# AIBluefisher/DReg-NeRF

Measured on AMD Instinct MI355X. Metric: nerf_pairs_per_sec_regtr_fwd_bwd_128, higher is better.
Workload: dtype bf16; 1 GPU; RegTR fwd+bwd+AdamW, shell-R synthetic pairs, 128^3 grids, 4 pairs (8 grids) per GPU per step, random-init weights; global_batch_pairs=4, resolution=128, fpn_head=active-set (identical results; rows around occupied voxels), parallelism=dp1

## Files before the change

dreg_nerf_amd/csrc/conv.hip:

```cpp
#include "common.h"
#include "../../include/dreg_nerf.h"
#include <cstring>
extern "C" int dreg_fill_zero(void* p, size_t bytes, void* stream);

struct ConvGeom {
    int B, Di, Hi, Wi, Cin, log2Cin;
    int Cmask;
    int Do, Ho, Wo, Cout;
    int ksz, ntaps;
    int sn, dsign, off, sd;
    uint32_t M;
    uint32_t magW, magH, magD;
    int Kpad;
};

__device__ __forceinline__ void tap_decode(int tap, int ksz, int& dz, int& dy, int& dx) {
    if (ksz == 1) { dz = dy = dx = 0; }
    else if (ksz == 3) { dz = tap / 9; int r = tap - dz * 9; dy = r / 3; dx = r - dy * 3; }
    else { int k2 = ksz * ksz; dz = tap / k2; int r = tap - dz * k2; dy = r / ksz; dx = r - dy * ksz; }
}

__device__ __forceinline__ void vox_decode(uint32_t m, const ConvGeom& g, int& b, int& z, int& y, int& x) {
    uint32_t q1 = fdiv(m, g.magW); x = (int)(m - q1 * g.Wo);
    uint32_t q2 = fdiv(q1, g.magH); y = (int)(q1 - q2 * g.Ho);
// ... 785 lines not shown
        }
    };

    if (v_begin < v_end) {
        const int nk = (int)((v_end - v_begin + KV - 1) / KV);
        auto next = [&](int k) {
            if (rowocc)
                while (k < nk && rowocc[(v_begin + (uint32_t)k * KV) / (uint32_t)g.Wo] == 0) ++k;
            return k;
        };
        int k = next(0), buf = 0;
        if (k < nk) {
            load_g(v_begin + (uint32_t)k * KV);
            store_l(0);
        }
        __syncthreads();
        while (k < nk) {
            const int kn = next(k + 1);
            if (kn < nk) load_g(v_begin + (uint32_t)kn * KV);
            compute(buf);
            if (kn < nk) store_l(buf ^ 1);
            __syncthreads();
            k = kn; buf ^= 1;
        }
    }
    float* dst = part + (size_t)blockIdx.y * g.Cout * g.Kpad;
    const int col_l = lane & 15, rowq = (lane >> 4) * 4;
#pragma unroll
    for (int i = 0; i < TM; ++i)
#pragma unroll
        for (int r = 0; r < 4; ++r) {
            const int co = co0 + wm * WM + i * 16 + rowq + r;
#pragma unroll
            for (int j = 0; j < TN; ++j)
                dst[(size_t)co * g.Kpad + n0 + wn * WN + j * 16 + col_l] = acc[i][j][r];
        }
}

#ifdef DREG_PROBE
__device__ unsigned long long g_wgrad_dbg[8];
#endif
template <int GP> __device__ __forceinline__ int wg_swz(int row) {
    return GP >= 16 ? (((row & 3) + 4 * ((row >> 3) & 1)) << 1) : ((((row >> 1) & 1) + 2 * ((row >> 3) & 1)) << 1);
}

struct WgradGroupDesc {
    const bf16_t* gout; const bf16_t* in; float* part;
    ConvGeom g;
    int tilesCol, tiles, nsplit;
    uint32_t vps, gbytes, ibytes, nrows;
    int block0;
};
static_assert(sizeof(WgradGroupDesc) == 144, "descriptor layout is part of the ABI (dreg_wgrad_group_desc_bytes)");
template <int BM, int BNC, bool ROWS, int NW = 4, int ABL = 0, int KV_ = 64, int NS_ = 2, int PIPE = 0, int AP = 0, bool GRP = false>
__global__ __launch_bounds__(NW * 64) void conv_wgrad_glds_kernel(
    const bf16_t* __restrict__ gout, const bf16_t* __restrict__ in, float* __restrict__ part,
    ConvGeom g, int tilesCol, int tiles, int nsplit, uint32_t vox_per_split, uint32_t gout_bytes, uint32_t in_bytes,
    const int* __restrict__ rowlist, uint32_t nrows, const uint8_t* __restrict__ rowocc = nullptr, int rows_fast = 0)
{
    uint32_t bid = blockIdx.x;
    if constexpr (GRP) {
        const WgradGroupDesc* D = reinterpret_cast<const WgradGroupDesc*>(rowocc);
        int lo = 0, hi = rows_fast - 1;
        while (lo < hi) {
            const int mid = (lo + hi + 1) >> 1;
            if (D[mid].block0 <= (int)bid) lo = mid; else hi = mid - 1;
        }
        const WgradGroupDesc d = D[lo];
        gout = d.gout; in = d.in; part = d.part; g = d.g; tilesCol = d.tilesCol; tiles = d.tiles; nsplit = d.nsplit;
        vox_per_split = d.vps; gout_bytes = d.gbytes; in_bytes = d.ibytes; nrows = d.nrows;
        rowocc = nullptr; rows_fast = 0; rowlist = nullptr;
        bid -= (uint32_t)d.block0;
    }
    typedef __attribute__((address_space(3))) void* lds_ptr_t;
    typedef __attribute__((address_space(3))) bf16x4_t* lds4_t;
    constexpr int KV = KV_, NS = NS_;
    constexpr int RSA = BM * 2, RSB = BNC * 2;
    constexpr int GPA = RSA / 16, GPB = RSB / 16;
    constexpr int A_BYTES = KV * RSA, B_BYTES = KV * RSB, STAGE = A_BYTES + B_BYTES;
    constexpr int IA = A_BYTES / 1024 / NW, IB = B_BYTES / 1024 / NW;
    constexpr int LPS = IA + IB;
    static_assert(IA >= 1 && IB >= 1, "stage too small for the wave count");
    constexpr int RPA = 64 / GPA, RPB = 64 / GPB;
    constexpr int WAVES_N = NW / 2;
    constexpr int WN = BNC / WAVES_N, WM = BM / 2, TM = WM / 16, TN = WN / 16;
    constexpr uint32_t OOB = 0x7fffff00u;
    extern __shared__ __attribute__((aligned(16))) char smem[];

    const int t = threadIdx.x, lane = t & 63;
    const int wave = __builtin_amdgcn_readfirstlane(t >> 6);
    const int wm = wave / WAVES_N, wn = wave % WAVES_N;
    uint32_t split, tile;
    if ((nsplit & 7) == 0) { const uint32_t xcd = bid & 7, j = bid >> 3; split = (j / tiles) * 8 + xcd; tile = j % tiles; }
    else { split = bid / tiles; tile = bid - split * tiles; }
    const uint32_t tile_r = tile / tilesCol, tile_c = tile - tile_r * tilesCol;
    const int co0 = tile_r * BM, n0 = tile_c * BNC;
    const uint32_t v_begin = split * vox_per_split;
    const uint32_t v_end = min(v_begin + vox_per_split, nrows);
    const int* srow = reinterpret_cast<const int*>(smem + NS * STAGE);
    typedef __attribute__((ext_vector_type(2))) uint32_t u32x2_t;
    const u32x2_t* srow2 = reinterpret_cast<const u32x2_t*>(smem + NS * STAGE);
    if constexpr (ROWS && AP >= 3) {
        u32x2_t* w2_ = reinterpret_cast<u32x2_t*>(smem + NS * STAGE);
        const uint32_t nreal = v_begin < v_end ? v_end - v_begin : 0u;
        const uint32_t npad = ((nreal + KV - 1) / KV + 4) * KV;
        const uint32_t m_sent = 0x7fffff00u / (uint32_t)((g.Cout > g.Cin ? g.Cout : g.Cin) * 2) + 1u;
        for (uint32_t i = t; i < npad; i += NW * 64) {
            if (i < nreal) {
                const int m = rowlist[v_begin + i];
                int b, z, y, x;
                vox_decode((uint32_t)m, g, b, z, y, x);
                const uint32_t fl = (z == 0 ? 1u : 0u) | (z == g.Do - 1 ? 2u : 0u) | (y == 0 ? 4u : 0u) | (y == g.Ho - 1 ? 8u : 0u) |
                                    (x == 0 ? 16u : 0u) | (x == g.Wo - 1 ? 32u : 0u) | 256u;
                w2_[i] = (u32x2_t){(uint32_t)m, fl};
            } else w2_[i] = (u32x2_t){m_sent, 128u};
        }
        __syncthreads();
    } else
    if constexpr (ROWS) {
        int* w_ = reinterpret_cast<int*>(smem + NS * STAGE);
        u32x2_t* w2_ = reinterpret_cast<u32x2_t*>(smem + NS * STAGE);
        for (uint32_t i = v_begin + t; i < v_end; i += NW * 64) {
            const int m = rowlist[i];
            if (rows_fast) {
                int b, z, y, x;
                vox_decode((uint32_t)m, g, b, z, y, x);
                w2_[i - v_begin] = (u32x2_t){(uint32_t)m, ((uint32_t)z << 20) | ((uint32_t)y << 10) | (uint32_t)x};
            } else w_[i - v_begin] = m;
        }
        __syncthreads();
    }
    const __amdgpu_buffer_rsrc_t rs_g = __builtin_amdgcn_make_buffer_rsrc((void*)gout, 0, gout_bytes, 0x00020000);
    const __amdgpu_buffer_rsrc_t rs_in = __builtin_amdgcn_make_buffer_rsrc((void*)in, 0, in_bytes, 0x00020000);

    const int ra = lane / GPA, rb = lane / GPB;
    uint32_t a_col[IA];
    int b_dz[IB], b_dy[IB], b_dx[IB], b_ci[IB];
    bool b_tv[IB];
#pragma unroll
    for (int i = 0; i < IA; ++i) {
        const int row = (wave * IA + i) * RPA + ra;
        a_col[i] = (uint32_t)(co0 + (((lane % GPA) ^ wg_swz<GPA>(row)) * 8)) * 2u;
    }
#pragma unroll
    for (int i = 0; i < IB; ++i) {
        const int row = (wave * IB + i) * RPB + rb;
        const int n = n0 + (((lane % GPB) ^ wg_swz<GPB>(row)) * 8);
        const int tap = n >> g.log2Cin;
        b_ci[i] = n & g.Cmask;
        tap_decode(tap, g.ksz, b_dz[i], b_dy[i], b_dx[i]);
        b_dz[i] *= g.dsign; b_dy[i] *= g.dsign; b_dx[i] *= g.dsign;
        b_tv[i] = tap < g.ntaps && b_ci[i] < g.Cin;
    }

    f32x4_t acc[TM][TN];
#pragma unroll
    for (int i = 0; i < TM; ++i)
#pragma unroll
        for (int j = 0; j < TN; ++j) acc[i][j] = (f32x4_t){0.f, 0.f, 0.f, 0.f};

    const bool aligned = !ROWS && g.sn == 1 && g.sd == 1 && g.dsign == 1 &&
                         (((KV % g.Wo) == 0 && ((g.Ho * g.Wo) % KV) == 0) || (g.Wo % KV) == 0) &&
                         (uint64_t)g.B * g.Di * g.Hi * g.Wi * g.Cin * 2 < 0x7fffff00ull;
    int al_dz[IB], al_dy[IB], al_x[IB];
    uint32_t al_off[IB];
    uint32_t al_l[IB];
    if (ROWS && rows_fast) {
#pragma unroll
        for (int i = 0; i < IB; ++i) {
            al_dz[i] = g.off + b_dz[i]; al_dy[i] = g.off + b_dy[i]; al_x[i] = g.off + b_dx[i];
            al_off[i] = (uint32_t)((((al_dz[i] * g.Hi + al_dy[i]) * g.Wi + al_x[i]) * g.Cin + b_ci[i]) * 2);
        }
    }
    if (aligned) {
#pragma unroll
        for (int i = 0; i < IB; ++i) {
            const int l = (wave * IB + i) * RPB + rb;
            const int ly = l / g.Wo, lx = l - ly * g.Wo;
            al_l[i] = b_tv[i] ? (uint32_t)l : 0x7fffffffu;
            al_dz[i] = g.off + b_dz[i];
            al_dy[i] = ly + g.off + b_dy[i];
            al_x[i] = lx + g.off + b_dx[i];
            al_off[i] = (uint32_t)((((al_dz[i] * g.Hi + al_dy[i]) * g.Wi + al_x[i]) * g.Cin + b_ci[i]) * 2);
        }
    }

    auto issue = [&](uint32_t v0, int buf) {
        char* sA = smem + buf * STAGE;
        char* sB = sA + A_BYTES;
        if constexpr (ROWS) {
            if (rows_fast) {
                uint32_t am[IA];
                u32x2_t bm[IB];
                const uint32_t last = v_end - 1 - v_begin;
#pragma unroll
                for (int i = 0; i < IA; ++i) am[i] = srow2[min(v0 + (wave * IA + i) * RPA + ra - v_begin, last)][0];
#pragma unroll
                for (int i = 0; i < IB; ++i) bm[i] = srow2[min(v0 + ((wave * IB) + i) * RPB + rb - v_begin, last)];
#pragma unroll
                for (int i = 0; i < IA; ++i) {
                    const int j = wave * IA + i;
                    const uint32_t vi = v0 + j * RPA + ra;
                    const uint32_t voff = (vi < v_end) ? am[i] * (uint32_t)(g.Cout * 2) + a_col[i] : OOB;
                    if constexpr (ABL != 3) __builtin_amdgcn_raw_ptr_buffer_load_lds(rs_g, (lds_ptr_t)(sA + j * 1024), 16, (int)voff, 0, 0, 0);
                    else asm volatile("" :: "v"(voff));
                }
#pragma unroll
                for (int i = 0; i < IB; ++i) {
                    const int j = wave * IB + i;
                    const uint32_t vi = v0 + j * RPB + rb, p = bm[i][1];
                    const bool v = vi < v_end && b_tv[i] && (unsigned)((int)(p >> 20) + al_dz[i]) < (unsigned)g.Di &&
                                   (unsigned)((int)((p >> 10) & 1023u) + al_dy[i]) < (unsigned)g.Hi && (unsigned)((int)(p & 1023u) + al_x[i]) < (unsigned)g.Wi;
// ... 127 lines not shown
            for (int ks = 0; ks < KS; ++ks)
#pragma unroll
                for (int grp = 0; grp < NG; ++grp) {
                    const int as = (ks * NG + grp) & 1, bs = ks & 1;
                    if (grp + 1 < NG) rdA(ks, grp + 1, as ^ 1);
                    else if (ks + 1 < KS) { rdB(ks + 1, bs ^ 1); rdA(ks + 1, 0, as ^ 1); }
                    __builtin_amdgcn_sched_barrier(0);
                    bf16x8_t af[G], bf[TN];
#pragma unroll
                    for (int i = 0; i < G; ++i) { i32x4_t t4 = {alo[as][i][0], alo[as][i][1], ahi[as][i][0], ahi[as][i][1]}; af[i] = __builtin_bit_cast(bf16x8_t, t4); }
#pragma unroll
                    for (int j = 0; j < TN; ++j) { i32x4_t t4 = {blo[bs][j][0], blo[bs][j][1], bhi[bs][j][0], bhi[bs][j][1]}; bf[j] = __builtin_bit_cast(bf16x8_t, t4); }
#pragma unroll
                    for (int i = 0; i < G; ++i)
#pragma unroll
                        for (int j = 0; j < TN; ++j)
                            acc[grp * G + i][j] = __builtin_amdgcn_mfma_f32_16x16x32_bf16(af[i], bf[j], acc[grp * G + i][j], 0, 0, 0);
                    asm volatile("s_waitcnt lgkmcnt(0)" ::: "memory");
                    __builtin_amdgcn_sched_barrier(0);
                }
            return;
        }
#pragma unroll
        for (int ks = 0; ks < KV / 32; ++ks) {
            const int kb = ks * 32 + (lane >> 4) * 8;
            const int r0 = kb + (fi >> 2), r1 = r0 + 4;
            i32x2_t alo[TM], ahi[TM], blo[TN], bhi[TN];
#pragma unroll
            for (int i = 0; i < TM; ++i) {
                const int gi = (wm * WM + i * 16) / 8 + ((fi & 3) >> 1), o8 = (fi & 1) * 8;
                alo[i] = tr_read(sA + r0 * RSA + ((gi ^ wg_swz<GPA>(r0)) << 4) + o8);
                ahi[i] = tr_read(sA + r1 * RSA + ((gi ^ wg_swz<GPA>(r1)) << 4) + o8);
            }
#pragma unroll
            for (int j = 0; j < TN; ++j) {
                const int gi = (wn * WN + j * 16) / 8 + ((fi & 3) >> 1), o8 = (fi & 1) * 8;
                blo[j] = tr_read(sB + r0 * RSB + ((gi ^ wg_swz<GPB>(r0)) << 4) + o8);
                bhi[j] = tr_read(sB + r1 * RSB + ((gi ^ wg_swz<GPB>(r1)) << 4) + o8);
            }
            asm volatile("s_waitcnt lgkmcnt(0)" ::: "memory");
            __builtin_amdgcn_sched_barrier(0);
            bf16x8_t af[TM], bf[TN];
#pragma unroll
            for (int i = 0; i < TM; ++i) { typedef __attribute__((ext_vector_type(4))) int i32x4_t; i32x4_t t4 = {alo[i][0], alo[i][1], ahi[i][0], ahi[i][1]}; af[i] = __builtin_bit_cast(bf16x8_t, t4); }
#pragma unroll
            for (int j = 0; j < TN; ++j) { typedef __attribute__((ext_vector_type(4))) int i32x4_t; i32x4_t t4 = {blo[j][0], blo[j][1], bhi[j][0], bhi[j][1]}; bf[j] = __builtin_bit_cast(bf16x8_t, t4); }
#pragma unroll
            for (int i = 0; i < TM; ++i)
#pragma unroll
                for (int j = 0; j < TN; ++j) {
                    if constexpr (ABL != 1) acc[i][j] = __builtin_amdgcn_mfma_f32_16x16x32_bf16(af[i], bf[j], acc[i][j], 0, 0, 0);
                    else asm volatile("" :: "v"(af[i]), "v"(bf[j]));
                }
        }
    };

    if constexpr (AP) {
        constexpr bool FAST = AP >= 3, STAMP = (AP == 2 || AP == 4);
        static_assert(NW == 8 && KV == 32 && NS == 4 && PIPE == 0 && LPS <= 15, "anti-phase loop: 8 waves, four 32-voxel units in the ring");
        if (v_begin < v_end) {
            const int nk = (int)((v_end - v_begin + KV - 1) / KV);
            const int grp = wave >> 2;
            const int fi = lane & 15;
            i32x2_t alo[TM], ahi[TM], blo[TN], bhi[TN];
            uint32_t fa[TM + TN];
            if constexpr (FAST) {
                static_assert(RSA == RSB, "one row stride for both operands");
                const int kb = (lane >> 4) * 8;
                const int r0 = kb + (fi >> 2);
#pragma unroll
                for (int i = 0; i < TM; ++i) {
                    const int gi = (wm * WM + i * 16) / 8 + ((fi & 3) >> 1), o8 = (fi & 1) * 8;
                    fa[i] = lds_base + r0 * RSA + ((gi ^ wg_swz<GPA>(r0)) << 4) + o8;
                }
#pragma unroll
                for (int j = 0; j < TN; ++j) {
                    const int gi = (wn * WN + j * 16) / 8 + ((fi & 3) >> 1), o8 = (fi & 1) * 8;
                    fa[TM + j] = lds_base + A_BYTES + r0 * RSB + ((gi ^ wg_swz<GPB>(r0)) << 4) + o8;
                }
            }
            auto tr_read_o = [&](uint32_t addr, int which) -> i32x2_t {
                i32x2_t v;
                if constexpr (ABL != 2) {
                    if (which == 0) asm volatile("ds_read_b64_tr_b16 %0, %1" : "=v"(v) : "v"(addr));
                    else if (which == 1) asm volatile("ds_read_b64_tr_b16 %0, %1 offset:%2" : "=v"(v) : "v"(addr), "n"(4 * RSA));
                    else if (which == 2) asm volatile("ds_read_b64_tr_b16 %0, %1 offset:%2" : "=v"(v) : "v"(addr), "n"(STAGE));
                    else asm volatile("ds_read_b64_tr_b16 %0, %1 offset:%2" : "=v"(v) : "v"(addr), "n"(STAGE + 4 * RSA));
                } else { v = (i32x2_t){(int)addr, (int)addr}; asm volatile("" : "+v"(v)); }
                return v;
            };
            auto rd = [&](int buf) {
                if constexpr (FAST) {
                    const int odd = (buf & 1) * 2;
#pragma unroll
                    for (int i = 0; i < TM; ++i) { alo[i] = tr_read_o(fa[i], odd); ahi[i] = tr_read_o(fa[i], odd + 1); }
#pragma unroll
                    for (int j = 0; j < TN; ++j) { blo[j] = tr_read_o(fa[TM + j], odd); bhi[j] = tr_read_o(fa[TM + j], odd + 1); }
                    return;
                }
                const uint32_t sA = lds_base + buf * STAGE;
                const uint32_t sB = sA + A_BYTES;
                const int kb = (lane >> 4) * 8;
                const int r0 = kb + (fi >> 2), r1 = r0 + 4;
#pragma unroll
                for (int i = 0; i < TM; ++i) {
                    const int gi = (wm * WM + i * 16) / 8 + ((fi & 3) >> 1), o8 = (fi & 1) * 8;
                    alo[i] = tr_read(sA + r0 * RSA + ((gi ^ wg_swz<GPA>(r0)) << 4) + o8);
                    ahi[i] = tr_read(sA + r1 * RSA + ((gi ^ wg_swz<GPA>(r1)) << 4) + o8);
                }
#pragma unroll
                for (int j = 0; j < TN; ++j) {
                    const int gi = (wn * WN + j * 16) / 8 + ((fi & 3) >> 1), o8 = (fi & 1) * 8;
                    blo[j] = tr_read(sB + r0 * RSB + ((gi ^ wg_swz<GPB>(r0)) << 4) + o8);
                    bhi[j] = tr_read(sB + r1 * RSB + ((gi ^ wg_swz<GPB>(r1)) << 4) + o8);
                }
            };
            auto mm = [&]() {
                typedef __attribute__((ext_vector_type(4))) int i32x4_t;
                bf16x8_t af[TM], bf[TN];
#pragma unroll
                for (int i = 0; i < TM; ++i) { i32x4_t t4 = {alo[i][0], alo[i][1], ahi[i][0], ahi[i][1]}; af[i] = __builtin_bit_cast(bf16x8_t, t4); }
#pragma unroll
                for (int j = 0; j < TN; ++j) { i32x4_t t4 = {blo[j][0], blo[j][1], bhi[j][0], bhi[j][1]}; bf[j] = __builtin_bit_cast(bf16x8_t, t4); }
#pragma unroll
                for (int i = 0; i < TM; ++i)
#pragma unroll
                    for (int j = 0; j < TN; ++j) {
                        if constexpr (ABL != 1) acc[i][j] = __builtin_amdgcn_mfma_f32_16x16x32_bf16(af[i], bf[j], acc[i][j], 0, 0, 0);
                        else asm volatile("" :: "v"(af[i]), "v"(bf[j]));
                    }
            };
            uint32_t pa_off[IA], pb_off[IB], pb_m[IB];
            int cz = 0, cy = 0, cx = 0;
            uint32_t lp = 0;
            u32x2_t lm[IA];
            if constexpr (FAST && ROWS) {
                static_assert(IA == IB && RPA == RPB, "one row per lane for both operands");
                lp = lds_base + NS * STAGE + (uint32_t)(wave * IA * RPA + ra) * 8u;
#pragma unroll
                for (int i = 0; i < IA; ++i) pa_off[i] = a_col[i];
#pragma unroll
                for (int i = 0; i < IB; ++i) {
                    const int dz = g.off + b_dz[i], dy = g.off + b_dy[i], dx = g.off + b_dx[i];
                    pb_off[i] = (uint32_t)((((dz * g.Hi + dy) * g.Wi + dx) * g.Cin + b_ci[i]) * 2);
                    pb_m[i] = (dz < 0 ? 1u : 0u) | (dz > 0 ? 2u : 0u) | (dy < 0 ? 4u : 0u) | (dy > 0 ? 8u : 0u) |
                              (dx < 0 ? 16u : 0u) | (dx > 0 ? 32u : 0u) | 128u | (b_tv[i] ? 0u : 256u);
                }
            } else
            if constexpr (FAST) {
#pragma unroll
                for (int i = 0; i < IA; ++i) pa_off[i] = (uint32_t)((wave * IA + i) * RPA + ra) * (uint32_t)(g.Cout * 2) + a_col[i];
#pragma unroll
                for (int i = 0; i < IB; ++i) {
                    const int l = (wave * IB + i) * RPB + rb;
                    const int dz = g.off + b_dz[i], dy = g.off + b_dy[i], dx = g.off + b_dx[i];
                    pb_off[i] = (uint32_t)((((dz * g.Hi + dy) * g.Wi + (l + dx)) * g.Cin + b_ci[i]) * 2);
                    pb_m[i] = (dz < 0 ? 1u : 0u) | (dz > 0 ? 2u : 0u) | (dy < 0 ? 4u : 0u) | (dy > 0 ? 8u : 0u) |
                              (l + dx < 0 ? 16u : 0u) | (l + dx >= KV ? 32u : 0u) | (b_tv[i] ? 0u : 64u);
                }
                int cb;
                vox_decode(v_begin, g, cb, cz, cy, cx);
            }
            uint32_t voa[IA], vob[IB];
            uint32_t cur_a = v_begin * (uint32_t)(g.Cout * 2), cur_b = v_begin * (uint32_t)(g.Cin * 2);
            uint32_t m_zy = 0;
            auto zy_flags = [&]() { m_zy = (cz == 0 ? 1u : 0u) | (cz == g.Do - 1 ? 2u : 0u) | (cy == 0 ? 4u : 0u) | (cy == g.Ho - 1 ? 8u : 0u) | 64u; };
            if constexpr (FAST) zy_flags();
            uint32_t nx_mask = 0, nx_a = 0, nx_b = 0;
            auto prep_scalar = [&]() {
                nx_mask = m_zy | (cx == 0 ? 16u : 0u) | (cx + KV == g.Wo ? 32u : 0u);
                nx_a = cur_a; nx_b = cur_b;
                cur_a += (uint32_t)(KV * 2) * (uint32_t)g.Cout; cur_b += (uint32_t)(KV * 2) * (uint32_t)g.Cin; cx += KV;
                if (cx == g.Wo) {
                    asm volatile("" ::: "memory");
                    cx = 0; if (++cy == g.Ho) { cy = 0; if (++cz == g.Do) cz = 0; } zy_flags();
                }
            };
            auto prep_fast = [&]() {
#pragma unroll
                for (int i = 0; i < IA; ++i) voa[i] = nx_a + pa_off[i];
#pragma unroll
                for (int i = 0; i < IB; ++i) vob[i] = (pb_m[i] & nx_mask) == 0u ? nx_b + pb_off[i] : OOB;
            };
// ... 37 lines not shown
            }
            if constexpr (FAST && ROWS) {
                for (int p = nk < 3 ? nk : 3; p < 3; ++p) list_read();
                list_read(); asm volatile("s_waitcnt lgkmcnt(0)" ::: "memory"); prep_rows();
            } else if constexpr (FAST) { prep_scalar(); prep_fast(); }
            if (nk >= 3) asm volatile("s_waitcnt vmcnt(%0)" ::"n"(2 * LPS) : "memory");
            else if (nk == 2) asm volatile("s_waitcnt vmcnt(%0)" ::"n"(LPS) : "memory");
            else asm volatile("s_waitcnt vmcnt(0)" ::: "memory");
            __builtin_amdgcn_s_barrier();
            if (grp) __builtin_amdgcn_s_barrier();
            unsigned long long dsum[6] = {0, 0, 0, 0, 0, 0}, tprev = 0;
            auto stamp = [&](int q) {
                if constexpr (STAMP) {
                    unsigned long long tnow;
                    asm volatile("s_memtime %0\n\ts_waitcnt lgkmcnt(0)" : "=s"(tnow) :: "memory");
                    if (q >= 0) dsum[q] += tnow - tprev;
                    tprev = tnow;
                }
            };
            stamp(-1);
            auto unit = [&](int u, int slot) {
                rd(slot);
                if constexpr (FAST && ROWS) list_read();
                stamp(0);
                if (u + 3 < nk) {
                    request(u + 3);
                    stamp(1);
                    asm volatile("s_waitcnt vmcnt(%0)" ::"n"(2 * LPS) : "memory");
                } else {
                    stamp(1);
                    if (u + 2 < nk) asm volatile("s_waitcnt vmcnt(%0)" ::"n"(LPS) : "memory");
                    else asm volatile("s_waitcnt vmcnt(0)" ::: "memory");
                }
                asm volatile("s_waitcnt lgkmcnt(0)" ::: "memory");
                stamp(2);
                __builtin_amdgcn_sched_barrier(0);
                __builtin_amdgcn_s_barrier();
                stamp(3);
                __builtin_amdgcn_s_setprio(1);
                if constexpr (FAST && ROWS) prep_rows();
                else if constexpr (FAST) { prep_scalar(); prep_fast(); }
                mm();
                if constexpr (FAST) {
#pragma unroll
                    for (int q = 0; q < 14; ++q) {
                        __builtin_amdgcn_sched_group_barrier(0x008, 1, 0);
                        __builtin_amdgcn_sched_group_barrier(0x004, 1, 0);
                        __builtin_amdgcn_sched_group_barrier(0x008, 1, 0);
                        __builtin_amdgcn_sched_group_barrier(0x002, 1, 0);
                    }
                }
                __builtin_amdgcn_s_setprio(0);
                __builtin_amdgcn_sched_barrier(0);
                stamp(4);
                __builtin_amdgcn_s_barrier();
                stamp(5);
            };
            if constexpr (FAST) {
                for (int u = 0; u < nk; u += 4) {
                    unit(u, 0);
                    if (u + 1 < nk) unit(u + 1, 1);
#pragma unroll
                    for (int k = 0; k < TM + TN; ++k) fa[k] += 2u * STAGE;
                    if (u + 2 < nk) unit(u + 2, 2);
                    if (u + 3 < nk) unit(u + 3, 3);
#pragma unroll
                    for (int k = 0; k < TM + TN; ++k) fa[k] -= 2u * STAGE;
                }
            } else {
                for (int u = 0; u < nk; ++u) unit(u, u & 3);
            }
            if (!grp) __builtin_amdgcn_s_barrier();
            if constexpr (STAMP) {
#ifdef DREG_PROBE
                if (lane == 0) {
                    for (int q = 0; q < 6; ++q) atomicAdd(&g_wgrad_dbg[q], dsum[q]);
                    atomicAdd(&g_wgrad_dbg[6], (unsigned long long)nk);
                    atomicAdd(&g_wgrad_dbg[7], 1ull);
                }
#endif
            }
        }
    } else
    if (v_begin < v_end) {
        const int nk = (int)((v_end - v_begin + KV - 1) / KV);
        if (rowocc) {
            uint8_t* socc = reinterpret_cast<uint8_t*>(smem + NS * STAGE);
            for (int i = t; i < nk; i += NW * 64) socc[i] = rowocc[(v_begin + (uint32_t)i * KV) / (uint32_t)g.Wo];
            __syncthreads();
            auto next = [&](int k) { while (k < nk && socc[k] == 0) ++k; return k; };
            int k = next(0), buf = 0;
            if (k < nk) issue(v_begin + (uint32_t)k * KV, 0);
            while (k < nk) {
                const int kn = next(k + 1);
                asm volatile("s_waitcnt vmcnt(0)" ::: "memory");
                __builtin_amdgcn_s_barrier();
                if (kn < nk) issue(v_begin + (uint32_t)kn * KV, buf ^ 1);
                compute(buf);
                k = kn; buf ^= 1;
            }
        } else {
        static_assert(NS >= 2 && NS <= 5 && 3 * LPS <= 63, "ring depth / counted wait range");
        for (int p = 0; p < NS - 1 && p < nk; ++p) issue(v_begin + (uint32_t)p * KV, p);
        int cur = 0, nxt = NS - 1;
        for (int k = 0; k < nk; ++k) {
            const int ahead = min(nk - 1 - k, NS - 2);
            if (ahead >= 3) asm volatile("s_waitcnt vmcnt(%0)" ::"n"(3 * LPS) : "memory");
            else if (ahead == 2) asm volatile("s_waitcnt vmcnt(%0)" ::"n"(2 * LPS) : "memory");
            else if (ahead == 1) asm volatile("s_waitcnt vmcnt(%0)" ::"n"(LPS) : "memory");
            else asm volatile("s_waitcnt vmcnt(0)" ::: "memory");
            __builtin_amdgcn_s_barrier();
            if (k + NS - 1 < nk) issue(v_begin + (uint32_t)(k + NS - 1) * KV, nxt);
            compute(cur);
            cur = cur + 1 == NS ? 0 : cur + 1;
            nxt = nxt + 1 == NS ? 0 : nxt + 1;
        }
        }
    }
    float* dst = part + (size_t)split * g.Cout * g.Kpad;
    const int col_l = lane & 15, rowq = (lane >> 4) * 4;
#pragma unroll
    for (int i = 0; i < TM; ++i)
#pragma unroll
        for (int r = 0; r < 4; ++r) {
            const int co = co0 + wm * WM + i * 16 + rowq + r;
#pragma unroll
            for (int j = 0; j < TN; ++j) {
                const int n = n0 + wn * WN + j * 16 + col_l;
                if (n < g.Kpad) dst[(size_t)co * g.Kpad + n] = acc[i][j][r];
            }
        }
}

struct WgradReduceDesc {
    const float* part; float* dw;
    int nsplit, Cout, Kpad, ntaps, Cin, Cin_real, accumulate, block0;
};
static_assert(sizeof(WgradReduceDesc) == 48, "descriptor layout is part of the ABI");
constexpr int WR_STAGE = 8192;
__host__ __device__ static inline int wr_epb(int nsplit) { return nsplit < 8 ? 2048 : (nsplit < 64 ? 512 : 128); }
__host__ __device__ static inline int wr_chunk(int nsplit) { return nsplit < 32 ? 64 : 16; }
static inline int wgrad_reduce_blocks(int Cout, int Cin_real, int ntaps, int nsplit)
{
    if (ntaps == 1) return (int)(((size_t)Cout * Cin_real + wr_epb(nsplit) - 1) / wr_epb(nsplit));
    return Cout * ((Cin_real + wr_chunk(nsplit) - 1) / wr_chunk(nsplit));
}
__device__ __forceinline__ float wr_sum(const float* p, size_t slab, int k0, int kstep, int nsplit)
{
    float a = 0.f;
#pragma unroll 4
    for (int k = k0; k < nsplit; k += kstep) a += p[(size_t)k * slab];
    return a;
}
__device__ __forceinline__ void wgrad_reduce_block(const WgradReduceDesc& d, int r, float* stage)
{
    const int t = threadIdx.x;
    const size_t slab = (size_t)d.Cout * d.Kpad;
    int nwritten = d.nsplit;
    if (d.accumulate & 2) {
        const int e = *reinterpret_cast<const int*>(d.part + (size_t)d.nsplit * slab);
        nwritten = e < 1 ? 1 : (e < d.nsplit ? e : d.nsplit);
    }
    const bool accum = (d.accumulate & 1) != 0;
    if (d.ntaps == 1) {
        const int epb = wr_epb(d.nsplit), KG = 2048 / epb, EL = 256 / KG, g = t / EL, l = t - g * EL;
        const size_t total = (size_t)d.Cout * d.Cin_real;
        const bool vec = (d.Cin_real & 3) == 0;
        const int per = vec ? 4 : 1, passes = epb / (EL * per);
        for (int ps = 0; ps < passes; ++ps) {
            const size_t i = (size_t)r * epb + (size_t)(ps * EL + l) * per;
            float4 a = make_float4(0.f, 0.f, 0.f, 0.f);
            if (i < total) {
                const int co = (int)(i / d.Cin_real), ci = (int)(i - (size_t)co * d.Cin_real);
                const float* src = d.part + (size_t)co * d.Kpad + ci;
                if (vec) {
#pragma unroll 4
                    for (int k = g; k < nwritten; k += KG) {
                        const float4 v = *reinterpret_cast<const float4*>(src + (size_t)k * slab);
                        a.x += v.x; a.y += v.y; a.z += v.z; a.w += v.w;
                    }
                } else a.x = wr_sum(src, slab, g, KG, nwritten);
            }
            if (KG > 1) {
                __syncthreads();
                reinterpret_cast<float4*>(stage)[g * EL + l] = a;
                __syncthreads();
                if (g == 0) {
                    a = reinterpret_cast<float4*>(stage)[l];
                    for (int q = 1; q < KG; ++q) { const float4 v = reinterpret_cast<float4*>(stage)[q * EL + l]; a.x += v.x; a.y += v.y; a.z += v.z; a.w += v.w; }
                }
            }
            if (g == 0 && i < total) {
                if (vec) {
                    float4* o = reinterpret_cast<float4*>(d.dw + i);
                    if (accum) { const float4 q = *o; a.x += q.x; a.y += q.y; a.z += q.z; a.w += q.w; }
                    *o = a;
                } else d.dw[i] = accum ? d.dw[i] + a.x : a.x;
            }
        }
        return;
    }
    const int cc = wr_chunk(d.nsplit);
    const int nchunk = (d.Cin_real + cc - 1) / cc;
    const int co = r / nchunk, ci0 = (r - co * nchunk) * cc;
    const int nci = min(cc, d.Cin_real - ci0);
    const int chp = d.Cin < cc ? d.Cin : cc;
    const int sh = 31 - __builtin_clz(chp);
    const int ne = d.ntaps << sh;
    const int no = nci * d.ntaps;
    const int KG = (d.nsplit >= 8 && 4 * no <= WR_STAGE) ? 4 : 1, EL = 256 / KG, g = t / EL, l = t - g * EL;
    const float* src = d.part + (size_t)co * d.Kpad + ci0;
    if ((chp & 3) == 0 && (d.Cin & 3) == 0 && (d.Kpad & 3) == 0) {
        for (int e = l; e < (ne >> 2); e += EL) {
            const int tap = (e << 2) >> sh, cl = (e << 2) & (chp - 1);
            if (cl >= nci) continue;
            const float* p = src + (size_t)tap * d.Cin + cl;
// ... 611 lines not shown
    static_assert(sizeof(PackDesc) == 48, "descriptor layout is part of the ABI");
    if (n <= 0 || total_rows <= 0) return DREG_OK;
    if (stage_floats < 0 || (size_t)stage_floats * 4 > 48 * 1024) return DREG_EINVAL;
    hipLaunchKernelGGL(pack_weights_batched_kernel, dim3(total_rows), dim3(256), (size_t)(stage_floats > 0 ? 64 * 125 : 1) * 4, (hipStream_t)stream,
                       (const PackDesc*)descs, n, row_desc);
    DREG_LAUNCH_CHECK();
    return DREG_OK;
}

DREG_KNOB(int, g_force_wgrad_splits, 0);
DREG_KNOB(int, g_wgrad_target_blocks, 384);
#ifdef DREG_PROBE
void dreg_conv_set_narrow_small(int on) { if (on >= 10) { g_narrow_small = 2; g_narrow_thr = on; } else { g_narrow_small = on; g_narrow_thr = 224; } }
void dreg_conv_set_glds_stages(int stages) { g_glds_stages = (stages >= 2 && stages <= 4) ? stages : 0; }
void dreg_conv_set_wgrad_target_blocks(int blocks) { g_wgrad_target_blocks = blocks > 0 ? blocks : 384; }
void dreg_conv_set_wgrad_splits(int splits) { g_force_wgrad_splits = splits; }
#endif
int dreg_conv3d_wgrad_splits(int B, int Do, int Ho, int Wo, int Cin, int Cout, int ksz, int dtype) {
    if (g_force_wgrad_splits > 0) {
        const long Mf = (long)B * Do * Ho * Wo;
        long f = g_force_wgrad_splits;
        if (f > (Mf + 63) / 64) f = (Mf + 63) / 64;
        return (int)(f > 64 ? 64 : (f < 1 ? 1 : f));
    }
    const int Kpad = dreg_conv3d_kpad(ksz, Cin, dtype);
    const int bnc = (Kpad % 128 == 0 || (dtype == 0 && Kpad > 128)) ? 128 : 64;
    const long tiles = (long)((Cout % 128 == 0) ? Cout / 128 : Cout / 64) * ((Kpad + bnc - 1) / bnc);
    const long M = (long)B * Do * Ho * Wo;
    long s = (g_wgrad_target_blocks + tiles - 1) / tiles;
    const long vmin = ksz == 1 ? 512 : 1024;
    const long maxs = (M + vmin - 1) / vmin;
    if (s > maxs) s = maxs;
    if (s < 1) s = 1;
    const long cap = (tiles * 64 >= 1024 || dtype != 0) ? 64 : ((1024 + tiles - 1) / tiles > 512 ? 512 : (1024 + tiles - 1) / tiles);
    if (s > cap) s = cap;
    if (s > 8) s = (s + 7) / 8 * 8;
    if (dtype == 0 && Cout % 256 == 0 && (Kpad % 256 == 0 || Kpad >= 1024) && M >= 65536) {
        const long t256 = (long)(Cout / 256) * ((Kpad + 255) / 256);
        long best = s;
        double best_eff = 0.0;
        for (long c = 24; c <= 64; c += 8) {
            if (M / c < 2048) break;
            const double rounds = (double)(t256 * c) / 256.0;
            const double eff = rounds / (double)((t256 * c + 255) / 256);
            if (eff >= best_eff - 1e-9) { best_eff = eff; best = c; }
        }
        if (best_eff > 0.0) s = best;
    }
    return (int)s;
}
size_t dreg_conv3d_wgrad_workspace_bytes(int B, int Do, int Ho, int Wo, int Cin, int Cout, int ksz, int dtype) {
    const int Kpad = dreg_conv3d_kpad(ksz, Cin, dtype);
    return (size_t)dreg_conv3d_wgrad_splits(B, Do, Ho, Wo, Cin, Cout, ksz, dtype) * Cout * Kpad * sizeof(float) + 256;
}
DREG_KNOB(bool, g_row_splits, true);
#ifdef DREG_PROBE
extern "C" void dreg_conv_set_row_splits(int on) { g_row_splits = on != 0; }
#endif
static int wgrad_row_splits(int Cout, int Kpad, int ksz, uint32_t nrows, int smax, bool tile256)
{
    if (smax <= 1 || !g_row_splits) return smax;
    if (tile256) {
        const long t256 = (long)(Cout / 256) * ((Kpad + 255) / 256);
        const long vmax = (((long)160 * 1024 - (long)4 * 32 * 512 * 2 - 5 * 32 * 8) / 8) / 64 * 64;
        long cmin = ((long)nrows + vmax - 1) / vmax;
        if (cmin < 1) cmin = 1;
        if (cmin >= smax) return smax;
        long cmax = (long)nrows / 2048;
        if (cmax > smax) cmax = smax;
        if (cmax < cmin) cmax = cmin;
        long best = cmin;
        double best_eff = -1.0;
        for (long c = cmin; c <= cmax; ++c) {
            const double eff = (double)(t256 * c) / 256.0 / (double)((t256 * c + 255) / 256);
            if (eff > best_eff + 1e-9) { best_eff = eff; best = c; }
        }
        return (int)best;
    }
    const long vmin = ksz == 1 ? 512 : 1024;
    long s = ((long)nrows + vmin - 1) / vmin;
    if (s < 1) s = 1;
    return (int)(s < smax ? s : smax);
}

}

enum WgradFamily {
    WG_UNSUPPORTED = -1,
    WG_REG,
    WG_GLDS4,
    WG_256x128,
    WG_DENSE8,
    WG_ROWS8,
    WG_ROWS8_AP
};
struct WgradChoice {
    WgradFamily family;
    int bm, bnc, tilesRow, tilesCol;
    int smax, nsplit;
    uint32_t vps;
    int rows_fast;
    bool occ;
    int abl, kv, ns, pipe, ap;
    uint64_t gbytes, ibytes;
    dim3 grid; int block; size_t lds;
};
// ... 7 lines not shown
    const bool k256 = Cout % 256 == 0 && (Kpad % 256 == 0 || Kpad >= 1024);
    const bool rows_ap = rowlist && same_vol && g_rows_fast && g_wgrad_big == 3 && g_wgrad_ring == 3 && g.ksz <= 3 && k256 && nrows >= 16384;
    c.nsplit = rowlist ? wgrad_row_splits(Cout, Kpad, g.ksz, nrows, c.smax, rows_ap) : c.smax;
    c.vps = (uint32_t)((nrows + c.nsplit - 1) / c.nsplit);
    c.vps = ((c.vps + 63) / 64) * 64;
    if (c.vps == 0) c.vps = 64;
    c.gbytes = (uint64_t)g.M * Cout * 2; c.ibytes = (uint64_t)g.B * g.Di * g.Hi * g.Wi * g.Cin * 2;
    const bool glds = dtype == 0 && use_tr && g_use_glds && c.gbytes < 0x7fffff00ull && c.ibytes < 0x7fffff00ull;
    c.bm = (Cout % 128 == 0) ? 128 : 64;
    c.bnc = (Kpad % 128 == 0 || (glds && Kpad > 128)) ? 128 : 64;
    if (g_narrow_small >= 2 && dtype == 0 && (Cout / c.bm) * ((Kpad + c.bnc - 1) / c.bnc) * c.nsplit < g_narrow_thr) {
        if (c.bnc == 128) c.bnc = 64;
        if (c.bm == 128 && (Cout / c.bm) * (Kpad / c.bnc) * c.nsplit < g_narrow_thr) c.bm = 64;
    }
    c.occ = occ && !rowlist && g.Wo % 64 == 0;
    c.kv = 64; c.ns = 2; c.block = 256;
    size_t lds_rows = 0;
    if (!glds) c.family = WG_REG;
    else if (rowlist && c.vps > 20480) { c.family = WG_UNSUPPORTED; return c; }
    else if (rows_ap && (size_t)4 * 32 * 512 * 2 + ((size_t)c.vps + 5 * 32) * 8 <= (size_t)160 * 1024) {
        c.family = WG_ROWS8_AP; c.kv = 32; c.ns = 4; c.ap = 3; c.rows_fast = 1; lds_rows = ((size_t)c.vps + 5 * 32) * 8;
    } else if (rowlist && same_vol && g_rows_fast && g_wgrad_big == 3 && Cout % 256 == 0 && Kpad % 256 == 0 && nrows >= 65536 &&
               (size_t)2 * 64 * 512 * 2 + (size_t)c.vps * 8 <= (size_t)160 * 1024) {
        c.family = WG_ROWS8; c.rows_fast = 1; lds_rows = (size_t)c.vps * 8;
    } else if (!rowlist && !c.occ && g_wgrad_big && Cout % 256 == 0 && (Kpad % 256 == 0 || (Kpad >= 1024 && g_wgrad_big == 3 && g_wgrad_ring >= 3 && !g_wgrad_pipe)) && nrows >= 65536) {
        c.family = WG_DENSE8;
        if (g_wgrad_big == 1) { c.family = WG_256x128; c.kv = 32; }
        else if (g_wgrad_big >= 11 && g_wgrad_big <= 13) c.abl = g_wgrad_big - 10;
        else if (g_wgrad_pipe && !g_wgrad_ring) c.pipe = 1;
        else if (g_wgrad_ring == 2) { c.kv = 32; c.ns = 5; }
        else if (g_wgrad_ring >= 3 && g_wgrad_ring <= 8) {
            const bool fast_ok = g.ksz <= 3 && g.sn == 1 && g.sd == 1 && g.dsign == 1 && g.Di == g.Do && g.Hi == g.Ho && g.Wi == g.Wo && (g.Wo % 32) == 0 &&
                                 (g.M % 32u) == 0 && (c.vps % 32u) == 0;
            c.kv = 32; c.ns = 4;
            if (g_wgrad_ring == 8 || !fast_ok) c.ap = 1;
            else if (g_wgrad_ring == 3) c.ap = 3;
            else { c.ap = 4; c.abl = g_wgrad_ring == 5 ? 2 : (g_wgrad_ring == 6 ? 3 : (g_wgrad_ring == 7 ? 1 : 0)); }
        } else if (g_wgrad_ring == 1) { c.kv = 32; c.ns = 4; }
    } else {
        c.family = WG_GLDS4;
        if (rowlist) {
            c.rows_fast = (same_vol && g_rows_fast && (size_t)2 * 64 * (c.bm + c.bnc) * 2 + (size_t)c.vps * 8 <= (size_t)160 * 1024) ? 1 : 0;
            lds_rows = (size_t)c.vps * (c.rows_fast ? 8 : 4);
        } else if (c.occ) lds_rows = (size_t)(c.vps / 64 + 16);
    }
    if (c.family == WG_256x128) { c.bm = 256; c.bnc = 128; }
    else if (c.family >= WG_DENSE8) { c.bm = 256; c.bnc = 256; c.block = 512; }
    c.tilesRow = Cout / c.bm; c.tilesCol = (Kpad + c.bnc - 1) / c.bnc;
    if (c.family == WG_REG) { c.grid = dim3(c.tilesRow * c.tilesCol, c.nsplit); c.lds = (size_t)2 * 32 * (c.bm + c.bnc) * es; }
    else { c.grid = dim3(c.tilesRow * c.tilesCol * c.nsplit); c.lds = (size_t)c.ns * c.kv * (c.bm + c.bnc) * 2 + lds_rows; }
    return c;
}

struct WgradArgs { const void *gout, *in; float* part; const int* rowlist; uint32_t nrows; const uint8_t* rowocc; };
template <typename T, bool TR>
static void wgrad_reg_launch(const WgradChoice& c, const ConvGeom& g, const WgradArgs& a, hipStream_t st)
{
#define WG_LAUNCH(BMv, BNv) hipLaunchKernelGGL((conv_wgrad_kernel<T, BMv, BNv, TR>), c.grid, dim3(c.block), c.lds, st, (const T*)a.gout, (const T*)a.in, a.part, g, c.tilesCol, c.vps, a.rowocc)
    if (c.bm == 128 && c.bnc == 128) WG_LAUNCH(128, 128); else if (c.bm == 128) WG_LAUNCH(128, 64);
    else if (c.bnc == 128) WG_LAUNCH(64, 128); else WG_LAUNCH(64, 64);
#undef WG_LAUNCH
}
template <int BM, int BNC, bool ROWS, int NW = 4, int ABL = 0, int KV = 64, int NS = 2, int PIPE = 0, int AP = 0>
static void wgrad_glds_launch(const WgradChoice& c, const ConvGeom& g, const WgradArgs& a, hipStream_t st)
{
    if (c.lds > 65536) (void)hipFuncSetAttribute((const void*)conv_wgrad_glds_kernel<BM, BNC, ROWS, NW, ABL, KV, NS, PIPE, AP>, hipFuncAttributeMaxDynamicSharedMemorySize, (int)c.lds);
    hipLaunchKernelGGL((conv_wgrad_glds_kernel<BM, BNC, ROWS, NW, ABL, KV, NS, PIPE, AP>), c.grid, dim3(c.block), c.lds, st, (const bf16_t*)a.gout, (const bf16_t*)a.in, a.part, g,
                       c.tilesCol, c.tilesRow * c.tilesCol, c.nsplit, c.vps, (uint32_t)c.gbytes, (uint32_t)c.ibytes, a.rowlist, a.nrows, a.rowocc, c.rows_fast);
}
template <bool ROWS>
static void wgrad_glds4_launch(const WgradChoice& c, const ConvGeom& g, const WgradArgs& a, hipStream_t st)
{
    if (c.bm == 128 && c.bnc == 128) wgrad_glds_launch<128, 128, ROWS>(c, g, a, st); else if (c.bm == 128) wgrad_glds_launch<128, 64, ROWS>(c, g, a, st);
    else if (c.bnc == 128) wgrad_glds_launch<64, 128, ROWS>(c, g, a, st); else wgrad_glds_launch<64, 64, ROWS>(c, g, a, st);
}
static void wgrad_dense8_launch(const WgradChoice& c, const ConvGeom& g, const WgradArgs& a, hipStream_t st)
{
#define D8(A, KVv, NSv, PPv, APv) if (c.abl == A && c.kv == KVv && c.ns == NSv && c.pipe == PPv && c.ap == APv) return wgrad_glds_launch<256, 256, false, 8, A, KVv, NSv, PPv, APv>(c, g, a, st)
    D8(0, 32, 4, 0, 3); D8(0, 32, 4, 0, 1);
    D8(0, 64, 2, 0, 0); D8(0, 32, 4, 0, 0); D8(0, 32, 5, 0, 0); D8(0, 64, 2, 1, 0);
    D8(1, 64, 2, 0, 0); D8(2, 64, 2, 0, 0); D8(3, 64, 2, 0, 0);
    D8(0, 32, 4, 0, 4); D8(1, 32, 4, 0, 4); D8(2, 32, 4, 0, 4); D8(3, 32, 4, 0, 4);
#undef D8
}

static int wgrad_impl(const void* gout, const void* in, float* dw, void* workspace, size_t workspace_bytes,
                      int B, int Di, int Hi, int Wi, int Cin, int Cin_real, int Do, int Ho, int Wo, int Cout,
                      int ksz, int stride, int pad, int accumulate, int dtype, int use_tr, void* stream,
                      const int* rowlist, uint32_t nrows_list, const uint8_t* rowocc = nullptr, bool defer_reduce = false)
{
    ConvGeom g;
    int rc = fill_geom(g, B, Di, Hi, Wi, Cin, Do, Ho, Wo, Cout, ksz, stride, pad, 0, dtype == 0 ? 2 : 4);
    if (rc) return rc;
    if (Cout % 128 != 0 && Cout != 64) return DREG_EINVAL;
    if (workspace_bytes < dreg_conv3d_wgrad_workspace_bytes(B, Do, Ho, Wo, Cin, Cout, ksz, dtype)) return DREG_EINVAL;
    if (rowlist && !(dtype == 0 && use_tr && g_use_glds)) return DREG_EINVAL;
    hipStream_t st = (hipStream_t)stream;
    const WgradChoice c = wgrad_choose(g, dtype, use_tr != 0, rowlist != nullptr, nrows_list, rowocc != nullptr);
    float* part = (float*)workspace;
    const WgradArgs a{gout, in, part, rowlist, rowlist ? nrows_list : g.M, c.occ ? rowocc : nullptr};
    switch (c.family) {
    case WG_UNSUPPORTED: return DREG_EINVAL;
    case WG_REG:
        if (dtype != 0) wgrad_reg_launch<float, false>(c, g, a, st);
        else if (use_tr) wgrad_reg_launch<bf16_t, true>(c, g, a, st);
        else wgrad_reg_launch<bf16_t, false>(c, g, a, st);
        break;
    case WG_GLDS4: if (rowlist) wgrad_glds4_launch<true>(c, g, a, st); else wgrad_glds4_launch<false>(c, g, a, st); break;
    case WG_256x128: wgrad_glds_launch<256, 128, false, 4, 0, 32>(c, g, a, st); break;
    case WG_DENSE8: wgrad_dense8_launch(c, g, a, st); break;
    case WG_ROWS8: wgrad_glds_launch<256, 256, true, 8>(c, g, a, st); break;
    case WG_ROWS8_AP: wgrad_glds_launch<256, 256, true, 8, 0, 32, 4, 0, 3>(c, g, a, st); break;
    }
    DREG_LAUNCH_CHECK();
    if (defer_reduce) {
        if (rowlist && hipMemsetD32Async((hipDeviceptr_t)(part + (size_t)c.smax * Cout * g.Kpad), c.nsplit, 1, st) != hipSuccess) return DREG_ELAUNCH;
        return DREG_OK;
    }
    if (g.ntaps > 1 && (size_t)g.ntaps * (Cin < 64 ? Cin : 64) > (size_t)WR_STAGE) return DREG_EINVAL;
    WgradReduceDesc rd{part, dw, c.nsplit, Cout, g.Kpad, g.ntaps, Cin, Cin_real, accumulate, 0};
    hipLaunchKernelGGL(wgrad_reduce_kernel, dim3(wgrad_reduce_blocks(Cout, Cin_real, g.ntaps, c.nsplit)), dim3(256), 0, st, rd);
    DREG_LAUNCH_CHECK();
    return DREG_OK;
}

extern "C" {

int dreg_wgrad_group_desc_bytes() { return (int)sizeof(WgradGroupDesc); }
int dreg_linear_wgrad_group_fill(void* desc_host, const void* gout, const void* in, void* workspace, size_t workspace_bytes,
                                 int rows, int Cin, int Cout, int* variant, int* nblocks)
{
    return dreg_conv3d_wgrad_group_fill(desc_host, gout, in, workspace, workspace_bytes, rows, 1, 1, 1, Cin, 1, 1, 1, Cout, 1, 1, 0, variant, nblocks);
}
int dreg_conv3d_wgrad_group_fill(void* desc_host, const void* gout, const void* in, void* workspace, size_t workspace_bytes,
                                 int B, int Di, int Hi, int Wi, int Cin, int Do, int Ho, int Wo, int Cout, int ksz, int stride, int pad,
                                 int* variant, int* nblocks)
{
    ConvGeom g;
    int rc = fill_geom(g, B, Di, Hi, Wi, Cin, Do, Ho, Wo, Cout, ksz, stride, pad, 0, 2);
    if (rc) return rc;
    if (Cout % 128 != 0 && Cout != 64) return DREG_EINVAL;
    if (workspace_bytes < dreg_conv3d_wgrad_workspace_bytes(B, Do, Ho, Wo, Cin, Cout, ksz, 0)) return DREG_EINVAL;
    const WgradChoice c = wgrad_choose(g, 0, true, false, 0, false);
    if (c.family != WG_GLDS4) return DREG_EINVAL;
    WgradGroupDesc d{};
    d.gout = (const bf16_t*)gout; d.in = (const bf16_t*)in; d.part = (float*)workspace; d.g = g;
    d.tilesCol = c.tilesCol; d.tiles = c.tilesRow * c.tilesCol; d.nsplit = c.nsplit; d.vps = c.vps; d.gbytes = (uint32_t)c.gbytes; d.ibytes = (uint32_t)c.ibytes;
    d.nrows = g.M; d.block0 = 0;
    std::memcpy(desc_host, &d, sizeof(d));
    *variant = c.bm * 1000 + c.bnc;
    *nblocks = (int)c.grid.x;
    return DREG_OK;
}
int dreg_wgrad_group_launch(const void* descs_dev, int n, int variant, int total_blocks, void* stream)
{
    if (n <= 0 || total_blocks <= 0) return DREG_OK;
    if (!descs_dev) return DREG_EINVAL;
    hipStream_t st = (hipStream_t)stream;
    const int bm = variant / 1000, bnc = variant % 1000;
    const ConvGeom g0{};
#define WGRP(BMv, BNv) hipLaunchKernelGGL((conv_wgrad_glds_kernel<BMv, BNv, false, 4, 0, 64, 2, 0, 0, true>), dim3(total_blocks), dim3(256), (size_t)2 * 64 * (BMv + BNv) * 2, st, \
        (const bf16_t*)nullptr, (const bf16_t*)nullptr, (float*)nullptr, g0, 0, 0, 0, 0u, 0u, 0u, (const int*)nullptr, 0u, (const uint8_t*)descs_dev, n)
    if (bm == 128 && bnc == 128) WGRP(128, 128); else if (bm == 128 && bnc == 64) WGRP(128, 64);
    else if (bm == 64 && bnc == 128) WGRP(64, 128); else if (bm == 64 && bnc == 64) WGRP(64, 64);
    else return DREG_EINVAL;
#undef WGRP
    DREG_LAUNCH_CHECK();
    return DREG_OK;
}

int dreg_conv3d_wgrad(const void* gout, const void* in, float* dw, void* workspace, size_t workspace_bytes,
                      int B, int Di, int Hi, int Wi, int Cin, int Cin_real, int Do, int Ho, int Wo, int Cout,
                      int ksz, int stride, int pad, int accumulate, int dtype, int use_tr, void* stream)
{
    return wgrad_impl(gout, in, dw, workspace, workspace_bytes, B, Di, Hi, Wi, Cin, Cin_real, Do, Ho, Wo, Cout, ksz, stride, pad,
                      accumulate, dtype, use_tr, stream, nullptr, 0);
}
int dreg_conv3d_wgrad_occ(const void* gout, const void* in, float* dw, void* workspace, size_t workspace_bytes,
                          int B, int Di, int Hi, int Wi, int Cin, int Cin_real, int Do, int Ho, int Wo, int Cout,
                          int ksz, int stride, int pad, int accumulate, int dtype, int use_tr, const uint8_t* rowocc, void* stream)
{
    return wgrad_impl(gout, in, dw, workspace, workspace_bytes, B, Di, Hi, Wi, Cin, Cin_real, Do, Ho, Wo, Cout, ksz, stride, pad,
                      accumulate, dtype, use_tr, stream, nullptr, 0, rowocc);
}

int dreg_conv3d_igemm_rows(const void* in, const void* wt_packed, void* out, const float* bias, const void* addend,
                           const int* rows, int nrows,
                           int B, int Di, int Hi, int Wi, int Cin, int Do, int Ho, int Wo, int Cout,
                           int ksz, int stride, int pad, int transposed, int relu, int Da, int Ha, int Wa, int add_same,
                           int out_f32, void* stream)
{
    ConvGeom g;
    int rc = fill_geom(g, B, Di, Hi, Wi, Cin, Do, Ho, Wo, Cout, ksz, stride, pad, transposed, 2);
    if (rc) return rc;
    if (!rows || nrows < 0) return DREG_EINVAL;
    const int add_shift = add_same ? 0 : 1;
    hipStream_t st = (hipStream_t)stream;
    if (out_f32) return launch_conv<bf16_t, float>(in, wt_packed, out, bias, addend, g, relu, Da, Ha, Wa, add_shift, st, rows, (uint32_t)nrows);
    return launch_conv<bf16_t, bf16_t>(in, wt_packed, out, bias, addend, g, relu, Da, Ha, Wa, add_shift, st, rows, (uint32_t)nrows);
}
int dreg_conv3d_wgrad_partials(const void* gout, const void* in, void* workspace, size_t workspace_bytes, const int* rows, int nrows,
                               int B, int Di, int Hi, int Wi, int Cin, int Cin_real, int Do, int Ho, int Wo, int Cout,
                               int ksz, int stride, int pad, const uint8_t* rowocc, void* stream)
{
    if (rows && nrows < 0) return DREG_EINVAL;
    return wgrad_impl(gout, in, nullptr, workspace, workspace_bytes, B, Di, Hi, Wi, Cin, Cin_real, Do, Ho, Wo, Cout, ksz, stride, pad,
                      0, 0, 1, stream, rows, rows ? (uint32_t)nrows : 0, rows ? nullptr : rowocc, true);
}
int dreg_wgrad_reduce_blocks(int Cout, int Cin_real, int ksz, int nsplit) { return wgrad_reduce_blocks(Cout, Cin_real, ksz * ksz * ksz, nsplit); }
int dreg_wgrad_reduce_batched(const void* descs_dev, int n, int block_base, int nblocks, void* stream)
{
    if (n <= 0 || nblocks <= 0) return DREG_OK;
    if (!descs_dev || block_base < 0) return DREG_EINVAL;
    hipLaunchKernelGGL(wgrad_reduce_batched_kernel, dim3(nblocks), dim3(256), 0, (hipStream_t)stream, (const WgradReduceDesc*)descs_dev, n, block_base);
    DREG_LAUNCH_CHECK();
    return DREG_OK;
}
int dreg_conv3d_wgrad_variant(int B, int Do, int Ho, int Wo, int Cin, int Cout, int ksz, int rows, int nrows, int occ)
{
    ConvGeom g;
    if (fill_geom(g, B, Do, Ho, Wo, Cin, Do, Ho, Wo, Cout, ksz, 1, ksz / 2, 0, 2) || (Cout % 128 != 0 && Cout != 64) || (rows && nrows < 0)) return -1;
    const WgradChoice c = wgrad_choose(g, 0, true, rows != 0, (uint32_t)nrows, occ != 0);
    if (c.family == WG_UNSUPPORTED) return -1;
    return (c.family == WG_REG ? 1000000 : 0) + c.bm * 1000 + c.bnc;
}
int dreg_conv3d_wgrad_rows(const void* gout, const void* in, float* dw, void* workspace, size_t workspace_bytes,
                           const int* rows, int nrows,
                           int B, int Di, int Hi, int Wi, int Cin, int Cin_real, int Do, int Ho, int Wo, int Cout,
                           int ksz, int stride, int pad, int accumulate, void* stream)
{
    if (!rows || nrows < 0) return DREG_EINVAL;
    return wgrad_impl(gout, in, dw, workspace, workspace_bytes, B, Di, Hi, Wi, Cin, Cin_real, Do, Ho, Wo, Cout, ksz, stride, pad,
                      accumulate, 0, 1, stream, rows, (uint32_t)nrows);
}

}
```

dreg_nerf_amd/csrc/executor.hip:

```cpp
#include <hip/hip_runtime.h>
#include <cstdint>
#include <cstring>
#include <algorithm>
#include <vector>
#include <string>
#include <cstdio>
#include "../../include/dreg_nerf.h"
#ifndef DREG_ELAUNCH
#define DREG_ELAUNCH (-2)
#endif

namespace {

enum { OP_CONV = 0, OP_BN = 1, OP_MAXPOOL = 2, OP_CONV_ROWS = 3 };
constexpr int OP_INTS = 16;
constexpr int TENSOR_INTS = 5;
constexpr int RL = 8;
constexpr int PARAM_I64 = 5;

struct Tensor { int B, D, H, W, C; size_t bytes, off, goff; };
struct Param {
    float* val; float* grad; int d0, d1, ksz;
    size_t pk_fwd = SIZE_MAX, pk_dgrad = SIZE_MAX, pk_cls = SIZE_MAX;
    size_t pk_halo_fwd = SIZE_MAX, pk_halo_dgrad = SIZE_MAX;
    size_t pk_brick_fwd = SIZE_MAX, pk_brick_dgrad = SIZE_MAX;
    int cin_pad = 0;
};
struct Op {
    int kind, in, out, in2, w, b, p2, p3, p4, ksz, stride, pad, relu, add_same, rows_out, rows_in;
    size_t aux0 = 0, aux1 = 0;
    size_t wg_off = 0, wg_bytes = 0;
    int rd = -1;
    int ds_rows = -1;
    int sparse_gx = 0;
    size_t cl_off = 0;
    int cl_count = 0;
    int ds_sparse = 0;
    size_t cl2_off = 0;
    int cl2_count = 0;
    int pool = -1;
    int sstem = 0;
    int sstem_conv = -1, sstem_lat = -1;
    size_t xam_off = 0, pmask_off = 0;
    int halo = 0;
    int pointwise = 0;
    int stats_bn = -1;
    size_t stats_off = 0;
    int stats_conv = -1;
    int grp = 0;
    int fold_sk_fwd = 0, fold_sk_bwd = 0;
    int fold_into = -1, res_from = -1;
    int bt = -1;
    size_t keep_var = 0, keep_sums = 0;
    int self_coef = 0;
};
struct HaloPack { const float* w; size_t off; int Cout, Cin, transposed, brick; };
struct PackRec { const float* w; void* out; int Cout, Cin_real, inner, ntaps, for_dgrad, Kpad, dtype, row0; };
static_assert(sizeof(PackRec) == 48, "matches PackDesc of conv.hip");

struct ReduceRec { const float* part; float* dw; int nsplit, Cout, Kpad, ntaps, Cin, Cin_real, accumulate, block0; };
static_assert(sizeof(ReduceRec) == 48, "matches WgradReduceDesc of conv.hip");

struct BnTailRec { const float* a; const float* b; float* o0; float* o1; int B, V, C, block0; };
static_assert(sizeof(BnTailRec) == 48, "matches BnTailDesc of fpn_ops.hip");

struct TimedLaunch { hipEvent_t e0, e1; int op, kind, variant; };

struct Exec {
    std::vector<Tensor> t;
    std::vector<Op> ops;
    std::vector<Param> prm;
    std::vector<char> needs_grad;
    size_t act_bytes = 0, arena_bytes = 0, pack_bytes = 0;
    size_t off_bn_ws = 0, off_coef = 0, off_ks = 0, off_rd = 0, off_cs = 0, off_tmp = 0;
    size_t sz_ks = 0;
    std::vector<ReduceRec> reduce;
    const void* sparse_arena = nullptr;
    std::vector<ReduceRec> reduce_abs;
    int reduce_blocks = 0;
    const void* reduce_arena = nullptr;
    std::vector<BnTailRec> bn_fwd, bn_bwd;
    size_t off_bnf = 0, off_bnb = 0;
    int bn_blocks = 0;
    std::vector<PackRec> packs;
    std::vector<HaloPack> halo_packs;
    int pack_rows = 0, pack_max_floats = 0;
    int out_slot = -1;
    bool timing = false;
    std::vector<TimedLaunch> timed;
    size_t timed_used = 0;
    hipStream_t aux = nullptr;
    std::vector<hipEvent_t> ev;
    hipEvent_t ev_done = nullptr;
    bool use_aux = true;
    const uint8_t* in_rowocc = nullptr;
    char* pack_base = nullptr;
    std::vector<char> written;
    bool aux_used = false;
    struct GrpLaunch { size_t off; int n, variant, blocks; };
    std::vector<int> grp_ops;
    std::vector<GrpLaunch> grp_launch;
    size_t off_grp = 0;
    bool grp_ready = false;
    int pend_sk_bn = -1, pend_sk_n = 0;
    size_t pend_sk_slice = 0;
    const void* fwd_rows_arena = nullptr;
    struct Band { size_t off; const char* tag; int idx; };
    std::vector<Band> bands;
    size_t off_guard_tab = 0, off_guard_res = 0;
    const void* guard_arena = nullptr;
    int guard_op = -1, guard_pass = 0; long long guard_band = -1;
    dreg_exec_opts opt;
};

inline size_t align256(size_t v) { return (v + 255) / 256 * 256; }
constexpr size_t GUARD_BYTES = 64 * 1024;
struct Bump {
    size_t v = 0;
    std::vector<Exec::Band>* bands = nullptr;
    const char* tag = "?"; int idx = -1;
    operator size_t() const { return v; }
    Bump& operator+=(size_t n) { v += n; if (bands && n) { bands->push_back(Exec::Band{v, tag, idx}); v += GUARD_BYTES; } return *this; }
    void name(const char* t, int i) { tag = t; idx = i; }
};
inline int out_dim(int i, int k, int s, int p) { return (i + 2 * p - k) / s + 1; }

struct Scope {
    Exec* e; hipStream_t st; TimedLaunch* tl = nullptr;
    Scope(Exec* ex, hipStream_t s, int op, int kind) : e(ex), st(s) {
        if (!e->timing) return;
        if (e->timed_used == e->timed.size()) {
            TimedLaunch n{}; n.op = op; n.kind = kind;
            if (hipEventCreate(&n.e0) != hipSuccess || hipEventCreate(&n.e1) != hipSuccess) return;
            e->timed.push_back(n);
        }
        tl = &e->timed[e->timed_used++];
        tl->op = op; tl->kind = kind; tl->variant = 0;
        (void)hipEventRecord(tl->e0, st);
    }
    ~Scope() { if (tl) (void)hipEventRecord(tl->e1, st); }
    void variant(int v) { if (tl) tl->variant = v; }
};

#define CK(expr) do { int rc_ = (expr); if (rc_) return rc_; } while (0)

bool s2_class_ok(const Param& p, int ksz, int stride, int pad)
{
    return stride == 2 && ((ksz == 3 && pad == 1) || (ksz == 1 && pad == 0)) && p.d0 % 64 == 0 && p.d1 % 64 == 0 && dreg_conv_get_glds();
}

}

extern "C" {

void dreg_exec_default_opts(dreg_exec_opts* o)
{
    std::memset(o, 0, sizeof(*o));
    o->sparse_grads = 1; o->bn_batch_tails = 1; o->fuse_stem = 1; o->sparse_stem = 1; o->fold_res_bn = 1; o->fold_splitk = 1;
    o->group_wgrad = 1; o->s2_accumulate = 1; o->fuse_bn_stats = 1; o->brick = 1; o->defer_head_pg = 0; o->pointwise_stream = 1;
    o->bn_self_coef = 1;
}
void* dreg_exec_create(const int* tensors, int nt, const int* ops, int nops, const int64_t* params, int np)
{
    return dreg_exec_create_opts(tensors, nt, ops, nops, params, np, nullptr);
}
void* dreg_exec_create_opts(const int* tensors, int nt, const int* ops, int nops, const int64_t* params, int np, const dreg_exec_opts* opts)
{
    Exec* e = new Exec();
    if (opts) e->opt = *opts; else dreg_exec_default_opts(&e->opt);
    e->opt.brick &= 3;
    const int g_sparse_grads = e->opt.sparse_grads, g_bn_batch_tails = e->opt.bn_batch_tails, g_fuse_stem = e->opt.fuse_stem, g_sparse_stem = e->opt.sparse_stem,
              g_fold_res_bn = e->opt.fold_res_bn, g_fold_splitk = e->opt.fold_splitk, g_group_wgrad = e->opt.group_wgrad, g_fuse_bn_stats = e->opt.fuse_bn_stats,
              g_brick = e->opt.brick, g_bn_self_coef = e->opt.bn_self_coef;
    e->t.resize(nt);
    for (int i = 0; i < nt; ++i) {
        Tensor& t = e->t[i];
        t.B = tensors[i * TENSOR_INTS]; t.D = tensors[i * TENSOR_INTS + 1]; t.H = tensors[i * TENSOR_INTS + 2];
        t.W = tensors[i * TENSOR_INTS + 3]; t.C = tensors[i * TENSOR_INTS + 4];
        t.bytes = align256((size_t)t.B * t.D * t.H * t.W * t.C * 2);
    }
    e->prm.resize(np);
    for (int i = 0; i < np; ++i) {
        Param& p = e->prm[i];
        p.val = (float*)params[i * PARAM_I64]; p.grad = (float*)params[i * PARAM_I64 + 1];
        p.d0 = (int)params[i * PARAM_I64 + 2]; p.d1 = (int)params[i * PARAM_I64 + 3]; p.ksz = (int)params[i * PARAM_I64 + 4];
    }
    e->ops.resize(nops);
    for (int i = 0; i < nops; ++i) {
        const int* r = ops + i * OP_INTS;
        Op& o = e->ops[i];
        o.kind = r[0]; o.in = r[1]; o.out = r[2]; o.in2 = r[3]; o.w = r[4]; o.b = r[5]; o.p2 = r[6]; o.p3 = r[7]; o.p4 = r[8];
        o.ksz = r[9]; o.stride = r[10]; o.pad = r[11]; o.relu = r[12]; o.add_same = r[13]; o.rows_out = r[14]; o.rows_in = r[15];
        if (o.in < 0 || o.in >= nt || o.out <= 0 || o.out >= nt || o.in2 >= nt) { delete e; return nullptr; }
    }
    e->out_slot = nops ? e->ops.back().out : -1;

    e->needs_grad.assign(nt, 0);
    for (const Op& o : e->ops) {
        bool g = e->needs_grad[o.in] || (o.in2 >= 0 && e->needs_grad[o.in2]);
        if (o.kind == OP_CONV || o.kind == OP_CONV_ROWS) g = g || e->prm[o.w].grad || (o.b >= 0 && e->prm[o.b].grad);
        if (o.kind == OP_BN) g = g || e->prm[o.w].grad || e->prm[o.b].grad;
        e->needs_grad[o.out] = g;
    }

    for (size_t i = 0; i + 1 < e->ops.size(); ++i) {
        Op& o = e->ops[i];
        if (o.kind != OP_BN || o.in2 >= 0 || o.out == e->out_slot) continue;
        int users = 0, pool = -1;
        for (size_t j = 0; j < e->ops.size(); ++j) {
            const Op& q = e->ops[j];
            if (q.in == o.out || q.in2 == o.out) { ++users; if (q.kind == OP_MAXPOOL && q.in == o.out && j > i) pool = (int)j; }
        }
        if (users == 1 && pool >= 0 && e->t[o.out].C % 8 == 0 && g_fuse_stem) { o.pool = pool; e->ops[pool].pool = (int)i; }
// ... 63 lines not shown
                o.xam_off = off; off += align256((size_t)p.B * p.D * p.H * p.W * p.C * 2);
                o.pmask_off = off; off += align256((size_t)p.B * p.D * p.H * p.W);
            }
            if (w > bn_ws) bn_ws = w;
            if (sb > coef) coef = sb;
            bool shared = false;
            for (const Op& q : e->ops) shared = shared || (&q != &o && q.kind == OP_BN && (q.w == o.w || q.b == o.b || q.p2 == o.p2 || q.p3 == o.p3));
            if (g_bn_batch_tails && o.pool < 0 && !shared && dreg_bn_small(x.B, (int)V, x.C, 0)) {
                o.keep_var = off; off += align256((size_t)x.B * x.C * sizeof(float));
                o.keep_sums = off; off += sb;
                BnTailRec f{}, b{};
                f.a = (const float*)o.aux1; f.b = (const float*)o.keep_var; f.o0 = e->prm[o.p2].val; f.o1 = e->prm[o.p3].val;
                b.a = (const float*)o.keep_sums; b.b = nullptr; b.o0 = e->prm[o.w].grad; b.o1 = e->prm[o.b].grad;
                f.B = b.B = x.B; f.V = b.V = (int)V; f.C = b.C = x.C; f.block0 = b.block0 = e->bn_blocks;
                e->bn_blocks += (x.C + 255) / 256;
                o.bt = (int)e->bn_fwd.size();
                e->bn_fwd.push_back(f); e->bn_bwd.push_back(b);
            } else if (g_bn_self_coef && g_bn_batch_tails && o.pool < 0 && !shared && o.fold_into < 0 &&
                       (dreg_bn_self_coef_use(x.B, (int)V, x.C, 0, 0) || dreg_bn_self_coef_use(x.B, (int)V, x.C, 0, 1))) {
                o.self_coef = (dreg_bn_self_coef_use(x.B, (int)V, x.C, 0, 0) ? 1 : 0) | (dreg_bn_self_coef_use(x.B, (int)V, x.C, 0, 1) ? 2 : 0);
                const size_t kb = align256((size_t)x.B * x.C * 2 * sizeof(double));
                o.keep_var = off; off += kb;
                o.keep_sums = off; off += kb;
                BnTailRec f{}, b{};
                f.b = (const float*)o.keep_var; f.o0 = e->prm[o.p2].val; f.o1 = e->prm[o.p3].val;
                b.b = (const float*)o.keep_sums; b.o0 = e->prm[o.w].grad; b.o1 = e->prm[o.b].grad;
                f.B = b.B = x.B; f.V = b.V = (int)V; f.C = b.C = x.C; f.block0 = b.block0 = e->bn_blocks;
                e->bn_blocks += (x.C + 255) / 256;
                o.bt = (int)e->bn_fwd.size();
                e->bn_fwd.push_back(f); e->bn_bwd.push_back(b);
            }
        } else if (o.kind == OP_MAXPOOL) {
            const Tensor& y = e->t[o.out];
            o.aux0 = off; off += align256((size_t)y.B * y.D * y.H * y.W * y.C);
        } else {
            const Param& w = e->prm[o.w];
            const Tensor& y = e->t[o.out];
            const size_t k1 = dreg_conv3d_igemm_workspace_bytes(x.B, x.D, x.H, x.W, x.C, y.D, y.H, y.W, w.d0, o.ksz, o.stride, o.pad, 0, o.in2 >= 0, 0);
            const size_t k2 = dreg_conv3d_igemm_workspace_bytes(x.B, y.D, y.H, y.W, w.d0, x.D, x.H, x.W, w.d1, o.ksz, o.stride, o.pad, 1, 0, 0);
            if (k1 > e->sz_ks) e->sz_ks = k1;
            if (k2 > e->sz_ks) e->sz_ks = k2;
            if (w.grad) {
                o.wg_bytes = dreg_conv3d_wgrad_workspace_bytes(x.B, y.D, y.H, y.W, x.C, w.d0, o.ksz, 0);
                bool shared = false;
                for (const ReduceRec& q : e->reduce) shared = shared || q.dw == w.grad;
                if (shared) o.rd = -2;
                else {
                    ReduceRec r{};
                    r.dw = w.grad; r.nsplit = dreg_conv3d_wgrad_splits(x.B, y.D, y.H, y.W, x.C, w.d0, o.ksz, 0);
                    r.Cout = w.d0; r.Kpad = dreg_conv3d_kpad(o.ksz, x.C, 0); r.ntaps = o.ksz * o.ksz * o.ksz; r.Cin = x.C; r.Cin_real = w.d1;
                    r.accumulate = (o.kind == OP_CONV_ROWS || o.rows_out >= 0) ? 3 : 1;
                    r.block0 = e->reduce_blocks;
                    e->reduce_blocks += dreg_wgrad_reduce_blocks(w.d0, w.d1, o.ksz, r.nsplit);
                    o.rd = (int)e->reduce.size();
                    e->reduce.push_back(r);
                }
            }
            const size_t c = dreg_colsum_workspace_bytes((size_t)y.B * y.D * y.H * y.W, w.d0);
            if (c > cs) cs = c;
        }
    }
    if (g_fuse_bn_stats) {
        for (size_t j = 0; j < e->ops.size(); ++j) {
            Op& bn = e->ops[j];
            if (bn.kind != OP_BN || bn.pool >= 0) continue;
            const Tensor& x = e->t[bn.in];
            const int V = x.D * x.H * x.W;
            if (V % 128 != 0 || dreg_bn_small(x.B, V, x.C, 0)) continue;
            int prod = -1, writers = 0;
            for (size_t i = 0; i < j; ++i) if (e->ops[i].out == bn.in) { prod = (int)i; ++writers; }
            if (writers != 1 || e->ops[prod].kind != OP_CONV || e->ops[prod].stats_bn >= 0) continue;
            {
                const Op& pc = e->ops[prod];
                const Tensor& px = e->t[pc.in];
                const Param& pp = e->prm[pc.w];
                if (!pc.relu && pp.d1 == px.C && pp.d0 != 64 && dreg_conv3_halo_use(px.B, px.D, px.H, px.W, px.C, pp.d0, pc.ksz, pc.stride, pc.pad)) continue;
            }
            e->ops[prod].stats_bn = (int)j;
            bn.stats_conv = prod;
            off.name("epilogue chunk sums of BatchNorm op", (int)j);
            bn.stats_off = off; off += align256((size_t)x.B * (V / 128) * x.C * 2 * sizeof(float));
        }
    }
    e->act_bytes = off;
    for (int i = 1; i < nt; ++i) {
        if (e->t[i].bytes > max_tensor) max_tensor = e->t[i].bytes;
        off.name("gradient of activation", i);
        if (e->needs_grad[i] && i != e->out_slot) { e->t[i].goff = off; off += e->t[i].bytes; } else e->t[i].goff = SIZE_MAX;
    }
    for (Op& o : e->ops) {
        if (o.kind != OP_CONV_ROWS || o.in2 < 0 || o.add_same || !e->needs_grad[o.in2] || !g_sparse_grads) continue;
        for (const Op& q : e->ops) if (q.out == o.in2 && q.kind == OP_CONV_ROWS) o.ds_rows = q.rows_out;
    }
    for (Op& o : e->ops) {
        if (o.kind != OP_CONV_ROWS || !e->needs_grad[o.in] || o.in == 0 || e->t[o.in].goff == SIZE_MAX) continue;
        int writers = 0;
        for (const Op& q : e->ops) {
            if (q.kind == OP_MAXPOOL && q.pool >= 0 && e->ops[q.pool].sstem) continue;
            if ((q.in == o.in || q.in2 == o.in) && e->needs_grad[q.out]) ++writers;
        }
        if (writers != 1 || !g_sparse_grads) continue;
        const Tensor& x = e->t[o.in];
        off.name("row-list copy (sparse_gx) of op", (int)(&o - e->ops.data()));
        o.sparse_gx = 1; o.cl_off = off; off += align256((size_t)x.B * x.D * x.H * x.W * sizeof(int));
    }
    for (Op& o : e->ops) {
// ... 500 lines not shown
            const Tensor& ta = e->t[o.in2];
            if (fresh) { if (hipMemsetAsync(A + ta.goff, 0, (size_t)ta.B * ta.D * ta.H * ta.W * ta.C * 2, st) != hipSuccess) return DREG_ELAUNCH; }
            else if (o.cl2_count > 0) CK(dreg_zero_rows(A + ta.goff, (const int*)(A + o.cl2_off), o.cl2_count, ta.C, 0, stream));
            o.cl2_count = 0;
        }
        e->sparse_arena = arena;
    }
    const int g_s2_accumulate = e->opt.s2_accumulate, g_group_wgrad = e->opt.group_wgrad, g_brick = e->opt.brick, g_defer_head_pg = e->opt.defer_head_pg;
    std::vector<char> rd_done(e->reduce.size(), 0);
    hipStream_t rd_stream = st;
    size_t rd_pending = 0;
    auto flush_reduce = [&]() -> int {
        for (int lo = 0, nrec = (int)rd_done.size(); lo < nrec;) {
            if (!rd_done[lo]) { ++lo; continue; }
            int hi = lo;
            while (hi + 1 < nrec && rd_done[hi + 1]) ++hi;
            Scope sc(e, rd_stream, -1, 3);
            const int b0 = e->reduce[lo].block0;
            const int b1 = hi + 1 < nrec ? e->reduce[hi + 1].block0 : e->reduce_blocks;
            CK(dreg_wgrad_reduce_batched((const ReduceRec*)(A + e->off_rd) + lo, hi - lo + 1, b0, b1 - b0, (void*)rd_stream));
            for (int q = lo; q <= hi; ++q) rd_done[q] = 0;
            lo = hi + 1;
        }
        return DREG_OK;
    };
    const bool grp_active = g_group_wgrad && e->grp_ready && aux_on && !e->timing && op_begin == 0 && op_end == (int)e->ops.size() && (flags & 3) == 3;
    std::vector<int> grp_seen;
    auto param_grads = [&](int i, bool event_recorded) -> int {
        const Op& o = e->ops[i];
        const Tensor& x = e->t[o.in];
        const Tensor& y = e->t[o.out];
        const Param& w = e->prm[o.w];
        const void* gy = grad(o.out);
        const bool rows = o.kind == OP_CONV_ROWS;
        const bool lrows = rows || (o.kind == OP_CONV && o.rows_out >= 0 && o.rows_out < nlists);
        const int* r_out = lrows ? (const int*)rowlists[RL * o.rows_out] : nullptr;
        const int n_out = lrows ? (int)rowlists[RL * o.rows_out + 1] : 0;
        hipStream_t ws = st;
        if (aux_on && !(grp_active && o.grp && !(o.b >= 0 && e->prm[o.b].grad))) {
            if (!e->ev[i] && hipEventCreateWithFlags(&e->ev[i], hipEventDisableTiming) != hipSuccess) return DREG_ELAUNCH;
            if (!event_recorded && hipEventRecord(e->ev[i], st) != hipSuccess) return DREG_ELAUNCH;
            if (hipStreamWaitEvent(e->aux, e->ev[i], 0) != hipSuccess) return DREG_ELAUNCH;
            ws = e->aux;
            aux_used = true;
        }
        hipStream_t bs = ws;
        bool flush_now = false;
        if (w.grad && grp_active && o.grp) {
            grp_seen.push_back(i);
        } else
        if (w.grad) {
            Scope sc(e, ws, i, 2);
            if (o.rd >= 0) {
                CK(dreg_conv3d_wgrad_partials(gy, act(o.in), A + o.wg_off, o.wg_bytes, lrows ? r_out : nullptr, n_out, x.B, x.D, x.H, x.W, x.C, w.d1,
                                              y.D, y.H, y.W, w.d0, o.ksz, rows ? 1 : o.stride, o.pad, (!lrows && o.in == 0) ? e->in_rowocc : nullptr, (void*)ws));
                rd_done[o.rd] = 1;
                rd_stream = ws;
                rd_pending += o.wg_bytes;
                flush_now = rd_pending >= ((size_t)192 << 20);
            } else if (lrows) {
                CK(dreg_conv3d_wgrad_rows(gy, act(o.in), w.grad, A + o.wg_off, o.wg_bytes, r_out, n_out, x.B, x.D, x.H, x.W, x.C, w.d1,
                                          y.D, y.H, y.W, w.d0, o.ksz, rows ? 1 : o.stride, o.pad, 1, (void*)ws));
            } else {
                CK(dreg_conv3d_wgrad_occ(gy, act(o.in), w.grad, A + o.wg_off, o.wg_bytes, x.B, x.D, x.H, x.W, x.C, w.d1, y.D, y.H, y.W, w.d0,
                                         o.ksz, o.stride, o.pad, 1, 0, 1, o.in == 0 ? e->in_rowocc : nullptr, (void*)ws));
            }
        }
        if (flush_now) { CK(flush_reduce()); rd_pending = 0; }
        if (o.b >= 0 && e->prm[o.b].grad) {
            if (rows) CK(dreg_colsum_rows(gy, r_out, n_out, e->prm[o.b].grad, (float*)(A + e->off_cs), w.d0, 1, 0, (void*)bs));
            else CK(dreg_colsum(gy, e->prm[o.b].grad, (float*)(A + e->off_cs), (size_t)y.B * y.D * y.H * y.W, w.d0, 1, 0, (void*)bs));
        }
        return DREG_OK;
    };
    auto flush_group = [&](int ev_op) -> int {
        if (grp_seen.empty()) return DREG_OK;
        if (!e->ev[ev_op] && hipEventCreateWithFlags(&e->ev[ev_op], hipEventDisableTiming) != hipSuccess) return DREG_ELAUNCH;
        if (hipEventRecord(e->ev[ev_op], st) != hipSuccess || hipStreamWaitEvent(e->aux, e->ev[ev_op], 0) != hipSuccess) return DREG_ELAUNCH;
        aux_used = true;
        if (grp_seen.size() == e->grp_ops.size()) {
            for (const Exec::GrpLaunch& q : e->grp_launch) CK(dreg_wgrad_group_launch(A + q.off, q.n, q.variant, q.blocks, (void*)e->aux));
        } else {
            for (int j : grp_seen) {
                const Op& oj = e->ops[j]; const Tensor& xj = e->t[oj.in]; const Tensor& yj = e->t[oj.out]; const Param& wj = e->prm[oj.w];
                CK(dreg_conv3d_wgrad_partials(grad(oj.out), act(oj.in), A + oj.wg_off, oj.wg_bytes, nullptr, 0, xj.B, xj.D, xj.H, xj.W, xj.C, wj.d1,
                                              yj.D, yj.H, yj.W, wj.d0, oj.ksz, oj.stride, oj.pad, nullptr, (void*)e->aux));
            }
        }
        for (int j : grp_seen) { rd_done[e->ops[j].rd] = 1; rd_pending += e->ops[j].wg_bytes; }
        rd_stream = e->aux;
        grp_seen.clear();
        return DREG_OK;
    };
    std::vector<int> deferred_pg;
    bool deep_reached = false;
    auto run_deferred = [&]() -> int {
        for (int j : deferred_pg) CK(param_grads(j, true));
        deferred_pg.clear();
        return DREG_OK;
    };
    for (int i = op_end - 1; i >= op_begin; --i) {
        if (i < op_end - 1) CK(guard_after_op(e, A, i + 1, 1, st, aux_on ? e->aux : nullptr));
        const Op& o = e->ops[i];
        const Tensor& x = e->t[o.in];
        const Tensor& y = e->t[o.out];
        if (o.kind == OP_MAXPOOL && o.pool >= 0) continue;
        if (o.kind == OP_BN && o.pool >= 0) {
            const Op& q = e->ops[o.pool];
            const Tensor& p = e->t[q.out];
            if (!e->needs_grad[q.out] || !written[q.out]) continue;
            if (!e->prm[o.w].grad || !e->prm[o.b].grad) return DREG_EINVAL;
            if (o.sstem) {
                const Op& cv = e->ops[o.sstem_conv];
                if (cv.rows_out >= nlists) return DREG_EINVAL;
                const int64_t* rl = rowlists + RL * cv.rows_out;
                const int* ra = nullptr; int na = 0;
                const bool lat = o.sstem_lat >= 0 && written[o.out];
                if (lat) { const int li = e->ops[o.sstem_lat].rows_in; ra = (const int*)rowlists[RL * li]; na = (int)rowlists[RL * li + 1]; }
                CK(dreg_sparse_stem_bwd(act(o.in), grad(q.out), (const uint8_t*)(A + q.aux0), A + o.xam_off, lat ? grad(o.out) : nullptr, ra, na,
                                        (const int*)rl[0], (int)rl[1], (float*)(A + o.aux0), (float*)(A + o.aux1), dst_for(o.in), e->prm[o.w].grad, e->prm[o.b].grad,
                                        (float*)(A + e->off_coef), (float*)(A + e->off_bn_ws), x.B, x.D, x.H, x.W, p.D, p.H, p.W, x.C, o.relu, 1, stream));
                CK(commit(o.in));
// ... 157 lines not shown
```

dreg_nerf_amd/csrc/pointset_exec.hip:

```cpp
#include <hip/hip_runtime.h>
#include <cstdint>
#include <cstring>
#include <algorithm>
#include <vector>
#include "../../include/dreg_nerf.h"
#ifndef DREG_ELAUNCH
#define DREG_ELAUNCH (-2)
#endif

namespace {

constexpr int E = 256, E3 = 768, FF = 1024, NL = 6, NH = 8;
enum { N1W, N1B, SIW, SIB, SOW, SOB, N2W, N2B, CIW, CIB, COW, COB, N3W, N3B, L1W, L1B, L2W, L2B, PL_COUNT };
enum { FNW = NL * PL_COUNT, FNB, QW, QB, KW, KB, CW, CB, PS_NPARAM };
enum { LIN_SI, LIN_SO, LIN_CI, LIN_CO, LIN_1, LIN_2, LIN_PER_LAYER };
constexpr int NLIN = NL * LIN_PER_LAYER + 2;

struct Lin { int cout, cin, w, b; };
struct ReduceRec { const float* part; float* dw; int nsplit, Cout, Kpad, ntaps, Cin, Cin_real, accumulate, block0; };
static_assert(sizeof(ReduceRec) == 48, "matches WgradReduceDesc of conv.hip");
struct ColsumRec { const void* g; float* out; float* partial; int M, C, rpc, nch, pblock0, fblock0, accumulate, pad; };
static_assert(sizeof(ColsumRec) == 56, "matches ColsumDesc of fpn_ops.hip");
struct LnRec { const float* part; float* dg; float* db; int nblk, accumulate; };
static_assert(sizeof(LnRec) == 32, "matches LnFinalDesc of pointset.hip");

inline size_t al(size_t v) { return (v + 255) / 256 * 256; }

struct LayerBuf {
    size_t xa, xb, st1, st2, st3, h1, h2, h3, qkv1, qkv2, o1, o2, lse1, lse2, f;
    size_t gF, gB, gQ2, gC, gQ1;
    size_t wg[LIN_PER_LAYER], cs[LIN_PER_LAYER], lnp[3];
};
struct Layout {
    int R = -1;
    size_t allx, stf, dec_in, q, k, corr_lse;
    LayerBuf L[NL];
    size_t dallx, dallx_bf, dq, dk, ddec, ddec2, dH, dO, dvec, gx[2], lnpf[2], wgq, wgk, csq, csk, ov_ws, ks_ws, cs_ws, tables;
    size_t ks_bytes = 0, total = 0;
    size_t wg_bytes[NLIN];
};

struct Ps {
    float* val[PS_NPARAM];
    float* grad[PS_NPARAM];
    Lin lin[NLIN];
    Layout lay;
    int fuse = 1;
    int panel = 2;
    int group_wgrad = 1;
    std::vector<hipEvent_t> ev;
    hipEvent_t ev_done = nullptr;
    static constexpr int RING = 8;
    static constexpr size_t TABLE_BYTES = 16384;
    char* pinned = nullptr;
    hipEvent_t ring_ev[RING] = {};
    unsigned ring_next = 0;
    struct Timed { hipEvent_t e0, e1; int kind, rows, cin, cout, flags; };
    bool timing = false;
    std::vector<Timed> timed;
    size_t timed_used = 0;
};

struct PsScope {
    Ps::Timed* t = nullptr; hipStream_t st;
    PsScope(Ps* p, void* stream, int kind, int rows, int cin, int cout, int flags) : st((hipStream_t)stream) {
        if (!p->timing) return;
        if (p->timed_used == p->timed.size()) {
            Ps::Timed n{};
            if (hipEventCreate(&n.e0) != hipSuccess || hipEventCreate(&n.e1) != hipSuccess) return;
            p->timed.push_back(n);
        }
        t = &p->timed[p->timed_used++];
        t->kind = kind; t->rows = rows; t->cin = cin; t->cout = cout; t->flags = flags;
        (void)hipEventRecord(t->e0, st);
    }
    ~PsScope() { if (t) (void)hipEventRecord(t->e1, st); }
};

inline int lin_index(int layer, int which) { return layer * LIN_PER_LAYER + which; }

void build_layout(Ps* p, int R)
{
    Layout& y = p->lay;
    if (y.R == R) return;
    y = Layout();
    y.R = R;
    size_t off = 0;
    auto take = [&](size_t bytes) { const size_t o = off; off += al(bytes); return o; };
    const size_t r = (size_t)R;
    y.allx = take(NL * r * E * 4);
    y.stf = take(NL * r * 2 * 4);
    y.dec_in = take(NL * r * E * 2);
    y.q = take(NL * r * E * 2);
    y.k = take(NL * r * E * 2);
    y.corr_lse = take(NL * r * 4);
    for (int i = 0; i < NLIN; ++i) {
        const Lin& l = p->lin[i];
        const int rows = i < NL * LIN_PER_LAYER ? R : NL * R;
        y.wg_bytes[i] = dreg_conv3d_wgrad_workspace_bytes(rows, 1, 1, 1, l.cin, l.cout, 1, 0);
        const size_t k1 = dreg_conv3d_igemm_workspace_bytes(rows, 1, 1, 1, l.cin, 1, 1, 1, l.cout, 1, 1, 0, 0, 0, 0);
        const size_t k2 = dreg_conv3d_igemm_workspace_bytes(rows, 1, 1, 1, l.cout, 1, 1, 1, l.cin, 1, 1, 0, 1, 0, 0);
        if (k1 > y.ks_bytes) y.ks_bytes = k1;
        if (k2 > y.ks_bytes) y.ks_bytes = k2;
    }
    const size_t lnp = dreg_layernorm_bwd_workspace_bytes(R), lnpf = dreg_layernorm_bwd_workspace_bytes(NL * R);
    for (int l = 0; l < NL; ++l) {
        LayerBuf& b = y.L[l];
        b.xa = take(r * E * 4); b.xb = take(r * E * 4);
        b.st1 = take(r * 8); b.st2 = take(r * 8); b.st3 = take(r * 8);
        b.h1 = take(r * E * 2); b.h2 = take(r * E * 2); b.h3 = take(r * E * 2);
        b.qkv1 = take(r * E3 * 2); b.qkv2 = take(r * E3 * 2);
        b.o1 = take(r * E * 2); b.o2 = take(r * E * 2);
        b.lse1 = take(NH * r * 4); b.lse2 = take(NH * r * 4);
        b.f = take(r * FF * 2);
        b.gF = take(r * FF * 2); b.gB = take(r * E * 2); b.gQ2 = take(r * E3 * 2); b.gC = take(r * E * 2); b.gQ1 = take(r * E3 * 2);
        for (int w = 0; w < LIN_PER_LAYER; ++w) {
            b.wg[w] = take(y.wg_bytes[lin_index(l, w)]);
            b.cs[w] = take(dreg_colsum_workspace_bytes(r, p->lin[lin_index(l, w)].cout));
        }
        for (int k = 0; k < 3; ++k) b.lnp[k] = take(lnp);
    }
    y.dallx = take(NL * r * E * 4);
    y.dallx_bf = take(NL * r * E * 2);
    y.dq = take(NL * r * E * 2); y.dk = take(NL * r * E * 2);
    y.ddec = take(NL * r * E * 2); y.ddec2 = take(NL * r * E * 2);
    y.dH = take(r * E * 2); y.dO = take(r * FF * 2);
    y.dvec = take((size_t)NL * r * 4 > NH * r * 4 ? NL * r * 4 : NH * r * 4);
    y.gx[0] = take(r * E * 4); y.gx[1] = take(r * E * 4);
    y.lnpf[0] = take(lnpf); y.lnpf[1] = take(lnpf);
    y.wgq = take(y.wg_bytes[NLIN - 2]); y.wgk = take(y.wg_bytes[NLIN - 1]);
    y.csq = take(dreg_colsum_workspace_bytes(NL * r, E)); y.csk = take(dreg_colsum_workspace_bytes(NL * r, E));
    y.ov_ws = take(dreg_overlap_bwd_workspace_bytes(NL * R));
    y.ks_ws = take(y.ks_bytes);
    y.cs_ws = take(dreg_colsum_workspace_bytes(NL * r, FF));
    y.tables = take(Ps::TABLE_BYTES);
    y.total = off + 256;
}

#define CK(expr) do { int rc_ = (expr); if (rc_) return rc_; } while (0)

int linear_fwd(Ps* p, const Layout& y, char* A, const void* x, const void* wpk, const float* bias, const void* residual, void* out,
               int rows, int cin, int cout, int relu, int out_f32, void* st)
{
    PsScope sc(p, st, 0, rows, cin, cout, (residual ? 1 : 0) | (out_f32 ? 2 : 0) | (y.ks_bytes ? 4 : 0));
    return dreg_conv3d_igemm_ws(x, wpk, out, bias, residual, rows, 1, 1, 1, cin, 1, 1, 1, cout, 1, 1, 0, 0, relu, residual ? 1 : 0, residual ? 1 : 0,
                                residual ? 1 : 0, residual ? 1 : 0, 0, out_f32, y.ks_bytes ? A + y.ks_ws : nullptr, y.ks_bytes, st);
}
int linear_dgrad(Ps* p, const Layout& y, char* A, const void* g, const void* wpk_t, void* gx, const void* mask, const void* add,
                 int rows, int cin, int cout, void* st)
{
    const void* addend = mask ? mask : add;
    PsScope sc(p, st, 1, rows, cin, cout, (addend ? 1 : 0) | (y.ks_bytes ? 4 : 0));
    return dreg_conv3d_igemm_ws(g, wpk_t, gx, nullptr, addend, rows, 1, 1, 1, cout, 1, 1, 1, cin, 1, 1, 0, 1, mask ? 2 : 0, addend ? 1 : 0, addend ? 1 : 0,
                                addend ? 1 : 0, addend ? 1 : 0, 0, 0, y.ks_bytes ? A + y.ks_ws : nullptr, y.ks_bytes, st);
}

}

extern "C" {

int dreg_ps_num_params(void) { return PS_NPARAM; }
int dreg_ps_num_linears(void) { return NLIN; }

void* dreg_ps_create(const int64_t* params)
{
    Ps* p = new Ps();
    for (int i = 0; i < PS_NPARAM; ++i) { p->val[i] = (float*)params[2 * i]; p->grad[i] = (float*)params[2 * i + 1]; }
    for (int l = 0; l < NL; ++l) {
        const int o = l * PL_COUNT;
        p->lin[lin_index(l, LIN_SI)] = {E3, E, o + SIW, o + SIB};
        p->lin[lin_index(l, LIN_SO)] = {E, E, o + SOW, o + SOB};
        p->lin[lin_index(l, LIN_CI)] = {E3, E, o + CIW, o + CIB};
        p->lin[lin_index(l, LIN_CO)] = {E, E, o + COW, o + COB};
        p->lin[lin_index(l, LIN_1)] = {FF, E, o + L1W, o + L1B};
        p->lin[lin_index(l, LIN_2)] = {E, FF, o + L2W, o + L2B};
    }
    p->lin[NLIN - 2] = {E, E, QW, QB};
    p->lin[NLIN - 1] = {E, E, KW, KB};
    if (hipHostMalloc((void**)&p->pinned, Ps::RING * Ps::TABLE_BYTES, hipHostMallocDefault) != hipSuccess) { delete p; return nullptr; }
    return p;
}
void dreg_ps_destroy(void* h)
{
    Ps* p = (Ps*)h;
    if (!p) return;
    for (auto& e : p->ev) if (e) (void)hipEventDestroy(e);
    if (p->ev_done) (void)hipEventDestroy(p->ev_done);
    for (auto& e : p->ring_ev) if (e) (void)hipEventDestroy(e);
    for (auto& t : p->timed) { (void)hipEventDestroy(t.e0); (void)hipEventDestroy(t.e1); }
    if (p->pinned) (void)hipHostFree(p->pinned);
    delete p;
}
void dreg_ps_set_fuse(void* h, int fuse) { ((Ps*)h)->fuse = fuse ? 1 : 0; ((Ps*)h)->panel = fuse >= 3 ? 2 : fuse >= 2 ? 1 : 0; }
void dreg_ps_set_group_wgrad(void* h, int on) { ((Ps*)h)->group_wgrad = on ? 1 : 0; }
void dreg_ps_set_timing(void* h, int enable) { ((Ps*)h)->timing = enable != 0; }
int dreg_ps_read_timings(void* h, int* info, float* ms, int cap)
{
    Ps* p = (Ps*)h;
    int n = 0;
    for (size_t i = 0; i < p->timed_used && n < cap; ++i) {
        const Ps::Timed& t = p->timed[i];
        float v = 0.f;
        if (hipEventElapsedTime(&v, t.e0, t.e1) != hipSuccess) continue;
        info[5 * n] = t.kind; info[5 * n + 1] = t.rows; info[5 * n + 2] = t.cin; info[5 * n + 3] = t.cout; info[5 * n + 4] = t.flags;
        ms[n++] = v;
    }
    p->timed_used = 0;
    return n;
}
size_t dreg_ps_arena_bytes(void* h, int R) { Ps* p = (Ps*)h; build_layout(p, R); return p->lay.total; }

int dreg_ps_forward(void* h, void* arena, size_t arena_bytes, const int64_t* packs, const float* feats, const float* xyz, const float* pe,
                    const int* probs_self, const int* probs_cross, int nprob, int max_len, int R,
                    float* cond, float* corr, float* ov, void* stream)
{
    Ps* p = (Ps*)h;
    if (R <= 0) return DREG_EINVAL;
    build_layout(p, R);
    const Layout& y = p->lay;
    if (arena_bytes < y.total) return DREG_EINVAL;
    char* A = (char*)arena;
    const float sc = 0.17677669529663687f;
    auto pk = [&](int li, int t) { return (const void*)packs[2 * li + t]; };
    const float* xin = feats;
    const bool panel = p->fuse && p->panel;
    auto chain = [&](const void* a1, int li1, int b1, const float* res, float* x, int nw, int nb, const float* pe_, void* hh, float* stt, int li2, int b2,
                     void* out2, int k1, int n2, int relu) {
        PsScope sc(p, stream, 3, R, k1, n2, 0);
        return dreg_ps_panel_fwd(a1, pk(li1, 0), p->val[b1], res, x, p->val[nw], p->val[nb], pe_, hh, stt, pk(li2, 0), p->val[b2], out2, R, k1, n2, relu, 1e-5f, stream);
    };
    for (int l = 0; l < NL; ++l) {
        const LayerBuf& b = y.L[l];
        const int o = l * PL_COUNT;
        float* xout = (float*)(A + y.allx) + (size_t)l * R * E;
        if (l == 0 || !panel) {
            CK(dreg_layernorm_fwd(xin, p->val[o + N1W], p->val[o + N1B], pe, A + b.h1, (float*)(A + b.st1), R, E, 1e-5f, 0, stream));
            CK(linear_fwd(p, y, A, A + b.h1, pk(lin_index(l, LIN_SI), 0), p->val[o + SIB], nullptr, A + b.qkv1, R, E, E3, 0, 0, stream));
        }
        CK(dreg_mha_varlen_fwd(A + b.qkv1, A + b.qkv1 + E * 2, A + b.qkv1 + 2 * E * 2, A + b.o1, (float*)(A + b.lse1), probs_self, nprob, max_len, max_len,
                               R, NH, E3, E3, E3, E, sc, 0, stream));
        if (panel) {
            CK(chain(A + b.o1, lin_index(l, LIN_SO), o + SOB, xin, (float*)(A + b.xa), o + N2W, o + N2B, pe, A + b.h2, (float*)(A + b.st2),
                     lin_index(l, LIN_CI), o + CIB, A + b.qkv2, E, E3, 0));
        } else {
            CK(linear_fwd(p, y, A, A + b.o1, pk(lin_index(l, LIN_SO), 0), p->val[o + SOB], xin, A + b.xa, R, E, E, 0, 1, stream));
            CK(dreg_layernorm_fwd((const float*)(A + b.xa), p->val[o + N2W], p->val[o + N2B], pe, A + b.h2, (float*)(A + b.st2), R, E, 1e-5f, 0, stream));
            CK(linear_fwd(p, y, A, A + b.h2, pk(lin_index(l, LIN_CI), 0), p->val[o + CIB], nullptr, A + b.qkv2, R, E, E3, 0, 0, stream));
// ... 7 lines not shown
            CK(linear_fwd(p, y, A, A + b.o2, pk(lin_index(l, LIN_CO), 0), p->val[o + COB], A + b.xa, A + b.xb, R, E, E, 0, 1, stream));
            CK(dreg_layernorm_fwd((const float*)(A + b.xb), p->val[o + N3W], p->val[o + N3B], nullptr, A + b.h3, (float*)(A + b.st3), R, E, 1e-5f, 0, stream));
            CK(linear_fwd(p, y, A, A + b.h3, pk(lin_index(l, LIN_1), 0), p->val[o + L1B], nullptr, A + b.f, R, E, FF, 1, 0, stream));
        }
        if (panel && l + 1 < NL) {
            const LayerBuf& nb = y.L[l + 1];
            const int no = o + PL_COUNT;
            CK(chain(A + b.f, lin_index(l, LIN_2), o + L2B, (const float*)(A + b.xb), xout, no + N1W, no + N1B, pe, A + nb.h1, (float*)(A + nb.st1),
                     lin_index(l + 1, LIN_SI), no + SIB, A + nb.qkv1, FF, E3, 0));
        } else {
            CK(linear_fwd(p, y, A, A + b.f, pk(lin_index(l, LIN_2), 0), p->val[o + L2B], A + b.xb, xout, R, FF, E, 0, 1, stream));
        }
        xin = xout;
    }
    const int R6 = NL * R;
    CK(dreg_layernorm_fwd2((const float*)(A + y.allx), p->val[FNW], p->val[FNB], pe, R, cond, A + y.dec_in, (float*)(A + y.stf), R6, E, 1e-5f, stream));
    CK(linear_fwd(p, y, A, A + y.dec_in, pk(NLIN - 2, 0), p->val[QB], nullptr, A + y.q, R6, E, E, 0, 0, stream));
    CK(linear_fwd(p, y, A, A + y.dec_in, pk(NLIN - 1, 0), p->val[KB], nullptr, A + y.k, R6, E, E, 0, 0, stream));
    CK(dreg_corr_attention_varlen_fwd(A + y.q, A + y.k, xyz, corr, (float*)(A + y.corr_lse), probs_cross, nprob, max_len, max_len, NL, R, 0.0625f, 0, stream));
    CK(dreg_overlap_fwd(cond, p->val[CW], p->val[CB], ov, R6, stream));
    return DREG_OK;
}

int dreg_ps_backward(void* h, void* arena, size_t arena_bytes, const int64_t* packs, const float* feats, const float* xyz, const float* pe,
                     const int* probs_self, const int* probs_cross, int nprob, int max_len, int R,
                     const float* cond, const float* corr, const float* ov, const float* g_cond, const float* g_corr, const float* g_ov,
                     float* d_feats, void* stream, void* aux_stream, int last_only)
{
    Ps* p = (Ps*)h;
    if (R <= 0 || R != p->lay.R) return DREG_EINVAL;
    const Layout& y = p->lay;
    if (arena_bytes < y.total) return DREG_EINVAL;
    for (int i = 0; i < PS_NPARAM; ++i) if (!p->grad[i]) return DREG_EINVAL;
    char* A = (char*)arena;
    hipStream_t st = (hipStream_t)stream;
    hipStream_t ax = aux_stream && aux_stream != stream ? (hipStream_t)aux_stream : st;
    const bool two = ax != st;
    const float sc = 0.17677669529663687f;
    const int LB = last_only ? NL - 1 : 0, nlb = last_only ? 1 : NL;
    const int R6 = nlb * R;
    const size_t rb = (size_t)LB * R;
    const int fuse = p->fuse;
    auto pk = [&](int li, int t) { return (const void*)packs[2 * li + t]; };
    cond += rb * E; corr += rb * 3; ov += rb;
    if (p->ev.size() < (size_t)NLIN + 2) {
        p->ev.resize(NLIN + 2, nullptr);
        for (auto& e : p->ev) if (!e && hipEventCreateWithFlags(&e, hipEventDisableTiming) != hipSuccess) return DREG_ELAUNCH;
        if (hipEventCreateWithFlags(&p->ev_done, hipEventDisableTiming) != hipSuccess) return DREG_ELAUNCH;
    }
    std::vector<ReduceRec> rd;
    std::vector<ColsumRec> cs;
    std::vector<LnRec> ln;
    int rd_blocks = 0, cs_p = 0, cs_f = 0;
    struct GroupRec { char d[160]; int variant, nblocks; };
    std::vector<GroupRec> grp;
    const bool group = fuse && p->group_wgrad && !p->timing;
    const bool panel = fuse && p->panel >= 2;
    auto panel_bwd = [&](const void* g1, const void* w1t, const float* x, const float* stt, const float* gamma, const float* add, const float* add2, float* dx, void* dx_bf,
                         float* part, const void* w2t, void* out2, int k1, int n2) {
        PsScope sc(p, stream, 4, R, k1, n2, 0);
        return dreg_ps_panel_bwd(g1, w1t, x, stt, gamma, add, add2, dx, dx_bf, part, w2t, out2, R, k1, n2, stream);
    };
    auto param_grads = [&](int li, const void* g, const void* x, int rows, size_t wg_off, size_t cs_off) -> int {
        const Lin& l = p->lin[li];
        bool grouped = false;
        if (group) {
            GroupRec gr{};
            if (dreg_linear_wgrad_group_fill(gr.d, g, x, A + wg_off, y.wg_bytes[li], rows, l.cin, l.cout, &gr.variant, &gr.nblocks) == DREG_OK) { grp.push_back(gr); grouped = true; }
        }
        if (!grouped) {
            if (two) { if (hipEventRecord(p->ev[li], st) != hipSuccess || hipStreamWaitEvent(ax, p->ev[li], 0) != hipSuccess) return DREG_ELAUNCH; }
            PsScope sc(p, ax, 2, rows, l.cin, l.cout, 0);
            CK(dreg_conv3d_wgrad_partials(g, x, A + wg_off, y.wg_bytes[li], nullptr, 0, rows, 1, 1, 1, l.cin, l.cin, 1, 1, 1, l.cout, 1, 1, 0, nullptr, ax));
        }
        ReduceRec r{};
        r.part = (const float*)(A + wg_off); r.dw = p->grad[l.w];
        r.nsplit = dreg_conv3d_wgrad_splits(rows, 1, 1, 1, l.cin, l.cout, 1, 0);
        r.Cout = l.cout; r.Kpad = dreg_conv3d_kpad(1, l.cin, 0); r.ntaps = 1; r.Cin = l.cin; r.Cin_real = l.cin; r.accumulate = 1; r.block0 = rd_blocks;
        rd_blocks += dreg_wgrad_reduce_blocks(l.cout, l.cin, 1, r.nsplit);
        rd.push_back(r);
        if (!fuse) return dreg_colsum(g, p->grad[l.b], (float*)(A + y.cs_ws), (size_t)rows, l.cout, 1, 0, ax);
        ColsumRec c{};
        c.g = g; c.out = p->grad[l.b]; c.partial = (float*)(A + cs_off); c.M = rows; c.C = l.cout;
        c.rpc = dreg_colsum_rows_per_chunk((size_t)rows); c.nch = (rows + c.rpc - 1) / c.rpc; c.pblock0 = cs_p; c.fblock0 = cs_f; c.accumulate = 1;
        cs_p += c.nch; cs_f += (l.cout + 3) / 4;
        cs.push_back(c);
        return DREG_OK;
    };
    auto ln_rec = [&](size_t part_off, int wi, int bi, int rows) {
        LnRec r{(const float*)(A + part_off), p->grad[wi], p->grad[bi], dreg_layernorm_bwd_blocks(rows), 1};
        ln.push_back(r);
    };

    const float* Gcond = g_cond;
    if (g_ov) {
        CK(dreg_overlap_bwd_acc(cond, p->val[CW], ov, g_ov, (float*)(A + y.dallx) + rb * E, g_cond, p->grad[CW], p->grad[CB], 1, (float*)(A + y.ov_ws), R6, stream));
        Gcond = (const float*)(A + y.dallx) + rb * E;
    }
    bool have_dec = false;
    if (g_corr) {
        const size_t ob = rb * E * 2;
        CK(dreg_corr_attention_varlen_bwd(A + y.q + ob, A + y.k + ob, xyz, corr, g_corr, (const float*)(A + y.corr_lse) + rb, (float*)(A + y.dvec), A + y.dq + ob, A + y.dk + ob,
                                          probs_cross, nprob, max_len, max_len, nlb, R, 0.0625f, 0, stream));
        CK(param_grads(NLIN - 1, A + y.dk + ob, A + y.dec_in + ob, R6, y.wgk, y.csk));
        CK(param_grads(NLIN - 2, A + y.dq + ob, A + y.dec_in + ob, R6, y.wgq, y.csq));
        CK(linear_dgrad(p, y, A, A + y.dk + ob, pk(NLIN - 1, 1), A + y.ddec + ob, nullptr, nullptr, R6, E, E, stream));
        if (fuse) CK(linear_dgrad(p, y, A, A + y.dq + ob, pk(NLIN - 2, 1), A + y.ddec + ob, nullptr, A + y.ddec + ob, R6, E, E, stream));
        else {
            CK(linear_dgrad(p, y, A, A + y.dq + ob, pk(NLIN - 2, 1), A + y.ddec2 + ob, nullptr, nullptr, R6, E, E, stream));
            CK(dreg_add_inplace(A + y.ddec + ob, A + y.ddec2 + ob, (size_t)R6 * E, 0, stream));
        }
        have_dec = true;
    }
    float* dallx = (float*)(A + y.dallx);
    const float* allx = (const float*)(A + y.allx);
    {
        const float* ax = allx + rb * E;
        const float* stf = (const float*)(A + y.stf) + rb * 2;
        float* dg = dallx + rb * E;
        char* dgb = A + y.dallx_bf + rb * E * 2;
        const char* dd = A + y.ddec + rb * E * 2;
    if (Gcond && have_dec && fuse) {
        CK(dreg_layernorm_bwd_parts(ax, Gcond, dd, p->val[FNW], stf, dg, nullptr, nullptr, dgb, (float*)(A + y.lnpf[0]), R6, E, 1, stream));
        ln_rec(y.lnpf[0], FNW, FNB, R6);
    } else if (Gcond || have_dec) {
        bool first = true;
        if (Gcond) {
            CK(dreg_layernorm_bwd_parts(ax, Gcond, nullptr, p->val[FNW], stf, dg, nullptr, nullptr, have_dec ? nullptr : dgb, (float*)(A + y.lnpf[0]), R6, E, 1, stream));
            ln_rec(y.lnpf[0], FNW, FNB, R6);
            first = false;
        }
        if (have_dec) {
            CK(dreg_layernorm_bwd_parts(ax, dd, nullptr, p->val[FNW], stf, dg, first ? nullptr : dg, nullptr, dgb, (float*)(A + y.lnpf[1]), R6, E, 0, stream));
// ... 26 lines not shown
        CK(linear_dgrad(p, y, A, A + b.gF, pk(lin_index(l, LIN_1), 1), A + y.dH, nullptr, nullptr, R, E, FF, stream));
        CK(param_grads(lin_index(l, LIN_1), A + b.gF, A + b.h3, R, b.wg[LIN_1], b.cs[LIN_1]));
        CK(dreg_layernorm_bwd_parts((const float*)(A + b.xb), A + y.dH, nullptr, p->val[o + N3W], (const float*)(A + b.st3), Gb, G, nullptr, A + b.gB,
                                    (float*)(A + b.lnp[2]), R, E, 0, stream));
        ln_rec(b.lnp[2], o + N3W, o + N3B, R);
        CK(linear_dgrad(p, y, A, A + b.gB, pk(lin_index(l, LIN_CO), 1), A + y.dO, nullptr, nullptr, R, E, E, stream));
        }
        CK(param_grads(lin_index(l, LIN_CO), A + b.gB, A + b.o2, R, b.wg[LIN_CO], b.cs[LIN_CO]));
        CK(dreg_mha_varlen_bwd(A + b.qkv2, A + b.qkv2 + E * 2, A + b.qkv2 + 2 * E * 2, A + b.o2, A + y.dO, (const float*)(A + b.lse2), (float*)(A + y.dvec),
                               A + b.gQ2, A + b.gQ2 + E * 2, A + b.gQ2 + 2 * E * 2, probs_cross, nprob, max_len, max_len, R, NH, E3, E3, E3, E, sc, 0, stream));
        float* Ga = (float*)(A + y.gx[1]);
        if (panel) {
            CK(panel_bwd(A + b.gQ2, pk(lin_index(l, LIN_CI), 1), (const float*)(A + b.xa), (const float*)(A + b.st2), p->val[o + N2W], Gb, nullptr, Ga, A + b.gC,
                                 (float*)(A + b.lnp[1]), pk(lin_index(l, LIN_SO), 1), A + y.dO, E3, E));
            CK(param_grads(lin_index(l, LIN_CI), A + b.gQ2, A + b.h2, R, b.wg[LIN_CI], b.cs[LIN_CI]));
            ln_rec(b.lnp[1], o + N2W, o + N2B, R);
        } else {
        CK(linear_dgrad(p, y, A, A + b.gQ2, pk(lin_index(l, LIN_CI), 1), A + y.dH, nullptr, nullptr, R, E, E3, stream));
        CK(param_grads(lin_index(l, LIN_CI), A + b.gQ2, A + b.h2, R, b.wg[LIN_CI], b.cs[LIN_CI]));
        CK(dreg_layernorm_bwd_parts((const float*)(A + b.xa), A + y.dH, nullptr, p->val[o + N2W], (const float*)(A + b.st2), Ga, Gb, nullptr, A + b.gC,
                                    (float*)(A + b.lnp[1]), R, E, 0, stream));
        ln_rec(b.lnp[1], o + N2W, o + N2B, R);
        CK(linear_dgrad(p, y, A, A + b.gC, pk(lin_index(l, LIN_SO), 1), A + y.dO, nullptr, nullptr, R, E, E, stream));
        }
        CK(param_grads(lin_index(l, LIN_SO), A + b.gC, A + b.o1, R, b.wg[LIN_SO], b.cs[LIN_SO]));
        CK(dreg_mha_varlen_bwd(A + b.qkv1, A + b.qkv1 + E * 2, A + b.qkv1 + 2 * E * 2, A + b.o1, A + y.dO, (const float*)(A + b.lse1), (float*)(A + y.dvec),
                               A + b.gQ1, A + b.gQ1 + E * 2, A + b.gQ1 + 2 * E * 2, probs_self, nprob, max_len, max_len, R, NH, E3, E3, E3, E, sc, 0, stream));
        if (!panel) CK(linear_dgrad(p, y, A, A + b.gQ1, pk(lin_index(l, LIN_SI), 1), A + y.dH, nullptr, nullptr, R, E, E3, stream));
        CK(param_grads(lin_index(l, LIN_SI), A + b.gQ1, A + b.h1, R, b.wg[LIN_SI], b.cs[LIN_SI]));
        if (panel) {
            float* Gprev = l == 0 ? d_feats : dallx + (size_t)(l - 1) * R * E;
            void* Gprev_bf = l == 0 ? nullptr : A + y.dallx_bf + (size_t)(l - 1) * R * E * 2;
            CK(panel_bwd(A + b.gQ1, pk(lin_index(l, LIN_SI), 1), xin, (const float*)(A + b.st1), p->val[o + N1W], Ga, (l == 0 || last_only) ? nullptr : Gprev, Gprev,
                                 Gprev_bf, (float*)(A + b.lnp[0]), nullptr, nullptr, E3, 0));
            if (l > 0) { G = Gprev; Gbf = Gprev_bf; }
        } else if (l == 0) {
            CK(dreg_layernorm_bwd_parts(xin, A + y.dH, nullptr, p->val[o + N1W], (const float*)(A + b.st1), d_feats, Ga, nullptr, nullptr,
                                        (float*)(A + b.lnp[0]), R, E, 0, stream));
        } else {
            float* Gprev = dallx + (size_t)(l - 1) * R * E;
            void* Gprev_bf = A + y.dallx_bf + (size_t)(l - 1) * R * E * 2;
            CK(dreg_layernorm_bwd_parts(xin, A + y.dH, nullptr, p->val[o + N1W], (const float*)(A + b.st1), Gprev, Ga, last_only ? nullptr : Gprev, Gprev_bf,
                                        (float*)(A + b.lnp[0]), R, E, 0, stream));
            G = Gprev; Gbf = Gprev_bf;
        }
        ln_rec(b.lnp[0], o + N1W, o + N1B, R);
    }

    const size_t nb_rd = rd.size() * sizeof(ReduceRec), nb_cs = cs.size() * sizeof(ColsumRec), nb_ln = ln.size() * sizeof(LnRec);
    const size_t o_cs = al(nb_rd), o_ln = o_cs + al(nb_cs);
    const int gd = dreg_wgrad_group_desc_bytes();
    std::stable_sort(grp.begin(), grp.end(), [](const GroupRec& a, const GroupRec& b) { return a.variant < b.variant; });
    const size_t o_grp = al(o_ln + nb_ln), nb_grp = grp.size() * (size_t)gd;
    if (gd > 160 || o_grp + nb_grp > Ps::TABLE_BYTES) return DREG_EINVAL;
    if (o_ln + nb_ln > Ps::TABLE_BYTES) return DREG_EINVAL;
    const unsigned slot = p->ring_next++ % Ps::RING;
    if (!p->ring_ev[slot]) { if (hipEventCreateWithFlags(&p->ring_ev[slot], hipEventDisableTiming) != hipSuccess) return DREG_ELAUNCH; }
    else if (hipEventSynchronize(p->ring_ev[slot]) != hipSuccess) return DREG_ELAUNCH;
    char* host = p->pinned + (size_t)slot * Ps::TABLE_BYTES;
    std::memcpy(host, rd.data(), nb_rd);
    std::memcpy(host + o_cs, cs.data(), nb_cs);
    std::memcpy(host + o_ln, ln.data(), nb_ln);
    struct GroupLaunch { size_t off; int n, variant, blocks; };
    std::vector<GroupLaunch> gl;
    for (size_t i = 0; i < grp.size(); ++i) {
        if (gl.empty() || gl.back().variant != grp[i].variant) gl.push_back(GroupLaunch{o_grp + i * (size_t)gd, 0, grp[i].variant, 0});
        const int b0 = gl.back().blocks;
        std::memcpy(grp[i].d + gd - (int)sizeof(int), &b0, sizeof(int));
        std::memcpy(host + o_grp + i * (size_t)gd, grp[i].d, (size_t)gd);
        gl.back().n += 1; gl.back().blocks += grp[i].nblocks;
    }
    if (hipMemcpyAsync(A + y.tables, host, grp.empty() ? o_ln + nb_ln : o_grp + nb_grp, hipMemcpyHostToDevice, st) != hipSuccess) return DREG_ELAUNCH;
    if (hipEventRecord(p->ring_ev[slot], st) != hipSuccess) return DREG_ELAUNCH;
    if (two && hipStreamWaitEvent(ax, p->ring_ev[slot], 0) != hipSuccess) return DREG_ELAUNCH;
    const int ln_dup = (ln.size() >= 2 && ln[0].dg == ln[1].dg) ? 1 : 0;
    if (ln_dup) CK(dreg_layernorm_bwd_final_batched(A + y.tables + o_ln, 1, stream));
    CK(dreg_layernorm_bwd_final_batched(A + y.tables + o_ln + ln_dup * sizeof(LnRec), (int)ln.size() - ln_dup, stream));
    for (const GroupLaunch& q : gl) CK(dreg_wgrad_group_launch(A + y.tables + q.off, q.n, q.variant, q.blocks, ax));
    CK(dreg_wgrad_reduce_batched(A + y.tables, (int)rd.size(), 0, rd_blocks, ax));
    if (fuse) CK(dreg_colsum_batched(A + y.tables + o_cs, (int)cs.size(), cs_p, cs_f, ax));
    return DREG_OK;
}

}
```

dreg_nerf_amd/lib.py:

```python
import ctypes
import os
from ctypes import c_float, c_int, c_size_t, c_void_p

import torch

_HERE = os.path.dirname(os.path.abspath(__file__))
LIB_PATH = os.path.join(_HERE, "libdreg_nerf_hip.so")

DT_BF16 = 0
DT_F32 = 1

_lib = None


class DregError(RuntimeError):
    pass


def _sig(lib, name, restype, argtypes):
    fn = getattr(lib, name)
    fn.restype = restype
    fn.argtypes = argtypes
    return fn

# ... 6 lines not shown
    "dreg_conv3d_igemm_ws": (I, [P, P, P, P, P] + [I] * 18 + [I, I, P, Z, P]),
    "dreg_conv3d_igemm_occ": (I, [P, P, P, P, P] + [I] * 18 + [I, I, P, Z, P, P]),
    "dreg_conv3d_igemm_bnstats": (I, [P, P, P, P, P] + [I] * 17 + [P, Z, P, P, P]),
    "dreg_conv3d_kpad": (I, [I, I, I]),
    "dreg_gemm_f32_desc_bytes": (I, []),
    "dreg_gemm_f32_batched": (I, [P, I, I, P, P]),
    "dreg_infonce_wsym": (I, [P, P, I, P]),
    "dreg_conv3d_igemm_defer": (I, [P, P, P, P, P] + [I] * 18 + [P, Z, P, P, P, P]),
    "dreg_bn3d_fwd_ex": (I, [P] * 10 + [I, I, I, F, F, I, I, I, P, P, I, P, P]),
    "dreg_bn3d_bwd_ex": (I, [P] * 11 + [I] * 6 + [P, P, P, P]),
    "dreg_exec_default_opts": (None, [P]),
    "dreg_exec_guard_bands": (I, [P]),
    "dreg_exec_guard_check": (I, [P, P, P, P]),
    "dreg_exec_guard_describe": (I, [P, I, P, I]),
    "dreg_exec_guard_last": (I, [P, P, P, P]),
    "dreg_guard_fill": (I, [P, P, I, I, P]),
    "dreg_guard_scan": (I, [P, P, I, I, P, P]),
    "dreg_exec_create_opts": (P, [P, I, P, I, P, I, P]),
    "dreg_ps_set_group_wgrad": (None, [P, I]),
    "dreg_conv_get_glds": (I, []),
    "dreg_conv3d_dgrad_s2": (I, [P, P, P] + [I] * 11 + [P]),
    "dreg_conv3d_dgrad_s2_acc": (I, [P, P, P] + [I] * 11 + [P]),
    "dreg_pack_conv_weight": (I, [P, P, I, I, I, I, I, I, P]),
    "dreg_pack_conv_weights_batched": (I, [P, I, I, I, P, P]),
    "dreg_conv3d_wgrad_splits": (I, [I] * 8),
    "dreg_conv3d_wgrad_workspace_bytes": (Z, [I] * 8),
    "dreg_conv3d_wgrad": (I, [P, P, P, P, Z] + [I] * 16 + [P]),
    "dreg_conv3d_wgrad_occ": (I, [P, P, P, P, Z] + [I] * 16 + [P, P]),
    "dreg_conv3d_igemm_rows": (I, [P] * 5 + [P, I] + [I] * 18 + [I, P]),
    "dreg_conv3d_wgrad_rows": (I, [P, P, P, P, Z] + [P, I] + [I] * 14 + [P]),
    "dreg_conv3d_wgrad_partials": (I, [P, P, P, Z, P, I] + [I] * 13 + [P, P]),
    "dreg_wgrad_reduce_blocks": (I, [I, I, I, I]),
    "dreg_wgrad_reduce_batched": (I, [P, I, I, I, P]),
    "dreg_conv3_halo_supported": (I, [I] * 6),
    "dreg_conv3_halo_use": (I, [I] * 9),
    "dreg_conv3_halo_pack_bytes": (Z, [I]),
    "dreg_pack_conv_weight_halo": (I, [P, P, I, I, I, P]),
    "dreg_conv3_halo": (I, [P, P, P, P, P] + [I] * 10 + [P]),
    "dreg_conv3_halo_pack_bytes_n": (Z, [I, I]),
    "dreg_conv3_halo_n": (I, [P, P, P, P, P] + [I] * 11 + [P]),
    "dreg_conv3_halo_n_bnstats": (I, [P, P, P, P, P] + [I] * 10 + [P, P, P]),
    "dreg_conv1_stream_variant": (I, [I, I]),
    "dreg_conv1_stream_supported": (I, [I] * 14),
    "dreg_conv1_stream_use": (I, [I] * 14),
    "dreg_conv1_stream": (I, [P, P, P, P, P] + [I] * 20 + [P, Z, P, I]),
    "dreg_conv1_stream_bnstats": (I, [P, P, P, P, P] + [I] * 17 + [P, Z, P, P, P, I]),
    "dreg_conv3d_wgrad_variant": (I, [I] * 10),
    "dreg_conv3d_igemm_variant": (I, [I] * 17),
    "dreg_conv3d_wgrad_group_fill": (I, [P, P, P, P, Z] + [I] * 12 + [P, P]),
    "dreg_bn_small_in_regs": (I, [I, I, I, I]),
    "dreg_wgrad_group_desc_bytes": (I, []),
    "dreg_linear_wgrad_group_fill": (I, [P, P, P, P, Z, I, I, I, P, P]),
    "dreg_wgrad_group_launch": (I, [P, I, I, I, P]),
    "dreg_bn_num_chunks": (I, [I]),
    "dreg_bn_relu_maxpool_fwd": (I, [P] * 10 + [I] * 8 + [F, F, I, I, P]),
    "dreg_bn_relu_maxpool_bwd": (I, [P] * 10 + [I] * 10 + [P]),
    "dreg_sparse_stem_workspace_floats": (Z, [I] * 5),
    "dreg_sparse_stem_fwd": (I, [P, P, I, P, I] + [P] * 12 + [I] * 8 + [F, F, I, I, P]),
    "dreg_sparse_stem_bwd": (I, [P] * 6 + [I, P, I] + [P] * 7 + [I] * 10 + [P]),
    "dreg_bn3d_fwd": (I, [P] * 10 + [I, I, I, F, F, I, I, I, P]),
    "dreg_bn3d_bwd": (I, [P] * 11 + [I, I, I, I, I, I, P]),
    "dreg_bn_small": (I, [I, I, I, I]),
    "dreg_bn3d_fwd_defer_update": (I, [P] * 10 + [I, I, I, F, F, I, I, I, P, P, P]),
    "dreg_bn3d_fwd_from_sums": (I, [P] * 10 + [I, I, I, I, F, F, I, I, P]),
    "dreg_bn3d_bwd_defer_params": (I, [P] * 11 + [I, I, I, I, I, I, P, P, P]),
    "dreg_bn_running_update_batched": (I, [P, I, I, I, F, P]),
    "dreg_bn_param_grad_batched": (I, [P, I, I, I, I, P]),
    "dreg_bn_self_coef_supported": (I, [I, I, I, I]),
    "dreg_bn_self_coef_use": (I, [I, I, I, I, I]),
    "dreg_bn_self_coef_rows": (I, [I, I, I, I]),
    "dreg_bn3d_fwd_self_coef": (I, [P, P, P, P, P, P, P, P, I, I, I, I, F, I, I, P, P, P]),
    "dreg_bn3d_bwd_self_coef": (I, [P, P, P, P, P, P, P, P, I, I, I, I, I, P, P]),
    "dreg_maxpool3d_fwd": (I, [P, P, P] + [I] * 9 + [P]),
    "dreg_maxpool3d_bwd": (I, [P, P, P] + [I] * 9 + [P]),
    "dreg_maxpool3d_bwd_acc": (I, [P, P, P] + [I] * 10 + [P]),
    "dreg_downsample_sum": (I, [P, P] + [I] * 9 + [P]),
    "dreg_downsample_sum_rows": (I, [P, P, P] + [I] * 9 + [P]),
    "dreg_colsum_workspace_bytes": (Z, [Z, I]),
    "dreg_colsum": (I, [P, P, P, Z, I, I, I, P]),
    "dreg_trilinear_gather_fwd": (I, [P, P, P, P] + [I] * 10 + [P]),
    "dreg_trilinear_gather_bwd": (I, [P, P, P, P] + [I] * 8 + [P]),
    "dreg_cast_from_f32": (I, [P, P, Z, I, P]),
    "dreg_fill_zero": (I, [P, Z, P]),
    "dreg_active_sets_workspace_bytes": (Z, [I] * 4),
    "dreg_active_sets": (I, [P, P] + [I] * 8 + [P, P, P, P, Z, P]),
    "dreg_active_sets_level2_workspace_bytes": (Z, [I] * 4),
    "dreg_active_sets_level2": (I, [P] + [I] * 7 + [P, P, P, Z, P]),
    "dreg_conv_rows_workspace_bytes": (Z, [I, I, I, I]),
    "dreg_conv_rows": (I, [P, P, I, I, I, I, I, I, I, I, I, I, I, P, P, P, Z, P]),
    "dreg_trilinear_gather_bwd_rows": (I, [P, P, P, P, I, P, P, P] + [I] * 10 + [P]),
    "dreg_colsum_rows": (I, [P, P, I, P, P, I, I, I, P]),
    "dreg_trilinear_gather_bwd_gather": (I, [P, P, P, P, I, P, P] + [I] * 10 + [P]),
    "dreg_trilinear_gather_bwd_gather_rows_only": (I, [P, P, P, P, I, P, P] + [I] * 10 + [P]),
    "dreg_trilinear_gather_bwd_gather_seg": (I, [P, P, P, P, P, I, P, P] + [I] * 11 + [P]),
    "dreg_gather_segment_mean": (I, [P, P, P, I, P, P, P, P] + [I] * 9 + [P]),
    "dreg_zero_rows": (I, [P, P, I, I, I, P]),
    "dreg_add_inplace": (I, [P, P, Z, I, P]),
    "dreg_pack_rgba_grids": (I, [P, P, I, I, I, I, I, P]),
    "dreg_pack_rgba_grids_occ": (I, [P, P, P, I, I, I, I, I, P]),
    "dreg_pack_rgba_sparse": (I, [P, P, P, P, I, I, I, I, I, I, P]),
    "dreg_pack_rgba_sparse_occ": (I, [P, P, P, P, P, I, I, I, I, I, I, P]),
    "dreg_conv_row_occupancy": (I, [P, P, I, I, I, I, I, I, I, I, P]),
    "dreg_gather_grid_xyz": (I, [P, P, P, P, I, I, I, I, P]),
    "dreg_exec_create": (P, [P, I, P, I, P, I]),
    "dreg_exec_destroy": (None, [P]),
    "dreg_exec_op_halo": (I, [P, I]),
# ... 136 lines not shown
    "dreg_scene_voxel_grid": (I, [I, I, I, P, P, I, P, F, F, F, P, P, P, P]),
}


PROBE_SIGNATURES = {
    "dreg_conv1_bnrelu_a_probe": (I, [P, P, P, P, I, I, I, I, I, I, P]),
    "dreg_conv_set_glds": (None, [I]),
    "dreg_conv_set_wgrad_splits": (None, [I]),
    "dreg_conv_set_wgrad_big": (None, [I]),
    "dreg_conv_igemm_probe": (None, [I]),
    "dreg_conv_set_igemm_ap": (None, [I]),
    "dreg_conv_set_igemm_ap256": (None, [I]),
    "dreg_conv_set_pointwise_rmw_cin": (None, [I]),
    "dreg_conv_igemm_probe_read": (I, [P]),
    "dreg_conv_set_wgrad_pipe": (None, [I]),
    "dreg_conv_wgrad_probe_read": (I, [P]),
    "dreg_conv_set_wgrad_ring": (None, [I]),
    "dreg_conv_set_wgrad_rows_fast": (None, [I]),
    "dreg_conv_set_row_splits": (None, [I]),
    "dreg_conv_set_glds_stages": (None, [I]),
    "dreg_conv_set_wgrad_target_blocks": (None, [I]),
    "dreg_conv_set_narrow_small": (None, [I]),
    "dreg_bn_set_debug_skip": (None, [I]),
    "dreg_bn_set_store_g": (None, [I]),
    "dreg_bn_set_small_regs": (None, [I]),
    "dreg_sstem_set_pool_blocks": (None, [I]),
    "dreg_voxel_set_own_sort": (None, [I]),
    "dreg_conv_set_bn_stats_epilogue": (None, [I]),
    "dreg_conv3_halo_set_variant": (None, [I]),
    "dreg_conv3_halo64_set": (None, [I]),
    "dreg_conv3_halo_set_prof": (None, [P]),
    "dreg_bn_set_small_max_voxels": (None, [I]),
    "dreg_bn_set_self_wgs": (None, [I]),
    "dreg_ngp_set_rgb_chunks": (None, [I]),
    "dreg_ngp_set_density_unroll": (None, [I]),
    "dreg_ngp_set_xcd_levels": (None, [I]),
    "dreg_visibility_set_waves": (None, [I]),
    "dreg_visibility_set_pass_bound": (I, [ctypes.c_long]),
    "dreg_render_set_waves": (None, [I]),
    "dreg_render_pair_set_waves": (None, [I]),
    "dreg_render_bwd_set_waves": (None, [I]),
    "dreg_render_scene_set_waves": (None, [I]),
    "dreg_points_bwd_set_waves": (None, [I]),
    "dreg_render_samples_set_waves": (None, [I]),
    "dreg_scene_grid_set_waves": (None, [I]),
    "dreg_scene_grid_set_lanes_z": (None, [I]),
}
PROBE_LIB_PATH = os.path.join(_HERE, "libdreg_nerf_hip_probe.so")
_probe_lib = None


class ExecOpts(ctypes.Structure):
    _fields_ = [(n, c_int) for n in ("sparse_grads", "bn_batch_tails", "fuse_stem", "sparse_stem", "fold_res_bn", "fold_splitk", "group_wgrad",
                                     "s2_accumulate", "fuse_bn_stats", "brick", "defer_head_pg", "persistent_deep", "guard", "pointwise_stream", "bn_self_coef")] + [("reserved", c_int * 1)]


SCENE_MAX_BLOCKS = 4


class SceneBlock(ctypes.Structure):
    _fields_ = ([("origins", P), ("viewdirs", P), ("binary", P), ("rx", c_int), ("ry", c_int), ("rz", c_int), ("coarse_bits", P)] +
                [(n, P) for n in ("table", "w1", "w2", "cw1", "cw2", "cw3", "offset", "size", "res", "scale", "hashed", "roi_aabb", "scene_aabb", "model_aabb")] +
                [(n, c_float) for n in ("near_plane", "far_plane", "render_step_size", "alpha_thre")] + [("center", P)])


class FieldBlock(ctypes.Structure):
    _fields_ = ([("binary", P), ("rx", c_int), ("ry", c_int), ("rz", c_int)] +
                [(n, P) for n in ("table", "w1", "w2", "offset", "size", "res", "scale", "hashed", "roi_aabb", "model_aabb", "center", "pose")])


class RadianceBlock(ctypes.Structure):
    _fields_ = [("field", FieldBlock)] + [(n, P) for n in ("cw1", "cw2", "cw3", "dirbias")]


class IcpBlock(ctypes.Structure):
    _fields_ = [("src", P), ("n", c_int), ("tgt_points", P), ("tgt_normals", P), ("cell_start", P), ("grid_lo", c_float * 3), ("cell", c_float),
                ("nx", c_int), ("ny", c_int), ("nz", c_int)]


def load_probe():
    global _probe_lib
    if _probe_lib is None:
        if not os.path.exists(PROBE_LIB_PATH):
            raise DregError(f"{PROBE_LIB_PATH} not found: build it with `python -m dreg_nerf_amd.build`")
        lib = ctypes.CDLL(PROBE_LIB_PATH)
        for name, (rt, at) in list(SIGNATURES.items()) + list(PROBE_SIGNATURES.items()):
            _sig(lib, name, rt, at)
        _probe_lib = lib
    return _probe_lib


def use_probe():
    global _lib
    _lib = load_probe()
    return _lib


class probe:

    def __init__(self):
        self._restore = []

    def __enter__(self):
        global _lib
        self._saved = _lib
        _lib = load_probe()
        self.lib = _lib
# ... 97 lines not shown
```

dreg_nerf_amd/ops.py:

```python
import os
from typing import Optional

import numpy as np
import torch

from . import lib as L


def _ws(nbytes: int, device) -> torch.Tensor:
    return torch.empty(max(int(nbytes), 16), dtype=torch.uint8, device=device)


class KernelTimer:

    def __init__(self):
        self.entries = []
        self.measured = []
        self._overhead = None
        self.enabled = True

    def record(self, name, label, flops):
        if not self.enabled:
            return None
        start = torch.cuda.Event(enable_timing=True)
# ... 236 lines not shown
    L.check(lib.dreg_pack_conv_weight_halo(L.ptr(w.detach().contiguous()), L.ptr(out), cout, cin, int(transposed), L.stream()), "dreg_pack_conv_weight_halo")
    if len(_halo_cache) > 64:
        for k in [k for k, v in _halo_cache.items() if v[0]() is None]:
            del _halo_cache[k]
    _halo_cache[key] = (weakref.ref(base), stamp, out)
    return out


def halo_applies(x_shape, cin, cout, ksz, stride, pad, dt) -> bool:
    return dt == L.DT_BF16 and bool(L.load().dreg_conv3_halo_use(x_shape[0], x_shape[1], x_shape[2], x_shape[3], cin, cout, ksz, stride, pad))


def conv_halo(x, w, bias, addend, transposed: bool, add_same: bool = False, out_f32: bool = False):
    lib = L.load()
    B, D, H, W, C = x.shape
    n = w.shape[1] if transposed else w.shape[0]
    out = torch.empty(B, D, H, W, n, dtype=torch.float32 if out_f32 else torch.bfloat16, device=x.device)
    Da = Ha = Wa = 0
    if addend is not None:
        assert addend.dtype == out.dtype and addend.shape[0] == B and addend.shape[4] == n
        Da, Ha, Wa = addend.shape[1:4]
    ev = None
    if PROFILER is not None:
        label = f"{'dgrad' if transposed else 'fwd'} B{B} {D}x{H}x{W}x{C}->{D}x{H}x{W}x{n} k3s1"
        ev = PROFILER.record("conv3_halo64_kernel<bf16>" if n == 64 else "conv3_halo_kernel<bf16>", label, 2.0 * B * D * H * W * n * 27 * C)
        if ev is not None:
            ev[0].record()
    L.check(lib.dreg_conv3_halo_n(L.ptr(x), L.ptr(halo_packed_weight(w, transposed)), L.ptr(out), L.ptr(bias), L.ptr(addend), B, D, H, W, C, n,
                                  Da, Ha, Wa, int(add_same), int(out_f32), L.stream()), "dreg_conv3_halo_n")
    if ev is not None:
        ev[1].record()
    return out


def conv_dgrad_s2(g, wpk_class, x_shape, cout, ksz, pad):
    lib = L.load()
    B, Di, Hi, Wi, cin = x_shape
    Do, Ho, Wo = g.shape[1:4]
    gx = torch.empty(x_shape, dtype=g.dtype, device=g.device)
    ev = None
    if PROFILER is not None:
        ev = PROFILER.record("conv_igemm_glds_kernel<bf16,s2-dgrad>", f"dgrad-s2 B{B} {Do}x{Ho}x{Wo}x{cout}->{Di}x{Hi}x{Wi}x{cin} k{ksz}s2",
                             2.0 * B * Do * Ho * Wo * cout * (ksz ** 3) * cin)
        if ev is not None:
            ev[0].record()
    L.check(lib.dreg_conv3d_dgrad_s2(L.ptr(g), L.ptr(wpk_class), L.ptr(gx), B, Di, Hi, Wi, cin, Do, Ho, Wo, cout, ksz, pad, L.stream()),
            "dreg_conv3d_dgrad_s2")
    if ev is not None:
        ev[1].record()
    return gx


_PENDING_REDUCE = []
_REDUCE_DT = np.dtype([("part", "<u8"), ("dw", "<u8"), ("nsplit", "<i4"), ("Cout", "<i4"), ("Kpad", "<i4"), ("ntaps", "<i4"),
                       ("Cin", "<i4"), ("Cin_real", "<i4"), ("accumulate", "<i4"), ("block0", "<i4")])


def flush_wgrad_reduce():
    if not _PENDING_REDUCE:
        return
    lib = L.load()
    rounds = []
    for rec in _PENDING_REDUCE:
        key = rec[1].data_ptr()
        for seen, lst in rounds:
            if key not in seen:
                seen.add(key); lst.append(rec)
                break
        else:
            rounds.append(({key}, [rec]))
    dev = _PENDING_REDUCE[0][0].device
    st = torch.cuda.current_stream(dev)
    for _, lst in rounds:
        recs = np.zeros(len(lst), dtype=_REDUCE_DT)
        blocks = 0
        for i, (ws, dw, nsplit, cout, kpad, ntaps, cin, cin_real, ksz) in enumerate(lst):
            recs[i] = (ws.data_ptr(), dw.data_ptr(), nsplit, cout, kpad, ntaps, cin, cin_real, 1, blocks)
            blocks += lib.dreg_wgrad_reduce_blocks(cout, cin_real, ksz, nsplit)
        table = torch.from_numpy(recs.view(np.uint8)).pin_memory().to(dev, non_blocking=True)
        L.check(lib.dreg_wgrad_reduce_batched(L.ptr(table), len(lst), 0, blocks, L.stream()), "dreg_wgrad_reduce_batched")
        table.record_stream(st)
    for ws, *_ in _PENDING_REDUCE:
        ws.record_stream(st)
    _PENDING_REDUCE.clear()


def conv_wgrad(gout, x, w_shape, cin_pad, ksz, stride, pad, use_tr=True, accumulate_into=None, defer=False):
    lib = L.load()
    dt = L.dt_of(x)
    B, Di, Hi, Wi = x.shape[:4]
    Do, Ho, Wo, cout = gout.shape[1:]
    cin_real = w_shape[1]
    nbytes = lib.dreg_conv3d_wgrad_workspace_bytes(B, Do, Ho, Wo, cin_pad, cout, ksz, dt)
    ws = _ws(nbytes, x.device)
    if defer and accumulate_into is not None and dt == L.DT_BF16 and use_tr and accumulate_into.is_contiguous():
        L.check(lib.dreg_conv3d_wgrad_partials(L.ptr(gout), L.ptr(x), L.ptr(ws), nbytes, None, 0, B, Di, Hi, Wi, cin_pad, cin_real,
                                               Do, Ho, Wo, cout, ksz, stride, pad, None, L.stream()), "dreg_conv3d_wgrad_partials")
        _PENDING_REDUCE.append((ws, accumulate_into, lib.dreg_conv3d_wgrad_splits(B, Do, Ho, Wo, cin_pad, cout, ksz, dt), cout,
                                lib.dreg_conv3d_kpad(ksz, cin_pad, dt), ksz ** 3, cin_pad, cin_real, ksz))
        return None
    dw = accumulate_into if accumulate_into is not None else torch.empty(w_shape, dtype=torch.float32, device=x.device)
    ev = None
    if PROFILER is not None:
        tn = "bf16" if dt == L.DT_BF16 else "f32"
        label = f"wgrad B{B} {Di}x{Hi}x{Wi}x{cin_pad} g{Do}x{Ho}x{Wo}x{cout} k{ksz}s{stride}"
        if dt == L.DT_BF16 and use_tr:
            wname = wgrad_kernel_name(lib, B, Do, Ho, Wo, cin_pad, cout, ksz) + "+reduce"
        else:
# ... 514 lines not shown
```

dreg_nerf_amd/pointset_exec.py:

```python
import ctypes
from typing import Dict, Optional

import numpy as np
import torch

from . import lib as L
from . import ops

N_LAYERS = 6
_PER_LAYER = ("norm1.weight", "norm1.bias", "self_attn.in_proj_weight", "self_attn.in_proj_bias", "self_attn.out_proj.weight",
              "self_attn.out_proj.bias", "norm2.weight", "norm2.bias", "cross_attn.in_proj_weight", "cross_attn.in_proj_bias",
              "cross_attn.out_proj.weight", "cross_attn.out_proj.bias", "norm3.weight", "norm3.bias", "linear1.weight", "linear1.bias",
              "linear2.weight", "linear2.bias")
_TAIL = ("transformer_encoder.norm.weight", "transformer_encoder.norm.bias", "correspondence_decoder.q_proj.weight",
         "correspondence_decoder.q_proj.bias", "correspondence_decoder.k_proj.weight", "correspondence_decoder.k_proj.bias",
         "correspondence_decoder.conf_logits_decoder.weight", "correspondence_decoder.conf_logits_decoder.bias")
_LINEARS = ("self_attn.in_proj_weight", "self_attn.out_proj.weight", "cross_attn.in_proj_weight", "cross_attn.out_proj.weight",
            "linear1.weight", "linear2.weight")

FUSE = True
PANEL = 3
GROUP_WGRAD = True


def _fuse_level() -> int:
    return 0 if not FUSE else int(PANEL)


def param_names():
    names = [f"transformer_encoder.layers.{l}.{n}" for l in range(N_LAYERS) for n in _PER_LAYER]
    return names + list(_TAIL)


def linear_names():
    names = [f"transformer_encoder.layers.{l}.{n}" for l in range(N_LAYERS) for n in _LINEARS]
    return names + ["correspondence_decoder.q_proj.weight", "correspondence_decoder.k_proj.weight"]


class PointSetExecutor:

    def __init__(self, P: Dict[str, torch.Tensor], with_grad: bool):
        self.lib = L.load()
        names = param_names()
        assert len(names) == self.lib.dreg_ps_num_params()
        self.params = [P[n] for n in names]
        self.linears = [P[n] for n in linear_names()]
        assert len(self.linears) == self.lib.dreg_ps_num_linears()
        self.with_grad = with_grad
        tab = np.zeros((len(names), 2), dtype=np.int64)
        self._sig = []
        for i, t in enumerate(self.params):
            assert t.is_contiguous() and t.dtype == torch.float32, "the executor reads fp32 master parameters in place"
            g = t.grad if with_grad else None
            if with_grad and (g is None or not g.is_contiguous() or g.dtype != torch.float32):
                raise L.DregError("PointSetExecutor needs preallocated contiguous fp32 .grad buffers (FlatAdamW) on every parameter")
            tab[i, 0] = t.data_ptr()
            tab[i, 1] = g.data_ptr() if g is not None else 0
            self._sig.append((t.data_ptr(), int(tab[i, 1])))
        self.h = self.lib.dreg_ps_create(tab.ctypes.data)
        if not self.h:
            raise L.DregError("dreg_ps_create failed")
        self.lib.dreg_ps_set_fuse(self.h, _fuse_level())
        self.lib.dreg_ps_set_group_wgrad(self.h, int(GROUP_WGRAD))
        self._fuse = _fuse_level()
        self._group = GROUP_WGRAD
        self.device = self.params[0].device
        self.arena = None
        self.arena_bytes = 0
        self._timing = False
        self._packs = (ctypes.c_int64 * (2 * len(self.linears)))()
        self._pack_stamp = None
        self._pack_keep = None

    def __del__(self):
        try:
            if getattr(self, "h", None):
                self.lib.dreg_ps_destroy(self.h)
                self.h = None
        except Exception:
            pass

    def still_valid(self) -> bool:
        for t, (vp, gp) in zip(self.params, self._sig):
            g = t.grad if self.with_grad else None
            if t.data_ptr() != vp or (g.data_ptr() if g is not None else 0) != gp:
                return False
        return True

    def _pack_table(self):
        stamp = (ops._weight_generation, sum(t._version for t in self.linears))
        if stamp != self._pack_stamp:
            keep = []
            for i, w in enumerate(self.linears):
                f = ops.packed_weight(w, w.shape[1], False, L.DT_BF16)
                d = ops.packed_weight(w, w.shape[1], True, L.DT_BF16)
                self._packs[2 * i], self._packs[2 * i + 1] = f.data_ptr(), d.data_ptr()
                keep += [f, d]
            self._pack_keep, self._pack_stamp = keep, stamp
        return ctypes.addressof(self._packs)

    def _arena_for(self, R: int):
        need = self.lib.dreg_ps_arena_bytes(self.h, R)
        if need > self.arena_bytes:
            self.arena = None
            self.arena_bytes = int(need * 1.25)
            self.arena = torch.empty(self.arena_bytes, dtype=torch.uint8, device=self.device)
        return self.arena

    def set_timing(self, on: bool):
        self._timing = bool(on)
        self.lib.dreg_ps_set_timing(self.h, int(on))

    def drain_timings(self, profiler: "ops.KernelTimer"):
        cap = 4096
        info = (ctypes.c_int * (5 * cap))()
        ms = (ctypes.c_float * cap)()
        n = self.lib.dreg_ps_read_timings(self.h, info, ms, cap)
        for i in range(n):
            kind, rows, cin, cout, flags = (info[5 * i + k] for k in range(5))
            fl = 2.0 * rows * cin * cout
            if kind in (3, 4):
                fl = 2.0 * rows * 256 * (cin + cout)
                name = f"ps_panel_kernel<{'true' if kind == 4 else 'false'}>"
                label = f"panel {'bwd' if kind == 4 else 'fwd'} B{rows} {cin}->256->{cout}"
            elif kind == 2:
                name = ops.wgrad_kernel_name(self.lib, rows, 1, 1, 1, cin, cout, 1)
                label = f"wgrad B{rows} 1x1x1x{cin} g1x1x1x{cout} k1s1"
            elif kind == 1:
                name = ops.igemm_kernel_name(self.lib, rows, 1, 1, 1, cout, 1, 1, 1, cin, 1, 1, 0, 1, 0, bool(flags & 4), bool(flags & 1), L.DT_BF16, False)
                label = f"dgrad B{rows} 1x1x1x{cout}->1x1x1x{cin} k1s1"
            else:
                name = ops.igemm_kernel_name(self.lib, rows, 1, 1, 1, cin, 1, 1, 1, cout, 1, 1, 0, 0, 0, bool(flags & 4), bool(flags & 1), L.DT_BF16, bool(flags & 2))
                label = f"fwd B{rows} 1x1x1x{cin}->1x1x1x{cout} k1s1"
            profiler.add_measured(name, label, fl, ms[i])

    def forward(self, feats, xyz, pe, tab):
        if self._fuse != _fuse_level():
            self._fuse = _fuse_level()
            self.lib.dreg_ps_set_fuse(self.h, self._fuse)
        if self._group != GROUP_WGRAD:
            self.lib.dreg_ps_set_group_wgrad(self.h, int(GROUP_WGRAD))
            self._group = GROUP_WGRAD
        want = ops.PROFILER is not None and ops.PROFILER.enabled
        if want != self._timing:
            self.set_timing(want)
        ops.wait_packs()
        R = feats.shape[0]
        arena = self._arena_for(R)
        dev = feats.device
        cond = torch.empty(N_LAYERS, R, 256, dtype=torch.float32, device=dev)
        corr = torch.empty(N_LAYERS, R, 3, dtype=torch.float32, device=dev)
        ov = torch.empty(N_LAYERS, R, 1, dtype=torch.float32, device=dev)
        L.check(self.lib.dreg_ps_forward(self.h, L.ptr(arena), self.arena_bytes, self._pack_table(), L.ptr(feats), L.ptr(xyz), L.ptr(pe),
                                         L.ptr(tab.self_probs), L.ptr(tab.cross_probs), tab.nprob, tab.max_len, R,
                                         L.ptr(cond), L.ptr(corr), L.ptr(ov), L.stream()), "dreg_ps_forward")
        self.generation = getattr(self, "generation", 0) + 1
        return cond, corr, ov

    def backward(self, feats, xyz, pe, tab, cond, corr, ov, g_cond, g_corr, g_ov, last_only=False, generation=None):
        if generation is not None and generation != getattr(self, "generation", 0):
            raise L.DregError("PointSetExecutor.backward: the shared arena was overwritten by a later forward pass (two grad-mode forwards before a "
                              "backward: gradient accumulation over several forwards / retain_graph need one executor per live graph)")
        R = feats.shape[0]
        d_feats = torch.empty_like(feats)
        aux = None if self._timing else ops.PARAM_GRAD_STREAM
        if aux is not None:
            self.arena.record_stream(aux)
        L.check(self.lib.dreg_ps_backward(self.h, L.ptr(self.arena), self.arena_bytes, self._pack_table(), L.ptr(feats), L.ptr(xyz), L.ptr(pe),
                                          L.ptr(tab.self_probs), L.ptr(tab.cross_probs), tab.nprob, tab.max_len, R,
                                          L.ptr(cond), L.ptr(corr), L.ptr(ov), L.ptr(g_cond), L.ptr(g_corr), L.ptr(g_ov), L.ptr(d_feats),
                                          L.stream(), aux.cuda_stream if aux is not None else None, int(last_only)), "dreg_ps_backward")
        return d_feats


class _PointSetFn(torch.autograd.Function):

    @staticmethod
    def forward(ctx, feats, anchor, ex: PointSetExecutor, xyz, pe, tab):
        cond, corr, ov = ex.forward(feats, xyz, pe, tab)
        ctx.ex, ctx.tab, ctx.generation = ex, tab, ex.generation
        ctx.save_for_backward(feats, xyz, pe, cond, corr, ov)
        ctx.set_materialize_grads(False)
        return cond, corr, ov, cond[-1].clone(), corr[-1].clone(), ov[-1].clone()

    @staticmethod
    def backward(ctx, g_cond, g_corr, g_ov, g_cl, g_rl, g_ol):
        feats, xyz, pe, cond, corr, ov = ctx.saved_tensors
        f32 = lambda g: g.contiguous().float() if g is not None else None
        if FUSE and g_cond is None and g_corr is None and g_ov is None:
            d_feats = ctx.ex.backward(feats, xyz, pe, ctx.tab, cond, corr, ov, f32(g_cl), f32(g_rl), f32(g_ol), last_only=True, generation=ctx.generation)
            return d_feats, None, None, None, None, None
        full = []
        for g, gl, ref in ((g_cond, g_cl, cond), (g_corr, g_rl, corr), (g_ov, g_ol, ov)):
            if gl is not None:
                g = torch.zeros_like(ref) if g is None else g.contiguous().float().clone()
# ... 30 lines not shown
```

include/dreg_nerf.h:

```cpp
#ifndef DREG_NERF_H
#define DREG_NERF_H
#include <stddef.h>
#include <stdint.h>

#ifdef __cplusplus
extern "C" {
#endif

#define DREG_OK 0
#define DREG_EINVAL (-1)

int dreg_conv_get_glds(void);


int dreg_conv3d_kpad(int ksz, int Cin, int dtype);

int dreg_pack_conv_weight(const float* w, void* out, int Cout, int Cin_real, int Cin, int ksz, int for_dgrad,
                          int dtype, void* stream);
int dreg_pack_conv_weights_batched(const void* descs, int n, int total_rows, int stage_floats, const int* row_desc,
                                   void* stream);

int dreg_conv3d_igemm(const void* in, const void* wt_packed, void* out, const float* bias, const void* addend,
                      int B, int Di, int Hi, int Wi, int Cin, int Do, int Ho, int Wo, int Cout,
                      int ksz, int stride, int pad, int transposed, int relu, int Da, int Ha, int Wa, int add_same,
// ... 22 lines not shown
size_t dreg_conv3_halo_pack_bytes(int Cin_reduced);
int dreg_pack_conv_weight_halo(const float* w, void* out, int Cout, int Cin, int transposed, void* stream);
int dreg_conv3_halo(const void* in, const void* wpk, void* out, const float* bias, const void* addend,
                    int B, int D, int H, int W, int Cin, int Da, int Ha, int Wa, int add_same, int out_f32, void* stream);
size_t dreg_conv3_halo_pack_bytes_n(int Cin_reduced, int rows);
int dreg_conv3_halo_n(const void* in, const void* wpk, void* out, const float* bias, const void* addend,
                      int B, int D, int H, int W, int Cin, int Cout, int Da, int Ha, int Wa, int add_same, int out_f32, void* stream);
int dreg_conv3_halo_n_bnstats(const void* in, const void* wpk, void* out, const float* bias, const void* addend,
                              int B, int D, int H, int W, int Cin, int Cout, int Da, int Ha, int Wa, int add_same, float* bn_partial, int* rows_per_chunk, void* stream);

int dreg_conv1_stream_variant(int Cin, int Cout);
int dreg_conv1_stream_supported(int B, int D, int H, int W, int Cin, int Cout, int ksz, int stride, int pad, int relu,
                                int has_addend, int add_same, int dtype, int nrows);
int dreg_conv1_stream_use(int B, int D, int H, int W, int Cin, int Cout, int ksz, int stride, int pad, int relu,
                          int has_addend, int add_same, int dtype, int nrows);
int dreg_conv1_stream(const void* in, const void* wt_packed, void* out, const float* bias, const void* addend,
                      int B, int Di, int Hi, int Wi, int Cin, int Do, int Ho, int Wo, int Cout,
                      int ksz, int stride, int pad, int transposed, int relu, int Da, int Ha, int Wa, int add_same,
                      int dtype, int out_f32, void* workspace, size_t workspace_bytes, void* stream, int max_blocks);
int dreg_conv1_stream_bnstats(const void* in, const void* wt_packed, void* out, const float* bias, const void* addend,
                              int B, int Di, int Hi, int Wi, int Cin, int Do, int Ho, int Wo, int Cout,
                              int ksz, int stride, int pad, int relu, int Da, int Ha, int Wa, int add_same,
                              void* workspace, size_t workspace_bytes, float* bn_partial, int* rows_per_chunk, void* stream, int max_blocks);

int dreg_conv3d_dgrad_s2(const void* gout, const void* wt_class_packed, void* din, int B, int Di, int Hi, int Wi, int Cin,
                         int Do, int Ho, int Wo, int Cout, int ksz, int pad, void* stream);
int dreg_conv3d_dgrad_s2_acc(const void* gout, const void* wt_class_packed, void* din, int B, int Di, int Hi, int Wi, int Cin,
                             int Do, int Ho, int Wo, int Cout, int ksz, int pad, void* stream);

int dreg_conv3d_igemm_variant(int B, int Di, int Hi, int Wi, int Cin, int Do, int Ho, int Wo, int Cout, int ksz, int stride, int pad,
                              int transposed, int nrows, int has_ws, int has_addend, int dtype);
int dreg_conv3d_wgrad_variant(int B, int Do, int Ho, int Wo, int Cin, int Cout, int ksz, int rows, int nrows, int occ);
int dreg_conv3d_wgrad_splits(int B, int Do, int Ho, int Wo, int Cin, int Cout, int ksz, int dtype);
size_t dreg_conv3d_wgrad_workspace_bytes(int B, int Do, int Ho, int Wo, int Cin, int Cout, int ksz, int dtype);
int dreg_conv3d_wgrad(const void* gout, const void* in, float* dw, void* workspace, size_t workspace_bytes,
                      int B, int Di, int Hi, int Wi, int Cin, int Cin_real, int Do, int Ho, int Wo, int Cout,
                      int ksz, int stride, int pad, int accumulate, int dtype, int use_tr, void* stream);
int dreg_conv3d_wgrad_occ(const void* gout, const void* in, float* dw, void* workspace, size_t workspace_bytes,
                          int B, int Di, int Hi, int Wi, int Cin, int Cin_real, int Do, int Ho, int Wo, int Cout,
                          int ksz, int stride, int pad, int accumulate, int dtype, int use_tr, const uint8_t* rowocc, void* stream);

int dreg_conv3d_igemm_rows(const void* in, const void* wt_packed, void* out, const float* bias, const void* addend,
                           const int* rows, int nrows,
                           int B, int Di, int Hi, int Wi, int Cin, int Do, int Ho, int Wo, int Cout,
                           int ksz, int stride, int pad, int transposed, int relu, int Da, int Ha, int Wa, int add_same,
                           int out_f32, void* stream);
int dreg_conv3d_wgrad_rows(const void* gout, const void* in, float* dw, void* workspace, size_t workspace_bytes,
                           const int* rows, int nrows,
                           int B, int Di, int Hi, int Wi, int Cin, int Cin_real, int Do, int Ho, int Wo, int Cout,
                           int ksz, int stride, int pad, int accumulate, void* stream);
int dreg_conv3d_wgrad_partials(const void* gout, const void* in, void* workspace, size_t workspace_bytes, const int* rows, int nrows,
                               int B, int Di, int Hi, int Wi, int Cin, int Cin_real, int Do, int Ho, int Wo, int Cout,
                               int ksz, int stride, int pad, const uint8_t* rowocc, void* stream);
int dreg_wgrad_reduce_blocks(int Cout, int Cin_real, int ksz, int nsplit);
int dreg_wgrad_reduce_batched(const void* descs_dev, int n, int block_base, int nblocks, void* stream);
int dreg_wgrad_group_desc_bytes(void);
int dreg_linear_wgrad_group_fill(void* desc_host, const void* gout, const void* in, void* workspace, size_t workspace_bytes,
                                 int rows, int Cin, int Cout, int* variant, int* nblocks);
int dreg_conv3d_wgrad_group_fill(void* desc_host, const void* gout, const void* in, void* workspace, size_t workspace_bytes,
                                 int B, int Di, int Hi, int Wi, int Cin, int Do, int Ho, int Wo, int Cout, int ksz, int stride, int pad,
                                 int* variant, int* nblocks);
int dreg_wgrad_group_launch(const void* descs_dev, int n, int variant, int total_blocks, void* stream);

int dreg_bn_num_chunks(int V);
int dreg_bn3d_fwd(const void* x, const void* res, void* y, const float* gamma, const float* beta,
                  float* running_mean, float* running_var, float* scale_shift, float* mean_rstd, float* workspace,
                  int B, int V, int C, float eps, float momentum, int train, int relu, int dtype, void* stream);
int dreg_bn3d_bwd(const void* x, const void* dy, const void* y, const float* scale_shift, const float* mean_rstd,
                  void* dx, void* dres, float* dgamma, float* dbeta, float* coef, float* workspace,
                  int B, int V, int C, int relu, int accumulate, int dtype, void* stream);
int dreg_bn_small(int B, int V, int C, int dtype);
int dreg_bn3d_fwd_defer_update(const void* x, const void* res, void* y, const float* gamma, const float* beta,
                               float* running_mean, float* running_var, float* scale_shift, float* mean_rstd, float* workspace,
                               int B, int V, int C, float eps, float momentum, int train, int relu, int dtype, float* var_keep, int* deferred, void* stream);
int dreg_bn3d_bwd_defer_params(const void* x, const void* dy, const void* y, const float* scale_shift, const float* mean_rstd,
                               void* dx, void* dres, float* dgamma, float* dbeta, float* coef, float* workspace,
                               int B, int V, int C, int relu, int accumulate, int dtype, float* sums_keep, int* deferred, void* stream);
typedef struct dreg_bn_extra {
    const float* res_scale_shift;
    const float* splitk_part;
    int splitk_nsplit;
    size_t splitk_slice;
} dreg_bn_extra;
int dreg_bn3d_fwd_ex(const void* x, const void* res, void* y, const float* gamma, const float* beta,
                     float* running_mean, float* running_var, float* scale_shift, float* mean_rstd, float* workspace,
                     int B, int V, int C, float eps, float momentum, int train, int relu, int dtype, float* var_keep, int* deferred,
                     int sums_rows_per_chunk, const dreg_bn_extra* ex, void* stream);
int dreg_bn3d_bwd_ex(const void* x, const void* dy, const void* y, const float* scale_shift, const float* mean_rstd,
                     void* dx, void* dres, float* dgamma, float* dbeta, float* coef, float* workspace,
                     int B, int V, int C, int relu, int accumulate, int dtype, float* sums_keep, int* deferred, const dreg_bn_extra* ex, void* stream);
int dreg_conv3d_igemm_defer(const void* in, const void* wt_packed, void* out, const float* bias, const void* addend,
                            int B, int Di, int Hi, int Wi, int Cin, int Do, int Ho, int Wo, int Cout,
                            int ksz, int stride, int pad, int transposed, int relu, int Da, int Ha, int Wa, int add_same,
                            void* workspace, size_t workspace_bytes, const uint8_t* rowocc, int* sk_nsplit, size_t* sk_slice, void* stream);
int dreg_bn_small_in_regs(int B, int V, int C, int dtype);
int dreg_bn_running_update_batched(const void* descs_dev, int n, int block_base, int nblocks, float momentum, void* stream);
int dreg_bn_param_grad_batched(const void* descs_dev, int n, int block_base, int nblocks, int accumulate, void* stream);
int dreg_bn_self_coef_supported(int B, int V, int C, int dtype);
int dreg_bn_self_coef_use(int B, int V, int C, int dtype, int backward);
int dreg_bn_self_coef_rows(int B, int V, int C, int dtype);
int dreg_bn3d_fwd_self_coef(const void* x, const void* res, void* y, const float* gamma, const float* beta, float* scale_shift, float* mean_rstd,
                            float* sums, int rows_per_chunk, int B, int V, int C, float eps, int relu, int dtype, double* keep,
                            const float* res_scale_shift, void* stream);
int dreg_bn3d_bwd_self_coef(const void* x, const void* dy, const void* y, const float* scale_shift, const float* mean_rstd,
                            void* dx, void* dres, float* workspace, int B, int V, int C, int relu, int dtype, double* keep, void* stream);

// ... 40 lines not shown
int dreg_pack_rgba_grids_occ(const void* grids, void* out, uint8_t* inocc, int B, int Z, int X, int Y, int dtype, void* stream);
int dreg_pack_rgba_sparse(const float* vals, const int64_t* idx, const int* pt_batch, void* out, int N, int B, int Z, int X,
                          int Y, int dtype, void* stream);
int dreg_pack_rgba_sparse_occ(const float* vals, const int64_t* idx, const int* pt_batch, void* out, uint8_t* inocc, int N, int B, int Z, int X,
                              int Y, int dtype, void* stream);
int dreg_conv_row_occupancy(const uint8_t* inocc, uint8_t* rowocc, int B, int Di, int Hi, int Do, int Ho, int ksz, int stride, int pad, void* stream);
int dreg_gather_grid_xyz(const void* grids, const int64_t* idx, const int* pt_batch, float* xyz, int N, int Zr, int Xr, int Yr,
                         void* stream);

size_t dreg_active_sets_workspace_bytes(int B, int d, int h, int w);
int dreg_active_sets(const int64_t* idx, const int* pt_batch, int N, int B, int Zr, int Xr, int Yr, int d, int h, int w,
                     int* rows, int* counts, int* map1, void* workspace, size_t workspace_bytes, void* stream);
size_t dreg_active_sets_level2_workspace_bytes(int B, int d2, int h2, int w2);
int dreg_active_sets_level2(const uint8_t* child_flags, int B, int d, int h, int w, int d2, int h2, int w2, int* rows2,
                            int* counts2, void* workspace, size_t workspace_bytes, void* stream);
size_t dreg_conv_rows_workspace_bytes(int B, int d, int h, int w);
int dreg_conv_rows(const int64_t* idx, const int* pt_batch, int N, int B, int Zr, int Xr, int Yr, int d, int h, int w, int ksz, int stride, int pad,
                   int* rows, int* count, void* workspace, size_t workspace_bytes, void* stream);
int dreg_trilinear_gather_bwd_rows(const float* dfeat, const int64_t* idx, const int* pt_batch, const int* rows1, int n1,
                                   const int* map1, float* comp, void* dp1, int N, int B, int d, int h, int w, int C,
                                   int Zr, int Xr, int Yr, int dtype, void* stream);
int dreg_trilinear_gather_bwd_gather(const float* dfeat, const int64_t* idx, const int* pt_batch, const int* rows1, int n1,
                                     int* fine_map, void* dp1, int N, int B, int d, int h, int w, int C, int Zr, int Xr,
                                     int Yr, int dtype, void* stream);
int dreg_trilinear_gather_bwd_gather_rows_only(const float* dfeat, const int64_t* idx, const int* pt_batch, const int* rows1, int n1,
                                               int* fine_map, void* dp1, int N, int B, int d, int h, int w, int C, int Zr, int Xr, int Yr,
                                               int dtype, void* stream);
int dreg_trilinear_gather_bwd_gather_seg(const float* g1, const void* seg_descs, const int64_t* idx, const int* pt_batch, const int* rows1, int n1,
                                         int* fine_map, void* dp1, int N, int B, int d, int h, int w, int C, int Zr, int Xr, int Yr,
                                         int dtype, int zero_dense, void* stream);
int dreg_gather_segment_mean(const void* p1, const int64_t* idx, const int* pt_batch, int point_start, const uint32_t* order, const uint32_t* starts,
                             const int* n_out, float* out, int M, int d, int h, int w, int C, int Zr, int Xr, int Yr, int dtype, void* stream);
int dreg_zero_rows(void* buf, const int* rows, int nrows, int C, int dtype, void* stream);
int dreg_colsum_rows(const void* g, const int* rows, int nrows, float* out, float* workspace, int C, int accumulate,
                     int dtype, void* stream);

void* dreg_exec_create(const int* tensors, int nt, const int* ops, int nops, const int64_t* params, int np);
typedef struct dreg_exec_opts {
    int sparse_grads;
    int bn_batch_tails;
    int fuse_stem;
    int sparse_stem;
    int fold_res_bn;
    int fold_splitk;
    int group_wgrad;
    int s2_accumulate;
    int fuse_bn_stats;
    int brick;
    int defer_head_pg;
    int persistent_deep;
    int guard;
    int pointwise_stream;
    int bn_self_coef;
    int reserved[1];
} dreg_exec_opts;
void dreg_exec_default_opts(dreg_exec_opts* o);
void* dreg_exec_create_opts(const int* tensors, int nt, const int* ops, int nops, const int64_t* params, int np, const dreg_exec_opts* opts);
#define DREG_EGUARD (-3)
int dreg_exec_guard_bands(void* h);
int dreg_exec_guard_check(void* h, void* arena, long long* out4, void* stream);
int dreg_exec_guard_describe(void* h, int band, char* buf, int buf_bytes);
int dreg_exec_guard_last(void* h, int* op, int* pass, long long* band);
void dreg_exec_destroy(void* h);
size_t dreg_exec_arena_bytes(void* h);
size_t dreg_exec_pack_bytes(void* h);
int dreg_exec_num_packs(void* h);
size_t dreg_exec_tensor_offset(void* h, int slot);
int dreg_exec_output_slot(void* h);
int dreg_exec_pack_rows(void* h);
int dreg_exec_export_pack_table(void* h, void* host_out, int* host_row_desc, void* pack_base);
int dreg_exec_repack(void* h, const void* descs_dev, const int* row_desc_dev, void* stream);
int dreg_exec_op_halo(void* h, int op);
int dreg_exec_op_wgrad_grouped(void* h, int op);
int dreg_exec_op_bn_self_coef(void* h, int op);
int dreg_exec_op_pointwise(void* h, int op);
void dreg_exec_set_overlap(void* h, int enable);
void dreg_exec_set_input_row_occupancy(void* h, const uint8_t* rowocc);
void dreg_exec_set_timing(void* h, int enable);
int dreg_exec_read_timings(void* h, int* op_kind, float* ms, int max);
int dreg_exec_forward(void* h, void* arena, size_t arena_bytes, const void* pack_base, const void* x_in,
                      const int64_t* rowlists, int nlists, int train, void* stream);
int dreg_exec_backward(void* h, void* arena, size_t arena_bytes, const void* pack_base, const void* x_in,
                       const void* grad_out, const int64_t* rowlists, int nlists, void* stream, void* aux_stream);
int dreg_exec_backward_range(void* h, void* arena, size_t arena_bytes, const void* pack_base, const void* x_in, const void* grad_out,
                             const int64_t* rowlists, int nlists, void* stream, void* aux_stream, int op_begin, int op_end, int flags);

int dreg_mha_fwd(const void* q, const void* k, const void* v, void* o, float* lse, int Nq, int Nk, int H,
                 int ldq, int ldk, int ldv, int ldo, float scale, int dtype, void* stream);
int dreg_mha_bwd(const void* q, const void* k, const void* v, const void* o, const void* dout, const float* lse,
                 float* dvec, void* dq, void* dk, void* dv, int Nq, int Nk, int H,
                 int ldq, int ldk, int ldv, int ldo, float scale, int dtype, void* stream);
int dreg_corr_attention_fwd(const void* q, const void* k, const float* xyz, float* out, float* lse, int L, int Nq, int Nk,
                            float scale, int dtype, void* stream);
int dreg_corr_attention_bwd(const void* q, const void* k, const float* xyz, const float* out, const float* dout,
                            const float* lse, float* dvec, void* dq, void* dk, int L, int Nq, int Nk,
                            float scale, int dtype, void* stream);

int dreg_mha_varlen_fwd(const void* q, const void* k, const void* v, void* o, float* lse, const int* probs, int nprob,
                        int max_q, int max_k, int R, int H, int ldq, int ldk, int ldv, int ldo, float scale, int dtype, void* stream);
int dreg_mha_varlen_bwd(const void* q, const void* k, const void* v, const void* o, const void* dout, const float* lse,
                        float* dvec, void* dq, void* dk, void* dv, const int* probs, int nprob, int max_q, int max_k, int R, int H,
                        int ldq, int ldk, int ldv, int ldo, float scale, int dtype, void* stream);
int dreg_corr_attention_varlen_fwd(const void* q, const void* k, const float* xyz, float* out, float* lse, const int* probs, int nprob,
                                   int max_q, int max_k, int L, int R, float scale, int dtype, void* stream);
int dreg_corr_attention_varlen_bwd(const void* q, const void* k, const float* xyz, const float* out, const float* dout,
                                   const float* lse, float* dvec, void* dq, void* dk, const int* probs, int nprob,
                                   int max_q, int max_k, int L, int R, float scale, int dtype, void* stream);
// ... 250 lines not shown

int dreg_mc_table(signed char* tris, int* width);
size_t dreg_mc_workspace_bytes(int nx, int ny, int nz);
int dreg_mc_count(const float* values, int nx, int ny, int nz, float level, void* workspace, size_t workspace_bytes, int* counts, void* stream);
int dreg_mc_emit(const float* values, int nx, int ny, int nz, float level, const float* origin, const float* spacing, const void* workspace,
                 size_t workspace_bytes, float* verts, int* faces, int V, int F, void* stream);

int dreg_pair_density(const float* x, long n, const float* origin, const float* spacing, int nx, int ny, int nz,
                      const uint8_t* src_binary, int src_rx, int src_ry, int src_rz, const void* src_table, const void* src_w1, const void* src_w2,
                      const uint32_t* src_offset, const uint32_t* src_size, const uint32_t* src_res, const float* src_scale, const uint32_t* src_hashed,
                      const float* src_roi_aabb, const float* src_model_aabb, const float* src_center,
                      const uint8_t* tgt_binary, int tgt_rx, int tgt_ry, int tgt_rz, const void* tgt_table, const void* tgt_w1, const void* tgt_w2,
                      const uint32_t* tgt_offset, const uint32_t* tgt_size, const uint32_t* tgt_res, const float* tgt_scale, const uint32_t* tgt_hashed,
                      const float* tgt_roi_aabb, const float* tgt_model_aabb, const float* tgt_center,
                      const float* pose, float power, float* sigma, float* w_src, float* w_tgt, float* sigma_src, float* sigma_tgt, void* stream);

typedef struct dreg_field_block {
    const uint8_t* binary;
    int rx, ry, rz;
    const void *table, *w1, *w2;
    const uint32_t *offset, *size, *res;
    const float* scale;
    const uint32_t* hashed;
    const float *roi_aabb, *model_aabb, *center;
    const float* pose;
} dreg_field_block;
int dreg_scene_density(const float* x, long n, const float* origin, const float* spacing, int nx, int ny, int nz,
                       int n_blocks, const dreg_field_block* blocks, float power,
                       float* sigma, float* weight_block, float* sigma_block, void* stream);

typedef struct dreg_radiance_block {
    dreg_field_block field;
    const void *cw1, *cw2, *cw3;
    const float* dirbias;
} dreg_radiance_block;
int dreg_scene_voxel_grid(int rx, int ry, int rz, const float* grid_aabb, const float* jitter, int n_blocks, const dreg_radiance_block* blocks,
                          float power, float delta, float density_thre, float* voxel_grid, uint8_t* keep, float* sigma, void* stream);

int dreg_brick_supported(int B, int D, int H, int W, int Cin, int Cout);
size_t dreg_conv3_brick_pack_bytes(int rows, int red);
int dreg_pack_conv_weight_brick(const float* w, void* out, int Cout, int Cin, int transposed, void* stream);
size_t dreg_brick_tiles_workspace_bytes(int B, int D, int H, int W);
int dreg_brick_tiles_build(const uint8_t* flags, int B, int D, int H, int W, int max_rows, int max_tiles, void* workspace, size_t workspace_bytes,
                           int* meta, int* rows_sorted, void* tiles, int* halo_vox, void* nbr, void* stream);
int dreg_conv3_brick(const void* in, const void* wpk, void* out, const float* bias, const void* addend, const void* tiles, int ntiles,
                     const int* halo_vox, const void* nbr, const int* rows_sorted,
                     int B, int D, int H, int W, int Cin, int Cout, int Da, int Ha, int Wa, int add_same, int out_f32, void* stream);

int dreg_ps_num_params(void);
int dreg_ps_num_linears(void);
void* dreg_ps_create(const int64_t* params);
void dreg_ps_destroy(void* h);
void dreg_ps_set_fuse(void* h, int fuse);
void dreg_ps_set_group_wgrad(void* h, int on);
void dreg_ps_set_timing(void* h, int enable);
int dreg_ps_read_timings(void* h, int* info, float* ms, int cap);
size_t dreg_ps_arena_bytes(void* h, int R);
int dreg_ps_forward(void* h, void* arena, size_t arena_bytes, const int64_t* packs, const float* feats, const float* xyz, const float* pe,
                    const int* probs_self, const int* probs_cross, int nprob, int max_len, int R,
                    float* cond, float* corr, float* ov, void* stream);
int dreg_ps_backward(void* h, void* arena, size_t arena_bytes, const int64_t* packs, const float* feats, const float* xyz, const float* pe,
                     const int* probs_self, const int* probs_cross, int nprob, int max_len, int R,
                     const float* cond, const float* corr, const float* ov, const float* g_cond, const float* g_corr, const float* g_ov,
                     float* d_feats, void* stream, void* aux_stream, int last_only);
int dreg_ps_panel_fwd(const void* a1, const void* w1_packed, const float* bias1, const float* residual, float* x_out,
                      const float* gamma, const float* beta, const float* pe, void* h_out, float* stats,
                      const void* w2_packed, const float* bias2, void* out2, int R, int K1, int N2, int relu, float eps, void* stream);
int dreg_ps_panel_bwd(const void* g1, const void* w1t_packed, const float* x, const float* stats, const float* gamma,
                      const float* dx_add, const float* dx_add2, float* dx, void* dx_bf16, float* part,
                      const void* w2t_packed, void* out2, int R, int K1, int N2, void* stream);

#ifdef __cplusplus
}
#endif
#endif
```

Measured before the change: 265.2 pairs/s.

## Compute bias gradients inside wgrad kernels via MFMA against a ones vector

Adds a BIAS template variant of the wgrad kernel that accumulates the per-output-channel column sum of the output gradient. It does this with extra MFMAs against a bf16 ones operand, writes per-split partials, and sums them in the batched reduce kernel. This replaces a separate colsum or bias-gradient pass for convs and grouped linears in the executor and pointset paths. The cost is extra MFMA work in one wave column, extra workspace, and a wider reduce descriptor, which changes the ABI.

After: 266.5 pairs/s, median of 6. Within noise of the previous version (+0.5%).

```diff
diff --git a/dreg_nerf_amd/csrc/conv.hip b/dreg_nerf_amd/csrc/conv.hip
--- a/dreg_nerf_amd/csrc/conv.hip
+++ b/dreg_nerf_amd/csrc/conv.hip
@@ -861,12 +861,14 @@
     int block0;
 };
 static_assert(sizeof(WgradGroupDesc) == 144, "descriptor layout is part of the ABI (dreg_wgrad_group_desc_bytes)");
-template <int BM, int BNC, bool ROWS, int NW = 4, int ABL = 0, int KV_ = 64, int NS_ = 2, int PIPE = 0, int AP = 0, bool GRP = false>
+template <int BM, int BNC, bool ROWS, int NW = 4, int ABL = 0, int KV_ = 64, int NS_ = 2, int PIPE = 0, int AP = 0, bool GRP = false, bool BIAS = false>
 __global__ __launch_bounds__(NW * 64) void conv_wgrad_glds_kernel(
     const bf16_t* __restrict__ gout, const bf16_t* __restrict__ in, float* __restrict__ part,
     ConvGeom g, int tilesCol, int tiles, int nsplit, uint32_t vox_per_split, uint32_t gout_bytes, uint32_t in_bytes,
-    const int* __restrict__ rowlist, uint32_t nrows, const uint8_t* __restrict__ rowocc = nullptr, int rows_fast = 0)
-{
+    const int* __restrict__ rowlist, uint32_t nrows, const uint8_t* __restrict__ rowocc = nullptr, int rows_fast = 0,
+    float* __restrict__ bias_part = nullptr)
+{
+    static_assert(!BIAS || (ABL == 0 && PIPE == 0 && (AP == 0 || AP == 1 || AP == 3)), "bias partials: product forms only");
     uint32_t bid = blockIdx.x;
     if constexpr (GRP) {
         const WgradGroupDesc* D = reinterpret_cast<const WgradGroupDesc*>(rowocc);
@@ -878,6 +880,7 @@
         const WgradGroupDesc d = D[lo];
         gout = d.gout; in = d.in; part = d.part; g = d.g; tilesCol = d.tilesCol; tiles = d.tiles; nsplit = d.nsplit;
         vox_per_split = d.vps; gout_bytes = d.gbytes; in_bytes = d.ibytes; nrows = d.nrows;
+        if constexpr (BIAS) bias_part = bias_part ? reinterpret_cast<float* const*>(bias_part)[lo] : nullptr;
         rowocc = nullptr; rows_fast = 0; rowlist = nullptr;
         bid -= (uint32_t)d.block0;
     }
@@ -967,6 +970,15 @@
     for (int i = 0; i < TM; ++i)
 #pragma unroll
         for (int j = 0; j < TN; ++j) acc[i][j] = (f32x4_t){0.f, 0.f, 0.f, 0.f};
+    const bool do_bias = BIAS && bias_part != nullptr && tile_c == 0 && wn == 0;
+    f32x4_t bacc[BIAS ? TM : 1];
+    bf16x8_t ones;
+    if constexpr (BIAS) {
+        typedef __attribute__((ext_vector_type(4))) int i32x4_t;
+        ones = __builtin_bit_cast(bf16x8_t, (i32x4_t){0x3f803f80, 0x3f803f80, 0x3f803f80, 0x3f803f80});
+#pragma unroll
+        for (int i = 0; i < TM; ++i) bacc[i] = (f32x4_t){0.f, 0.f, 0.f, 0.f};
+    }
 
     const bool aligned = !ROWS && g.sn == 1 && g.sd == 1 && g.dsign == 1 &&
                          (((KV % g.Wo) == 0 && ((g.Ho * g.Wo) % KV) == 0) || (g.Wo % KV) == 0) &&
@@ -1200,6 +1212,12 @@
                     if constexpr (ABL != 1) acc[i][j] = __builtin_amdgcn_mfma_f32_16x16x32_bf16(af[i], bf[j], acc[i][j], 0, 0, 0);
                     else asm volatile("" :: "v"(af[i]), "v"(bf[j]));
                 }
+            if constexpr (BIAS) {
+                if (do_bias) {
+#pragma unroll
+                    for (int i = 0; i < TM; ++i) bacc[i] = __builtin_amdgcn_mfma_f32_16x16x32_bf16(af[i], ones, bacc[i], 0, 0, 0);
+                }
+            }
         }
     };
 
@@ -1277,6 +1295,14 @@
                         if constexpr (ABL != 1) acc[i][j] = __builtin_amdgcn_mfma_f32_16x16x32_bf16(af[i], bf[j], acc[i][j], 0, 0, 0);
                         else asm volatile("" :: "v"(af[i]), "v"(bf[j]));
                     }
+            };
+            auto mm_bias = [&]() {
+                typedef __attribute__((ext_vector_type(4))) int i32x4_t;
+#pragma unroll
+                for (int i = 0; i < TM; ++i) {
+                    i32x4_t t4 = {alo[i][0], alo[i][1], ahi[i][0], ahi[i][1]};
+                    bacc[i] = __builtin_amdgcn_mfma_f32_16x16x32_bf16(__builtin_bit_cast(bf16x8_t, t4), ones, bacc[i], 0, 0, 0);
+                }
             };
             uint32_t pa_off[IA], pb_off[IB], pb_m[IB];
             int cz = 0, cy = 0, cx = 0;
@@ -1420,6 +1446,9 @@
                 }
                 __builtin_amdgcn_s_setprio(0);
                 __builtin_amdgcn_sched_barrier(0);
+                if constexpr (BIAS) {
+                    if (do_bias) mm_bias();
+                }
                 stamp(4);
                 __builtin_amdgcn_s_barrier();
                 stamp(5);
@@ -1498,13 +1527,23 @@
                 if (n < g.Kpad) dst[(size_t)co * g.Kpad + n] = acc[i][j][r];
             }
         }
+    if constexpr (BIAS) {
+        if (do_bias && col_l == 0) {
+            float* bp = bias_part + (size_t)split * g.Cout;
+#pragma unroll
+            for (int i = 0; i < TM; ++i)
+#pragma unroll
+                for (int r = 0; r < 4; ++r) bp[co0 + wm * WM + i * 16 + rowq + r] = bacc[i][r];
+        }
+    }
 }
 
 struct WgradReduceDesc {
     const float* part; float* dw;
     int nsplit, Cout, Kpad, ntaps, Cin, Cin_real, accumulate, block0;
+    float* dbias;
 };
-static_assert(sizeof(WgradReduceDesc) == 48, "descriptor layout is part of the ABI");
+static_assert(sizeof(WgradReduceDesc) == 56 && offsetof(WgradReduceDesc, dbias) == 48, "descriptor layout is part of the ABI");
 constexpr int WR_STAGE = 8192;
 __host__ __device__ static inline int wr_epb(int nsplit) { return nsplit < 8 ? 2048 : (nsplit < 64 ? 512 : 128); }
 __host__ __device__ static inline int wr_chunk(int nsplit) { return nsplit < 32 ? 64 : 16; }
@@ -1530,6 +1569,14 @@
         nwritten = e < 1 ? 1 : (e < d.nsplit ? e : d.nsplit);
     }
     const bool accum = (d.accumulate & 1) != 0;
+    if (d.dbias && r == 0) {
+        const float* bp = d.part + (size_t)d.nsplit * slab + 64;
+        for (int co = t; co < d.Cout; co += 256) {
+            float a = 0.f;
+            for (int k = 0; k < nwritten; ++k) a += bp[(size_t)k * d.Cout + co];
+            d.dbias[co] = accum ? d.dbias[co] + a : a;
+        }
+    }
     if (d.ntaps == 1) {
         const int epb = wr_epb(d.nsplit), KG = 2048 / epb, EL = 256 / KG, g = t / EL, l = t - g * EL;
         const size_t total = (size_t)d.Cout * d.Cin_real;
@@ -2247,6 +2294,9 @@
 size_t dreg_conv3d_wgrad_workspace_bytes(int B, int Do, int Ho, int Wo, int Cin, int Cout, int ksz, int dtype) {
     const int Kpad = dreg_conv3d_kpad(ksz, Cin, dtype);
     return (size_t)dreg_conv3d_wgrad_splits(B, Do, Ho, Wo, Cin, Cout, ksz, dtype) * Cout * Kpad * sizeof(float) + 256;
+}
+size_t dreg_conv3d_wgrad_bias_bytes(int B, int Do, int Ho, int Wo, int Cin, int Cout, int ksz) {
+    return ((size_t)dreg_conv3d_wgrad_splits(B, Do, Ho, Wo, Cin, Cout, ksz, 0) * Cout * sizeof(float) + 255) / 256 * 256;
 }
 DREG_KNOB(bool, g_row_splits, true);
 #ifdef DREG_PROBE
@@ -2360,7 +2410,16 @@
     return c;
 }
 
-struct WgradArgs { const void *gout, *in; float* part; const int* rowlist; uint32_t nrows; const uint8_t* rowocc; };
+struct WgradArgs { const void *gout, *in; float* part; const int* rowlist; uint32_t nrows; const uint8_t* rowocc; float* bias_part; };
+static bool wgrad_bias_form(const WgradChoice& c)
+{
+    switch (c.family) {
+    case WG_GLDS4: return !c.occ;
+    case WG_ROWS8: case WG_ROWS8_AP: return true;
+    case WG_DENSE8: return c.abl == 0 && c.kv == 32 && c.ns == 4 && c.pipe == 0 && (c.ap == 3 || c.ap == 1);
+    default: return false;
+    }
+}
 template <typename T, bool TR>
 static void wgrad_reg_launch(const WgradChoice& c, const ConvGeom& g, const WgradArgs& a, hipStream_t st)
 {
@@ -2369,18 +2428,34 @@
     else if (c.bnc == 128) WG_LAUNCH(64, 128); else WG_LAUNCH(64, 64);
 #undef WG_LAUNCH
 }
-template <int BM, int BNC, bool ROWS, int NW = 4, int ABL = 0, int KV = 64, int NS = 2, int PIPE = 0, int AP = 0>
+template <int BM, int BNC, bool ROWS, int NW = 4, int ABL = 0, int KV = 64, int NS = 2, int PIPE = 0, int AP = 0, bool BIAS = false>
 static void wgrad_glds_launch(const WgradChoice& c, const ConvGeom& g, const WgradArgs& a, hipStream_t st)
 {
-    if (c.lds > 65536) (void)hipFuncSetAttribute((const void*)conv_wgrad_glds_kernel<BM, BNC, ROWS, NW, ABL, KV, NS, PIPE, AP>, hipFuncAttributeMaxDynamicSharedMemorySize, (int)c.lds);
-    hipLaunchKernelGGL((conv_wgrad_glds_kernel<BM, BNC, ROWS, NW, ABL, KV, NS, PIPE, AP>), c.grid, dim3(c.block), c.lds, st, (const bf16_t*)a.gout, (const bf16_t*)a.in, a.part, g,
-                       c.tilesCol, c.tilesRow * c.tilesCol, c.nsplit, c.vps, (uint32_t)c.gbytes, (uint32_t)c.ibytes, a.rowlist, a.nrows, a.rowocc, c.rows_fast);
-}
-template <bool ROWS>
+    if (c.lds > 65536) (void)hipFuncSetAttribute((const void*)conv_wgrad_glds_kernel<BM, BNC, ROWS, NW, ABL, KV, NS, PIPE, AP, false, BIAS>, hipFuncAttributeMaxDynamicSharedMemorySize, (int)c.lds);
+    hipLaunchKernelGGL((conv_wgrad_glds_kernel<BM, BNC, ROWS, NW, ABL, KV, NS, PIPE, AP, false, BIAS>), c.grid, dim3(c.block), c.lds, st, (const bf16_t*)a.gout, (const bf16_t*)a.in, a.part, g,
+                       c.tilesCol, c.tilesRow * c.tilesCol, c.nsplit, c.vps, (uint32_t)c.gbytes, (uint32_t)c.ibytes, a.rowlist, a.nrows, a.rowocc, c.rows_fast,
+                       BIAS ? a.bias_part : (float*)nullptr);
+}
+template <bool ROWS, bool BIAS = false>
 static void wgrad_glds4_launch(const WgradChoice& c, const ConvGeom& g, const WgradArgs& a, hipStream_t st)
 {
-    if (c.bm == 128 && c.bnc == 128) wgrad_glds_launch<128, 128, ROWS>(c, g, a, st); else if (c.bm == 128) wgrad_glds_launch<128, 64, ROWS>(c, g, a, st);
-    else if (c.bnc == 128) wgrad_glds_launch<64, 128, ROWS>(c, g, a, st); else wgrad_glds_launch<64, 64, ROWS>(c, g, a, st);
+    if (c.bm == 128 && c.bnc == 128) wgrad_glds_launch<128, 128, ROWS, 4, 0, 64, 2, 0, 0, BIAS>(c, g, a, st);
+    else if (c.bm == 128) wgrad_glds_launch<128, 64, ROWS, 4, 0, 64, 2, 0, 0, BIAS>(c, g, a, st);
+    else if (c.bnc == 128) wgrad_glds_launch<64, 128, ROWS, 4, 0, 64, 2, 0, 0, BIAS>(c, g, a, st);
+    else wgrad_glds_launch<64, 64, ROWS, 4, 0, 64, 2, 0, 0, BIAS>(c, g, a, st);
+}
+static void wgrad_bias_launch(const WgradChoice& c, const ConvGeom& g, const WgradArgs& a, hipStream_t st)
+{
+    switch (c.family) {
+    case WG_GLDS4: if (a.rowlist) wgrad_glds4_launch<true, true>(c, g, a, st); else wgrad_glds4_launch<false, true>(c, g, a, st); break;
+    case WG_ROWS8: wgrad_glds_launch<256, 256, true, 8, 0, 64, 2, 0, 0, true>(c, g, a, st); break;
+    case WG_ROWS8_AP: wgrad_glds_launch<256, 256, true, 8, 0, 32, 4, 0, 3, true>(c, g, a, st); break;
+    case WG_DENSE8:
+        if (c.ap == 3) wgrad_glds_launch<256, 256, false, 8, 0, 32, 4, 0, 3, true>(c, g, a, st);
+        else wgrad_glds_launch<256, 256, false, 8, 0, 32, 4, 0, 1, true>(c, g, a, st);
+        break;
+    default: break;
+    }
 }
 static void wgrad_dense8_launch(const WgradChoice& c, const ConvGeom& g, const WgradArgs& a, hipStream_t st)
 {
@@ -2395,18 +2470,22 @@
 static int wgrad_impl(const void* gout, const void* in, float* dw, void* workspace, size_t workspace_bytes,
                       int B, int Di, int Hi, int Wi, int Cin, int Cin_real, int Do, int Ho, int Wo, int Cout,
                       int ksz, int stride, int pad, int accumulate, int dtype, int use_tr, void* stream,
-                      const int* rowlist, uint32_t nrows_list, const uint8_t* rowocc = nullptr, bool defer_reduce = false)
+                      const int* rowlist, uint32_t nrows_list, const uint8_t* rowocc = nullptr, bool defer_reduce = false, bool bias = false)
 {
     ConvGeom g;
     int rc = fill_geom(g, B, Di, Hi, Wi, Cin, Do, Ho, Wo, Cout, ksz, stride, pad, 0, dtype == 0 ? 2 : 4);
     if (rc) return rc;
     if (Cout % 128 != 0 && Cout != 64) return DREG_EINVAL;
-    if (workspace_bytes < dreg_conv3d_wgrad_workspace_bytes(B, Do, Ho, Wo, Cin, Cout, ksz, dtype)) return DREG_EINVAL;
+    const size_t ws_bytes = dreg_conv3d_wgrad_workspace_bytes(B, Do, Ho, Wo, Cin, Cout, ksz, dtype);
+    if (workspace_bytes < ws_bytes) return DREG_EINVAL;
     if (rowlist && !(dtype == 0 && use_tr && g_use_glds)) return DREG_EINVAL;
     hipStream_t st = (hipStream_t)stream;
     const WgradChoice c = wgrad_choose(g, dtype, use_tr != 0, rowlist != nullptr, nrows_list, rowocc != nullptr);
     float* part = (float*)workspace;
-    const WgradArgs a{gout, in, part, rowlist, rowlist ? nrows_list : g.M, c.occ ? rowocc : nullptr};
+    if (bias && (!wgrad_bias_form(c) || workspace_bytes < ws_bytes + dreg_conv3d_wgrad_bias_bytes(B, Do, Ho, Wo, Cin, Cout, ksz))) return DREG_EINVAL;
+    const WgradArgs a{gout, in, part, rowlist, rowlist ? nrows_list : g.M, c.occ ? rowocc : nullptr, bias ? (float*)((char*)workspace + ws_bytes) : nullptr};
+    if (bias) wgrad_bias_launch(c, g, a, st);
+    else
     switch (c.family) {
     case WG_UNSUPPORTED: return DREG_EINVAL;
     case WG_REG:
@@ -2476,6 +2555,22 @@
     DREG_LAUNCH_CHECK();
     return DREG_OK;
 }
+int dreg_wgrad_group_launch_bias(const void* descs_dev, const void* bias_tab_dev, int n, int variant, int total_blocks, void* stream)
+{
+    if (n <= 0 || total_blocks <= 0) return DREG_OK;
+    if (!descs_dev || !bias_tab_dev) return DREG_EINVAL;
+    hipStream_t st = (hipStream_t)stream;
+    const int bm = variant / 1000, bnc = variant % 1000;
+    const ConvGeom g0{};
+#define WGRP(BMv, BNv) hipLaunchKernelGGL((conv_wgrad_glds_kernel<BMv, BNv, false, 4, 0, 64, 2, 0, 0, true, true>), dim3(total_blocks), dim3(256), (size_t)2 * 64 * (BMv + BNv) * 2, st, \
+        (const bf16_t*)nullptr, (const bf16_t*)nullptr, (float*)nullptr, g0, 0, 0, 0, 0u, 0u, 0u, (const int*)nullptr, 0u, (const uint8_t*)descs_dev, n, (float*)bias_tab_dev)
+    if (bm == 128 && bnc == 128) WGRP(128, 128); else if (bm == 128 && bnc == 64) WGRP(128, 64);
+    else if (bm == 64 && bnc == 128) WGRP(64, 128); else if (bm == 64 && bnc == 64) WGRP(64, 64);
+    else return DREG_EINVAL;
+#undef WGRP
+    DREG_LAUNCH_CHECK();
+    return DREG_OK;
+}
 
 int dreg_conv3d_wgrad(const void* gout, const void* in, float* dw, void* workspace, size_t workspace_bytes,
                       int B, int Di, int Hi, int Wi, int Cin, int Cin_real, int Do, int Ho, int Wo, int Cout,
@@ -2515,6 +2610,23 @@
     return wgrad_impl(gout, in, nullptr, workspace, workspace_bytes, B, Di, Hi, Wi, Cin, Cin_real, Do, Ho, Wo, Cout, ksz, stride, pad,
                       0, 0, 1, stream, rows, rows ? (uint32_t)nrows : 0, rows ? nullptr : rowocc, true);
 }
+int dreg_conv3d_wgrad_partials_bias(const void* gout, const void* in, void* workspace, size_t workspace_bytes, const int* rows, int nrows,
+                                    int B, int Di, int Hi, int Wi, int Cin, int Cin_real, int Do, int Ho, int Wo, int Cout,
+                                    int ksz, int stride, int pad, void* stream)
+{
+    if (rows && nrows < 0) return DREG_EINVAL;
+    return wgrad_impl(gout, in, nullptr, workspace, workspace_bytes, B, Di, Hi, Wi, Cin, Cin_real, Do, Ho, Wo, Cout, ksz, stride, pad,
+                      0, 0, 1, stream, rows, rows ? (uint32_t)nrows : 0, nullptr, true, true);
+}
+int dreg_conv3d_wgrad_bias_use(int B, int Di, int Hi, int Wi, int Cin, int Do, int Ho, int Wo, int Cout, int ksz, int stride, int pad,
+                               int rows, int nrows, int occ)
+{
+    ConvGeom g;
+    if (fill_geom(g, B, Di, Hi, Wi, Cin, Do, Ho, Wo, Cout, ksz, stride, pad, 0, 2) || (Cout % 128 != 0 && Cout != 64) || (rows && nrows < 0)) return 0;
+    const WgradChoice c = wgrad_choose(g, 0, true, rows != 0, (uint32_t)nrows, occ != 0);
+    if (!wgrad_bias_form(c)) return 0;
+    return 1;
+}
 int dreg_wgrad_reduce_blocks(int Cout, int Cin_real, int ksz, int nsplit) { return wgrad_reduce_blocks(Cout, Cin_real, ksz * ksz * ksz, nsplit); }
 int dreg_wgrad_reduce_batched(const void* descs_dev, int n, int block_base, int nblocks, void* stream)
 {
diff --git a/dreg_nerf_amd/csrc/executor.hip b/dreg_nerf_amd/csrc/executor.hip
--- a/dreg_nerf_amd/csrc/executor.hip
+++ b/dreg_nerf_amd/csrc/executor.hip
@@ -47,6 +47,7 @@
     int stats_bn = -1;
     size_t stats_off = 0;
     int stats_conv = -1;
+    int bias_wg = 0;
     int grp = 0;
     int fold_sk_fwd = 0, fold_sk_bwd = 0;
     int fold_into = -1, res_from = -1;
@@ -58,8 +59,8 @@
 struct PackRec { const float* w; void* out; int Cout, Cin_real, inner, ntaps, for_dgrad, Kpad, dtype, row0; };
 static_assert(sizeof(PackRec) == 48, "matches PackDesc of conv.hip");
 
-struct ReduceRec { const float* part; float* dw; int nsplit, Cout, Kpad, ntaps, Cin, Cin_real, accumulate, block0; };
-static_assert(sizeof(ReduceRec) == 48, "matches WgradReduceDesc of conv.hip");
+struct ReduceRec { const float* part; float* dw; int nsplit, Cout, Kpad, ntaps, Cin, Cin_real, accumulate, block0; float* dbias; };
+static_assert(sizeof(ReduceRec) == 56, "matches WgradReduceDesc of conv.hip");
 
 struct BnTailRec { const float* a; const float* b; float* o0; float* o1; int B, V, C, block0; };
 static_assert(sizeof(BnTailRec) == 48, "matches BnTailDesc of fpn_ops.hip");
@@ -158,7 +159,7 @@
     std::memset(o, 0, sizeof(*o));
     o->sparse_grads = 1; o->bn_batch_tails = 1; o->fuse_stem = 1; o->sparse_stem = 1; o->fold_res_bn = 1; o->fold_splitk = 1;
     o->group_wgrad = 1; o->s2_accumulate = 1; o->fuse_bn_stats = 1; o->brick = 1; o->defer_head_pg = 0; o->pointwise_stream = 1;
-    o->bn_self_coef = 1;
+    o->bn_self_coef = 1; o->bias_from_wgrad = 1;
 }
 void* dreg_exec_create(const int* tensors, int nt, const int* ops, int nops, const int64_t* params, int np)
 {
@@ -328,6 +329,16 @@
                     r.accumulate = (o.kind == OP_CONV_ROWS || o.rows_out >= 0) ? 3 : 1;
                     r.block0 = e->reduce_blocks;
                     e->reduce_blocks += dreg_wgrad_reduce_blocks(w.d0, w.d1, o.ksz, r.nsplit);
+                    const bool lr = o.kind == OP_CONV_ROWS || o.rows_out >= 0;
+                    if (e->opt.bias_from_wgrad && o.b >= 0 && e->prm[o.b].grad && o.in != 0 &&
+                        dreg_conv3d_wgrad_bias_use(x.B, x.D, x.H, x.W, x.C, y.D, y.H, y.W, w.d0, o.ksz, o.kind == OP_CONV_ROWS ? 1 : o.stride, o.pad, lr ? 1 : 0, lr ? 1 : 0, 0)) {
+                        bool shared_b = false;
+                        for (const ReduceRec& q : e->reduce) shared_b = shared_b || q.dbias == e->prm[o.b].grad;
+                        if (!shared_b) {
+                            o.bias_wg = 1; r.dbias = e->prm[o.b].grad;
+                            o.wg_bytes += dreg_conv3d_wgrad_bias_bytes(x.B, y.D, y.H, y.W, x.C, w.d0, o.ksz);
+                        }
+                    }
                     o.rd = (int)e->reduce.size();
                     e->reduce.push_back(r);
                 }
@@ -934,6 +945,9 @@
         if (w.grad) {
             Scope sc(e, ws, i, 2);
             if (o.rd >= 0) {
+                if (o.bias_wg) CK(dreg_conv3d_wgrad_partials_bias(gy, act(o.in), A + o.wg_off, o.wg_bytes, lrows ? r_out : nullptr, n_out, x.B, x.D, x.H, x.W, x.C, w.d1,
+                                                                  y.D, y.H, y.W, w.d0, o.ksz, rows ? 1 : o.stride, o.pad, (void*)ws));
+                else
                 CK(dreg_conv3d_wgrad_partials(gy, act(o.in), A + o.wg_off, o.wg_bytes, lrows ? r_out : nullptr, n_out, x.B, x.D, x.H, x.W, x.C, w.d1,
                                               y.D, y.H, y.W, w.d0, o.ksz, rows ? 1 : o.stride, o.pad, (!lrows && o.in == 0) ? e->in_rowocc : nullptr, (void*)ws));
                 rd_done[o.rd] = 1;
@@ -949,7 +963,7 @@
             }
         }
         if (flush_now) { CK(flush_reduce()); rd_pending = 0; }
-        if (o.b >= 0 && e->prm[o.b].grad) {
+        if (o.b >= 0 && e->prm[o.b].grad && !(o.bias_wg && w.grad)) {
             if (rows) CK(dreg_colsum_rows(gy, r_out, n_out, e->prm[o.b].grad, (float*)(A + e->off_cs), w.d0, 1, 0, (void*)bs));
             else CK(dreg_colsum(gy, e->prm[o.b].grad, (float*)(A + e->off_cs), (size_t)y.B * y.D * y.H * y.W, w.d0, 1, 0, (void*)bs));
         }
diff --git a/dreg_nerf_amd/csrc/pointset_exec.hip b/dreg_nerf_amd/csrc/pointset_exec.hip
--- a/dreg_nerf_amd/csrc/pointset_exec.hip
+++ b/dreg_nerf_amd/csrc/pointset_exec.hip
@@ -17,8 +17,8 @@
 constexpr int NLIN = NL * LIN_PER_LAYER + 2;
 
 struct Lin { int cout, cin, w, b; };
-struct ReduceRec { const float* part; float* dw; int nsplit, Cout, Kpad, ntaps, Cin, Cin_real, accumulate, block0; };
-static_assert(sizeof(ReduceRec) == 48, "matches WgradReduceDesc of conv.hip");
+struct ReduceRec { const float* part; float* dw; int nsplit, Cout, Kpad, ntaps, Cin, Cin_real, accumulate, block0; float* dbias; };
+static_assert(sizeof(ReduceRec) == 56, "matches WgradReduceDesc of conv.hip");
 struct ColsumRec { const void* g; float* out; float* partial; int M, C, rpc, nch, pblock0, fblock0, accumulate, pad; };
 static_assert(sizeof(ColsumRec) == 56, "matches ColsumDesc of fpn_ops.hip");
 struct LnRec { const float* part; float* dg; float* db; int nblk, accumulate; };
@@ -48,6 +48,7 @@
     int fuse = 1;
     int panel = 2;
     int group_wgrad = 1;
+    int bias_from_wgrad = 1;
     std::vector<hipEvent_t> ev;
     hipEvent_t ev_done = nullptr;
     static constexpr int RING = 8;
@@ -97,7 +98,7 @@
     for (int i = 0; i < NLIN; ++i) {
         const Lin& l = p->lin[i];
         const int rows = i < NL * LIN_PER_LAYER ? R : NL * R;
-        y.wg_bytes[i] = dreg_conv3d_wgrad_workspace_bytes(rows, 1, 1, 1, l.cin, l.cout, 1, 0);
+        y.wg_bytes[i] = dreg_conv3d_wgrad_workspace_bytes(rows, 1, 1, 1, l.cin, l.cout, 1, 0) + dreg_conv3d_wgrad_bias_bytes(rows, 1, 1, 1, l.cin, l.cout, 1);
         const size_t k1 = dreg_conv3d_igemm_workspace_bytes(rows, 1, 1, 1, l.cin, 1, 1, 1, l.cout, 1, 1, 0, 0, 0, 0);
         const size_t k2 = dreg_conv3d_igemm_workspace_bytes(rows, 1, 1, 1, l.cout, 1, 1, 1, l.cin, 1, 1, 0, 1, 0, 0);
         if (k1 > y.ks_bytes) y.ks_bytes = k1;
@@ -193,6 +194,7 @@
 }
 void dreg_ps_set_fuse(void* h, int fuse) { ((Ps*)h)->fuse = fuse ? 1 : 0; ((Ps*)h)->panel = fuse >= 3 ? 2 : fuse >= 2 ? 1 : 0; }
 void dreg_ps_set_group_wgrad(void* h, int on) { ((Ps*)h)->group_wgrad = on ? 1 : 0; }
+void dreg_ps_bias_from_wgrad(void* h, int on) { ((Ps*)h)->bias_from_wgrad = on ? 1 : 0; }
 void dreg_ps_set_timing(void* h, int enable) { ((Ps*)h)->timing = enable != 0; }
 int dreg_ps_read_timings(void* h, int* info, float* ms, int cap)
 {
@@ -306,9 +308,10 @@
     std::vector<ColsumRec> cs;
     std::vector<LnRec> ln;
     int rd_blocks = 0, cs_p = 0, cs_f = 0;
-    struct GroupRec { char d[160]; int variant, nblocks; };
+    struct GroupRec { char d[160]; int variant, nblocks; float* bias_part; };
     std::vector<GroupRec> grp;
     const bool group = fuse && p->group_wgrad && !p->timing;
+    const bool bias_wg = fuse && p->bias_from_wgrad;
     const bool panel = fuse && p->panel >= 2;
     auto panel_bwd = [&](const void* g1, const void* w1t, const float* x, const float* stt, const float* gamma, const float* add, const float* add2, float* dx, void* dx_bf,
                          float* part, const void* w2t, void* out2, int k1, int n2) {
@@ -318,21 +321,28 @@
     auto param_grads = [&](int li, const void* g, const void* x, int rows, size_t wg_off, size_t cs_off) -> int {
         const Lin& l = p->lin[li];
         bool grouped = false;
+        const bool bw = bias_wg && li < NL * LIN_PER_LAYER && p->grad[l.b] && dreg_conv3d_wgrad_bias_use(rows, 1, 1, 1, l.cin, 1, 1, 1, l.cout, 1, 1, 0, 0, 0, 0);
         if (group) {
             GroupRec gr{};
-            if (dreg_linear_wgrad_group_fill(gr.d, g, x, A + wg_off, y.wg_bytes[li], rows, l.cin, l.cout, &gr.variant, &gr.nblocks) == DREG_OK) { grp.push_back(gr); grouped = true; }
+            if (dreg_linear_wgrad_group_fill(gr.d, g, x, A + wg_off, y.wg_bytes[li], rows, l.cin, l.cout, &gr.variant, &gr.nblocks) == DREG_OK) {
+                gr.bias_part = bw ? (float*)(A + wg_off + dreg_conv3d_wgrad_workspace_bytes(rows, 1, 1, 1, l.cin, l.cout, 1, 0)) : nullptr;
+                grp.push_back(gr); grouped = true;
+            }
         }
         if (!grouped) {
             if (two) { if (hipEventRecord(p->ev[li], st) != hipSuccess || hipStreamWaitEvent(ax, p->ev[li], 0) != hipSuccess) return DREG_ELAUNCH; }
             PsScope sc(p, ax, 2, rows, l.cin, l.cout, 0);
-            CK(dreg_conv3d_wgrad_partials(g, x, A + wg_off, y.wg_bytes[li], nullptr, 0, rows, 1, 1, 1, l.cin, l.cin, 1, 1, 1, l.cout, 1, 1, 0, nullptr, ax));
+            if (bw) CK(dreg_conv3d_wgrad_partials_bias(g, x, A + wg_off, y.wg_bytes[li], nullptr, 0, rows, 1, 1, 1, l.cin, l.cin, 1, 1, 1, l.cout, 1, 1, 0, ax));
+            else CK(dreg_conv3d_wgrad_partials(g, x, A + wg_off, y.wg_bytes[li], nullptr, 0, rows, 1, 1, 1, l.cin, l.cin, 1, 1, 1, l.cout, 1, 1, 0, nullptr, ax));
         }
         ReduceRec r{};
         r.part = (const float*)(A + wg_off); r.dw = p->grad[l.w];
         r.nsplit = dreg_conv3d_wgrad_splits(rows, 1, 1, 1, l.cin, l.cout, 1, 0);
         r.Cout = l.cout; r.Kpad = dreg_conv3d_kpad(1, l.cin, 0); r.ntaps = 1; r.Cin = l.cin; r.Cin_real = l.cin; r.accumulate = 1; r.block0 = rd_blocks;
         rd_blocks += dreg_wgrad_reduce_blocks(l.cout, l.cin, 1, r.nsplit);
+        if (bw) r.dbias = p->grad[l.b];
         rd.push_back(r);
+        if (bw) return DREG_OK;
         if (!fuse) return dreg_colsum(g, p->grad[l.b], (float*)(A + y.cs_ws), (size_t)rows, l.cout, 1, 0, ax);
         ColsumRec c{};
         c.g = g; c.out = p->grad[l.b]; c.partial = (float*)(A + cs_off); c.M = rows; c.C = l.cout;
@@ -465,7 +475,8 @@
     const int gd = dreg_wgrad_group_desc_bytes();
     std::stable_sort(grp.begin(), grp.end(), [](const GroupRec& a, const GroupRec& b) { return a.variant < b.variant; });
     const size_t o_grp = al(o_ln + nb_ln), nb_grp = grp.size() * (size_t)gd;
-    if (gd > 160 || o_grp + nb_grp > Ps::TABLE_BYTES) return DREG_EINVAL;
+    const size_t o_bt = al(o_grp + nb_grp), nb_bt = bias_wg ? grp.size() * sizeof(float*) : 0;
+    if (gd > 160 || o_bt + nb_bt > Ps::TABLE_BYTES) return DREG_EINVAL;
     if (o_ln + nb_ln > Ps::TABLE_BYTES) return DREG_EINVAL;
     const unsigned slot = p->ring_next++ % Ps::RING;
     if (!p->ring_ev[slot]) { if (hipEventCreateWithFlags(&p->ring_ev[slot], hipEventDisableTiming) != hipSuccess) return DREG_ELAUNCH; }
@@ -474,24 +485,28 @@
     std::memcpy(host, rd.data(), nb_rd);
     std::memcpy(host + o_cs, cs.data(), nb_cs);
     std::memcpy(host + o_ln, ln.data(), nb_ln);
-    struct GroupLaunch { size_t off; int n, variant, blocks; };
+    struct GroupLaunch { size_t off, bt_off; int n, variant, blocks; };
     std::vector<GroupLaunch> gl;
     for (size_t i = 0; i < grp.size(); ++i) {
-        if (gl.empty() || gl.back().variant != grp[i].variant) gl.push_back(GroupLaunch{o_grp + i * (size_t)gd, 0, grp[i].variant, 0});
+        if (gl.empty() || gl.back().variant != grp[i].variant) gl.push_back(GroupLaunch{o_grp + i * (size_t)gd, o_bt + i * sizeof(float*), 0, grp[i].variant, 0});
         const int b0 = gl.back().blocks;
         std::memcpy(grp[i].d + gd - (int)sizeof(int), &b0, sizeof(int));
         std::memcpy(host + o_grp + i * (size_t)gd, grp[i].d, (size_t)gd);
+        if (bias_wg) std::memcpy(host + o_bt + i * sizeof(float*), &grp[i].bias_part, sizeof(float*));
         gl.back().n += 1; gl.back().blocks += grp[i].nblocks;
     }
-    if (hipMemcpyAsync(A + y.tables, host, grp.empty() ? o_ln + nb_ln : o_grp + nb_grp, hipMemcpyHostToDevice, st) != hipSuccess) return DREG_ELAUNCH;
+    if (hipMemcpyAsync(A + y.tables, host, grp.empty() ? o_ln + nb_ln : o_bt + nb_bt, hipMemcpyHostToDevice, st) != hipSuccess) return DREG_ELAUNCH;
     if (hipEventRecord(p->ring_ev[slot], st) != hipSuccess) return DREG_ELAUNCH;
     if (two && hipStreamWaitEvent(ax, p->ring_ev[slot], 0) != hipSuccess) return DREG_ELAUNCH;
     const int ln_dup = (ln.size() >= 2 && ln[0].dg == ln[1].dg) ? 1 : 0;
     if (ln_dup) CK(dreg_layernorm_bwd_final_batched(A + y.tables + o_ln, 1, stream));
     CK(dreg_layernorm_bwd_final_batched(A + y.tables + o_ln + ln_dup * sizeof(LnRec), (int)ln.size() - ln_dup, stream));
-    for (const GroupLaunch& q : gl) CK(dreg_wgrad_group_launch(A + y.tables + q.off, q.n, q.variant, q.blocks, ax));
+    for (const GroupLaunch& q : gl) {
+        if (bias_wg) CK(dreg_wgrad_group_launch_bias(A + y.tables + q.off, A + y.tables + q.bt_off, q.n, q.variant, q.blocks, ax));
+        else CK(dreg_wgrad_group_launch(A + y.tables + q.off, q.n, q.variant, q.blocks, ax));
+    }
     CK(dreg_wgrad_reduce_batched(A + y.tables, (int)rd.size(), 0, rd_blocks, ax));
-    if (fuse) CK(dreg_colsum_batched(A + y.tables + o_cs, (int)cs.size(), cs_p, cs_f, ax));
+    if (fuse && !cs.empty()) CK(dreg_colsum_batched(A + y.tables + o_cs, (int)cs.size(), cs_p, cs_f, ax));
     return DREG_OK;
 }
 
diff --git a/dreg_nerf_amd/lib.py b/dreg_nerf_amd/lib.py
--- a/dreg_nerf_amd/lib.py
+++ b/dreg_nerf_amd/lib.py
@@ -82,6 +82,11 @@
     "dreg_wgrad_group_desc_bytes": (I, []),
     "dreg_linear_wgrad_group_fill": (I, [P, P, P, P, Z, I, I, I, P, P]),
     "dreg_wgrad_group_launch": (I, [P, I, I, I, P]),
+    "dreg_conv3d_wgrad_bias_bytes": (Z, [I] * 7),
+    "dreg_conv3d_wgrad_bias_use": (I, [I] * 15),
+    "dreg_conv3d_wgrad_partials_bias": (I, [P, P, P, Z, P, I] + [I] * 13 + [P]),
+    "dreg_wgrad_group_launch_bias": (I, [P, P, I, I, I, P]),
+    "dreg_ps_bias_from_wgrad": (None, [P, I]),
     "dreg_bn_num_chunks": (I, [I]),
     "dreg_bn_relu_maxpool_fwd": (I, [P] * 10 + [I] * 8 + [F, F, I, I, P]),
     "dreg_bn_relu_maxpool_bwd": (I, [P] * 10 + [I] * 10 + [P]),
@@ -324,7 +329,7 @@
 
 class ExecOpts(ctypes.Structure):
     _fields_ = [(n, c_int) for n in ("sparse_grads", "bn_batch_tails", "fuse_stem", "sparse_stem", "fold_res_bn", "fold_splitk", "group_wgrad",
-                                     "s2_accumulate", "fuse_bn_stats", "brick", "defer_head_pg", "persistent_deep", "guard", "pointwise_stream", "bn_self_coef")] + [("reserved", c_int * 1)]
+                                     "s2_accumulate", "fuse_bn_stats", "brick", "defer_head_pg", "persistent_deep", "guard", "pointwise_stream", "bn_self_coef", "bias_from_wgrad")]
 
 
 SCENE_MAX_BLOCKS = 4
diff --git a/dreg_nerf_amd/ops.py b/dreg_nerf_amd/ops.py
--- a/dreg_nerf_amd/ops.py
+++ b/dreg_nerf_amd/ops.py
@@ -312,8 +312,12 @@
 
 
 _PENDING_REDUCE = []
-_REDUCE_DT = np.dtype([("part", "<u8"), ("dw", "<u8"), ("nsplit", "<i4"), ("Cout", "<i4"), ("Kpad", "<i4"), ("ntaps", "<i4"),
-                       ("Cin", "<i4"), ("Cin_real", "<i4"), ("accumulate", "<i4"), ("block0", "<i4")])
+_REDUCE_FIELDS = [("part", "<u8"), ("dw", "<u8"), ("nsplit", "<i4"), ("Cout", "<i4"), ("Kpad", "<i4"), ("ntaps", "<i4"),
+                  ("Cin", "<i4"), ("Cin_real", "<i4"), ("accumulate", "<i4"), ("block0", "<i4")]
+_REDUCE_BIAS_DT = np.dtype(_REDUCE_FIELDS + [("dbias", "<u8")])
+_REDUCE_DT = np.dtype({"names": [n for n, _ in _REDUCE_FIELDS], "formats": [f for _, f in _REDUCE_FIELDS],
+                       "offsets": [_REDUCE_BIAS_DT.fields[n][1] for n, _ in _REDUCE_FIELDS], "itemsize": _REDUCE_BIAS_DT.itemsize})
+assert _REDUCE_DT.itemsize == 56
 
 
 def flush_wgrad_reduce():
diff --git a/dreg_nerf_amd/pointset_exec.py b/dreg_nerf_amd/pointset_exec.py
--- a/dreg_nerf_amd/pointset_exec.py
+++ b/dreg_nerf_amd/pointset_exec.py
@@ -21,6 +21,7 @@
 FUSE = True
 PANEL = 3
 GROUP_WGRAD = True
+BIAS_FROM_WGRAD = True
 
 
 def _fuse_level() -> int:
@@ -62,8 +63,10 @@
             raise L.DregError("dreg_ps_create failed")
         self.lib.dreg_ps_set_fuse(self.h, _fuse_level())
         self.lib.dreg_ps_set_group_wgrad(self.h, int(GROUP_WGRAD))
+        self.lib.dreg_ps_bias_from_wgrad(self.h, int(BIAS_FROM_WGRAD))
         self._fuse = _fuse_level()
         self._group = GROUP_WGRAD
+        self._bias_wg = BIAS_FROM_WGRAD
         self.device = self.params[0].device
         self.arena = None
         self.arena_bytes = 0
@@ -141,6 +144,9 @@
         if self._group != GROUP_WGRAD:
             self.lib.dreg_ps_set_group_wgrad(self.h, int(GROUP_WGRAD))
             self._group = GROUP_WGRAD
+        if self._bias_wg != BIAS_FROM_WGRAD:
+            self.lib.dreg_ps_bias_from_wgrad(self.h, int(BIAS_FROM_WGRAD))
+            self._bias_wg = BIAS_FROM_WGRAD
         want = ops.PROFILER is not None and ops.PROFILER.enabled
         if want != self._timing:
             self.set_timing(want)
diff --git a/include/dreg_nerf.h b/include/dreg_nerf.h
--- a/include/dreg_nerf.h
+++ b/include/dreg_nerf.h
@@ -98,6 +98,13 @@
 int dreg_conv3d_wgrad_partials(const void* gout, const void* in, void* workspace, size_t workspace_bytes, const int* rows, int nrows,
                                int B, int Di, int Hi, int Wi, int Cin, int Cin_real, int Do, int Ho, int Wo, int Cout,
                                int ksz, int stride, int pad, const uint8_t* rowocc, void* stream);
+size_t dreg_conv3d_wgrad_bias_bytes(int B, int Do, int Ho, int Wo, int Cin, int Cout, int ksz);
+int dreg_conv3d_wgrad_bias_use(int B, int Di, int Hi, int Wi, int Cin, int Do, int Ho, int Wo, int Cout, int ksz, int stride, int pad,
+                               int rows, int nrows, int occ);
+int dreg_conv3d_wgrad_partials_bias(const void* gout, const void* in, void* workspace, size_t workspace_bytes, const int* rows, int nrows,
+                                    int B, int Di, int Hi, int Wi, int Cin, int Cin_real, int Do, int Ho, int Wo, int Cout,
+                                    int ksz, int stride, int pad, void* stream);
+int dreg_wgrad_group_launch_bias(const void* descs_dev, const void* bias_tab_dev, int n, int variant, int total_blocks, void* stream);
 int dreg_wgrad_reduce_blocks(int Cout, int Cin_real, int ksz, int nsplit);
 int dreg_wgrad_reduce_batched(const void* descs_dev, int n, int block_base, int nblocks, void* stream);
 int dreg_wgrad_group_desc_bytes(void);
@@ -244,7 +251,7 @@
     int guard;
     int pointwise_stream;
     int bn_self_coef;
-    int reserved[1];
+    int bias_from_wgrad;
 } dreg_exec_opts;
 void dreg_exec_default_opts(dreg_exec_opts* o);
 void* dreg_exec_create_opts(const int* tensors, int nt, const int* ops, int nops, const int64_t* params, int np, const dreg_exec_opts* opts);
@@ -601,6 +608,7 @@
 void* dreg_ps_create(const int64_t* params);
 void dreg_ps_destroy(void* h);
 void dreg_ps_set_fuse(void* h, int fuse);
+void dreg_ps_bias_from_wgrad(void* h, int on);
 void dreg_ps_set_group_wgrad(void* h, int on);
 void dreg_ps_set_timing(void* h, int enable);
 int dreg_ps_read_timings(void* h, int* info, float* ms, int cap);
```
